# arnab39/equiadapt

Hardware: AMD Instinct MI355X
Metric: canonicalize+invert images/sec (224x224 C8) (higher is better)
Workload: dtype f32 (resampling / FFT / accumulation in fp32; the network's channel contraction as 2xfp16 split of every fp32 operand (within one fp32 ulp), 3 exact products, fp32 accumulate -- closer to fp64 than the fp32 matrix instruction, see step_ms_by_gemm_form); 1 GPU; configs[1]: 224x224x3 synthetic, C8, GroupEquivariantImageCanonicalization + ESCNNEquivariantNetwork in e2cnn's LAYER SHAPES (32 fields x 8 = 256 ch, k5, 3 layers, crop 0.8, resize 96) with this repository's own filter-bank parameterisation (bilinear-rotated banks; e2cnn's steerable basis is not restated -- e2cnn-trained weights enter via load_exported_dense), forward, then invert_canonicalization; batch_per_gpu=256, global_batch=256, parallelism=dp1 (no collective in the forward path)

## Files before the change

equiadapt_amd/_lib.py:

```python
import ctypes
import os
import subprocess
import threading

_HERE = os.path.dirname(os.path.abspath(__file__))
ROOT = os.path.dirname(_HERE)
CSRC = os.path.join(_HERE, "csrc")
SO_PATH = os.environ.get("EQA_LIB") or os.path.join(CSRC, "libeqa_hip.so")
SOURCES = [os.path.join(CSRC, f) for f in ("group_action.hip", "crop_resize.hip", "nearest_action.hip", "pooling.hip", "batchnorm.hip", "winograd.hip", "lift_conv.hip", "lift_conv_wide.hip", "lift_wgrad.hip", "pointcloud.hip", "vnsmall_train.hip", "vnsmall_tail.hip", "fftconv.hip", "fft_filter.hip", "lift_fft.hip", "cgemm3m.hip", "cgemm3m_bf16.hip", "smallconv.hip", "planegemm.hip", "convnet_train.hip", "fourier_act.hip", "nbody.hip")]
HEADERS = [os.path.join(CSRC, "eqa_common.hpp"), os.path.join(CSRC, "vn_common.hpp"), os.path.join(CSRC, "fft48.inc"), os.path.join(CSRC, "fft_common.inc"), os.path.join(CSRC, "cgemm3m_common.inc")]
INCLUDE = os.path.join(ROOT, "include")

ABI_VERSION = 3

_c_f = ctypes.POINTER(ctypes.c_float)
_c_i = ctypes.POINTER(ctypes.c_int32)
_vp = ctypes.c_void_p
_int = ctypes.c_int

SIGNATURES = {
    "eqa_abi_version": (_int, []),
    "eqa_set_option": (_int, [_int, _int]),
    "eqa_get_option": (_int, [_int]),
    "eqa_fold_edge_pad_workspace_bytes": (ctypes.c_int64, [_int] * 4),
    "eqa_fold_edge_pad": (_int, [_vp, _vp, _vp, _int, _int, _int, _int, _vp]),
    "eqa_canon_transform_fwd": (_int, [_vp, _vp, _vp, _vp, _vp] + [_int] * 6 + [_vp]),
    "eqa_invert_action_fwd": (_int, [_vp, _vp, _vp, _vp, _vp, _vp] + [_int] * 6 + [_vp]),
    "eqa_group_action_pair": (_int, [_vp] * 4 + [_int, _int] + [_vp] * 5 + [_int, _int, _vp] + [_int] * 4 + [_vp]),
    "eqa_orbit_expand_fwd": (_int, [_vp, _vp, _vp, _vp] + [_int] * 5 + [_vp]),
    "eqa_group_action_fwd": (_int, [_vp, _vp, _vp, _vp, _vp, _vp] + [_int] * 12 + [_vp]),
    "eqa_group_action_fwd_hint": (_int, [_vp, _vp, _vp, _vp, _vp, _vp] + [_int] * 13 + [_vp]),
    "eqa_crop_resize_aa": (_int, [_vp] * 6 + [_int] * 9 + [_vp]),
    "eqa_mask_action_nearest": (_int, [_vp] * 5 + [_int] * 4 + [_vp]),
    "eqa_mask_action_nearest_planes": (_int, [_vp] * 5 + [_int] * 4 + [_vp]),
    "eqa_boxes_action": (_int, [_vp] * 5 + [_int, ctypes.c_float, _int, _vp]),
    "eqa_image_action_nearest": (_int, [_vp] * 5 + [_int] * 10 + [_vp]),
    "eqa_group_action_bwd_tiles": (_int, [_int, _int]),
    "eqa_group_action_bwd": (_int, [_vp] * 8 + [_int] * 12 + [_vp]),
    "eqa_group_action_bwd_theta": (_int, [_vp] * 8 + [_int] * 12 + [_vp]),
    "eqa_group_pool_workspace_bytes": (ctypes.c_int64, [_int] * 4),
    "eqa_group_pool_argmax": (_int, [_vp, _vp, _vp, _vp] + [_int] * 4 + [_vp]),
    "eqa_window_sums": (_int, [_vp, _vp, _vp, _int, _vp] + [_int] * 5 + [_vp]),
    "eqa_bn_partial_blocks": (ctypes.c_int64, [ctypes.c_int64]),
    "eqa_bn_stats_nhwc": (_int, [_vp, _vp, ctypes.c_int64, _int, _vp]),
    "eqa_bn_relu_dropout_nhwc": (_int, [_vp, _vp, _vp, _vp, ctypes.c_int64, _int, ctypes.c_float, ctypes.c_uint32, _vp]),
    "eqa_bn_bwd_reduce_nhwc": (_int, [_vp] * 5 + [ctypes.c_float, _vp, ctypes.c_int64, _int, _vp, _vp, ctypes.c_uint32, _vp]),
    "eqa_bn_bwd_apply_nhwc": (_int, [_vp] * 8 + [ctypes.c_float, _vp, ctypes.c_int64, _int, _vp, _vp, ctypes.c_uint32, _vp]),
    "eqa_window_sums_nhwc_act": (_int, [_vp, _vp, _vp, _int, ctypes.c_float, ctypes.c_uint32, _vp, _vp] + [_int] * 5 + [_vp]),
    "eqa_bn_bwd_reduce_nhwc_wsgrad": (_int, [_vp] * 4 + [ctypes.c_float, _vp] + [_int] * 5 + [_vp, _vp, ctypes.c_uint32, _vp]),
    "eqa_bn_bwd_apply_nhwc_wsgrad": (_int, [_vp] * 7 + [ctypes.c_float, _vp] + [_int] * 5 + [_vp, _vp, ctypes.c_uint32, _vp]),
    "eqa_vn_blocks": (_int, [_int]),
    "eqa_vn_knn": (_int, [_vp, _vp, _int, _int, _int, _vp]),
    "eqa_vn_convpos_stats": (_int, [_vp, _vp, _vp, _vp, _int, _int, _int, _vp]),
    "eqa_vn_convpos_fwd": (_int, [_vp] * 7 + [_int, _int, _int, _vp]),
    "eqa_vn_convpos_bwd_reduce": (_int, [_vp] * 10 + [_int, _int, _int, _vp]),
    "eqa_vn_convpos_bwd_apply": (_int, [_vp] * 12 + [_int, _int, _int, _vp]),
    "eqa_vn_convpos_max_fwd": (_int, [_vp] * 9 + [_int, _int, _int, _vp]),
    "eqa_vn_convpos_max_bwd_reduce": (_int, [_vp] * 11 + [_int, _int, _int, _vp]),
    "eqa_vn_convpos_max_bwd_apply": (_int, [_vp] * 13 + [_int, _int, _int, _vp]),
    "eqa_vn_tail_blocks": (_int, [_int]),
    "eqa_vn_tail_partial_floats": (_int, [_int]),
    "eqa_vn_tail_pass": (_int, [_int] + [_vp] * 8 + [_int, _int, _vp]),
    "eqa_vn_bn_finalize": (_int, [_vp, _int, _int, _int, ctypes.c_int64] + [_vp] * 5 + [ctypes.c_float, ctypes.c_float, _vp, _vp]),
    "eqa_vn_bn_bwd_finalize": (_int, [_vp, _int, _int, _int, ctypes.c_int64, _vp, _vp, _vp]),
    "eqa_window_grad_table": (_int, [_vp, _vp] + [_int] * 5 + [_vp]),
    "eqa_window_sums_gemv_bwd_workspace_bytes": (ctypes.c_int64, [_int, _int]),
    "eqa_window_sums_gemv_bwd": (_int, [_vp] * 6 + [_int, _int, _int, ctypes.c_double, _vp]),
    "eqa_window_sums_gemv": (_int, [_vp, _vp, _vp, _int, _int, _int, ctypes.c_double, ctypes.c_double, _vp]),
    "eqa_lift_conv_nhwc": (_int, [_vp, _vp, _vp, _int, _vp] + [_int] * 7 + [_vp]),
    "eqa_lift_conv_grouped": (_int, [_vp, _vp, _vp, _int, _vp] + [_int] * 7 + [_vp]),
    "eqa_lift_conv_stats_rows": (_int, [_int] * 7),
    "eqa_lift_conv_nhwc_stats": (_int, [_vp, _vp, _vp, _vp] + [_int] * 7 + [_vp]),
    "eqa_lift_conv_wgrad_supported": (_int, [_int] * 7),
    "eqa_lift_conv_wgrad_workspace_bytes": (ctypes.c_int64, [_int] * 7),
    "eqa_lift_conv_wgrad_nhwc": (_int, [_vp, _vp, _vp, _vp] + [_int] * 7 + [_vp]),
    "eqa_plane_gemm_supported": (_int, [_int, _int]),
    "eqa_plane_gemm": (_int, [_vp, _vp, _vp, ctypes.c_longlong, _int, _int, _int, _vp]),
    "eqa_winograd_f2k5_input": (_int, [_vp, _vp, _vp, _int, _int, _int, _int, _int, _vp]),
    "eqa_winograd_f2k5_output": (_int, [_vp, _vp, _int, _vp, _int, _int, _int, _int, _vp]),
    "eqa_winograd_f4k5_input": (_int, [_vp, _vp, _vp, _int, _int, _int, _int, _int, _vp]),
    "eqa_winograd_f4k5_output": (_int, [_vp, _vp, _int, _vp, _int, _int, _int, _int, _vp]),
    "eqa_winograd_f2k5_input_padded": (_int, [_vp, _vp, _int, _int, _int, _int, _int, _vp]),
    "eqa_winograd_f4k5_input_padded": (_int, [_vp, _vp, _int, _int, _int, _int, _int, _vp]),
    "eqa_winograd_f2k5_output_adjoint": (_int, [_vp, _vp, _int, _int, _int, _int, _vp]),
    "eqa_winograd_f4k5_output_adjoint": (_int, [_vp, _vp, _int, _int, _int, _int, _vp]),
    "eqa_winograd_f2k5_output_sums_workspace_bytes": (ctypes.c_int64, [_int] * 4),
    "eqa_winograd_f2k5_output_sums": (_int, [_vp, _vp, _int, _vp, _vp] + [_int] * 5 + [_vp]),
    "eqa_winograd_f4k5_output_sums": (_int, [_vp, _vp, _int, _vp, _vp] + [_int] * 5 + [_vp]),
    "eqa_fft48k5_tiles": (ctypes.c_int64, [_int]),
    "eqa_fft48k5_tile_pitch": (ctypes.c_int64, [ctypes.c_int64]),
    "eqa_fft48k5_frequencies": (_int, []),
    "eqa_fft48k5_filter_spectra": (_int, [_vp, _vp, _int, _int, _int, _vp]),
    "eqa_fft48k5_input_grad": (_int, [_vp, _vp, _vp] + [_int] * 4 + [_vp]),
    "eqa_fft48k5_grad_transform": (_int, [_vp, _vp, _vp] + [_int] * 4 + [_vp]),
    "eqa_fft48k5_filter_grad": (_int, [_vp, _vp, _int, _int, _vp]),
    "eqa_fft48k5_filter_grad3m": (_int, [_vp, _vp, _int, _int, _vp]),
    "eqa_fft48k5_cgemm3m_supported": (_int, [_int, _int]),
    "eqa_fft48k5_spectra3m_floats": (ctypes.c_int64, [_int, _int]),
    "eqa_fft48k5_filter_spectra3m": (_int, [_vp, _vp, _int, _int, _int, _vp]),
    "eqa_fft48k5_cgemm3m": (_int, [_vp, _vp, _vp, ctypes.c_int64, _int, _int, _vp]),
    "eqa_lift_conv_wide_supported": (_int, [_int, _int, _int, _int]),
    "eqa_lift_conv_wide_weight_floats": (ctypes.c_int64, [_int, _int, _int, _int]),
    "eqa_lift_conv_wide": (_int, [_vp, _vp, _vp, _int, _vp, _int, _int, _int, _int, _int, _int, _int, _vp]),
    "eqa_lift_conv_wide_wgrad_workspace_bytes": (ctypes.c_int64, [_int, _int, _int, _int]),
    "eqa_lift_conv_wide_wgrad": (_int, [_vp, _vp, _vp, _vp, _int, _int, _int, _int, _int, _int, _int, _vp]),
    "eqa_fft48k5_spectra3m_bf16_bytes": (ctypes.c_int64, [_int, _int]),
    "eqa_fft48k5_spectra3m_split": (_int, [_vp, _vp, _int, _int, _vp]),
    "eqa_fft48k5_cgemm3m_bf16x3": (_int, [_vp, _vp, _vp, ctypes.c_int64, _int, _int, _int, _vp]),
    "eqa_fft48k5_spectra3m_f16_bytes": (ctypes.c_int64, [_int, _int]),
    "eqa_fft48k5_spectra3m_split_f16": (_int, [_vp, _vp, _int, _int, ctypes.c_float, _vp]),
    "eqa_fft48k5_cgemm3m_f16x2": (_int, [_vp, _vp, _vp, ctypes.c_int64, _int, _int, _vp, _int, ctypes.c_float, _vp]),
    "eqa_fft48k5_wgrad3m_supported": (_int, [_int, _int]),
    "eqa_fft48k5_wgrad3m": (_int, [_vp, _vp, _vp, ctypes.c_int64, _int, _int, _vp]),
    "eqa_fft48k5_group": (_int, [_int, _int]),
    "eqa_fft48k5_workspace_bytes": (ctypes.c_int64, [_int] * 4),
    "eqa_fft48k5_input": (_int, [_vp, _vp, _vp, _vp] + [_int] * 5 + [_vp]),
    "eqa_fft48k5_input_grouped": (_int, [_vp, _vp, _vp, _vp] + [_int] * 5 + [_vp]),
    "eqa_fft48k5_input_grouped_supported": (_int, [_int]),
    "eqa_lift5_fft48k5_input_supported": (_int, [_int] * 4),
    "eqa_lift5_fft48k5_input": (_int, [_vp, _vp, _vp, _int, _vp] + [_int] * 4 + [_vp]),
    "eqa_lift5_fft48k5_input_dcmax": (_int, [_vp, _vp, _vp, _int, _vp, _vp] + [_int] * 4 + [_vp]),
    "eqa_lift5_pieces_f16_bytes": (ctypes.c_int64, [_int]),
    "eqa_absmax_slots": (_int, [_vp, ctypes.c_int64, _vp, _vp]),
    "eqa_lift5_fft48k5_input_f16x2": (_int, [_vp, _vp, ctypes.c_float, _vp, _int, _vp, _int, _vp, _vp] + [_int] * 4 + [_vp]),
    "eqa_lift5_pieces_bytes": (ctypes.c_int64, [_int]),
    "eqa_lift5_fft48k5_input_bf16x3": (_int, [_vp, _vp, _vp, _int, _vp] + [_int] * 4 + [_vp]),
    "eqa_fft48k5_output": (_int, [_vp, _vp, _vp, _int, _vp] + [_int] * 4 + [_vp]),
    "eqa_fft48k5_output_stats_rows": (ctypes.c_int64, [_int] * 4),
    "eqa_fft48k5_output_stats": (_int, [_vp, _vp, _vp, _vp] + [_int] * 4 + [_vp]),
    "eqa_fft48k5_output_sums": (_int, [_vp, _vp, _vp, _int, _vp, _vp] + [_int] * 5 + [_vp]),
    "eqa_fft48_supported": (_int, [_int]),
    "eqa_fft48_tiles": (ctypes.c_int64, [_int, _int]),
    "eqa_fft48_workspace_bytes": (ctypes.c_int64, [_int] * 5),
    "eqa_fft48_filter_spectra": (_int, [_vp, _vp, _int, _int, _int, _int, _vp]),
    "eqa_fft48_filter_spectra3m": (_int, [_vp, _vp, _int, _int, _int, _int, _vp]),
    "eqa_fft48_input": (_int, [_vp, _vp, _vp, _vp] + [_int] * 6 + [_vp]),
    "eqa_fft48_grad_transform": (_int, [_vp, _vp, _vp] + [_int] * 5 + [_vp]),
    "eqa_fft48_output": (_int, [_vp, _vp, _vp, _int, _vp] + [_int] * 5 + [_vp]),
    "eqa_fft48_input_grad": (_int, [_vp, _vp, _vp] + [_int] * 5 + [_vp]),
    "eqa_fft48_filter_grad": (_int, [_vp, _vp, _int, _int, _int, _int, _vp]),
    "eqa_conv_s2_supported": (_int, [_int] * 5),
    "eqa_conv_s2": (_int, [_vp, _vp, _vp, _int, _vp] + [_int] * 8 + [_vp]),
    "eqa_conv_s2_wgrad_supported": (_int, [_int] * 5),
    "eqa_conv_s2_wgrad_workspace_bytes": (ctypes.c_int64, [_int] * 8),
    "eqa_conv_s2_wgrad": (_int, [_vp] * 4 + [_int] * 8 + [_vp]),
    "eqa_conv_s2_dgrad_supported": (_int, [_int] * 4),
    "eqa_conv_s2_dgrad": (_int, [_vp] * 3 + [_int] * 7 + [_vp]),
    "eqa_bn_act_fwd": (_int, [_vp] * 5 + [ctypes.c_int64, _int, _int, _vp]),
    "eqa_bn_act_partial_blocks": (ctypes.c_int64, [ctypes.c_int64]),
    "eqa_bn_act_stats": (_int, [_vp, _vp, ctypes.c_int64, _int, _vp]),
    "eqa_bn_act_finalize": (_int, [_vp, ctypes.c_int64, _int, _vp, _vp, ctypes.c_double, ctypes.c_double] + [_vp] * 6 + [_vp]),
    "eqa_bn_act_bwd_finalize": (_int, [_vp, ctypes.c_int64, _int] + [_vp] * 7 + [_vp]),
    "eqa_bn_act_bwd_reduce": (_int, [_vp] * 8 + [ctypes.c_int64, _int, _int, _vp]),
    "eqa_bn_act_bwd_apply": (_int, [_vp] * 11 + [ctypes.c_int64, _int, _int, _vp]),
    "eqa_affine_relu_rows": (_int, [_vp, _vp, _vp, _vp, ctypes.c_int64, _int, _vp]),
    "eqa_cosine_group_activations": (_int, [_vp, _vp, _vp, _int, _int, _int, ctypes.c_float, _vp]),
    "eqa_bias_relu_nhwc": (_int, [_vp, _vp, ctypes.c_int64, _int, _vp]),
    "eqa_window_sums_nhwc_workspace_bytes": (ctypes.c_int64, [_int] * 4),
    "eqa_window_sums_nhwc": (_int, [_vp, _vp, _vp, _int, _vp, _vp] + [_int] * 5 + [_vp]),
    "eqa_window_sums_bwd_expand_nhwc": (_int, [_vp, _vp] + [_int] * 5 + [_vp]),
    "eqa_group_argmax": (_int, [_vp, _vp, _int, _int, _vp]),
    "eqa_vnsmall_workspace_bytes": (ctypes.c_int64, [_int, _int]),
    "eqa_vnsmall_fwd": (_int, [_vp, _vp, _vp, _vp, _int, _int, _int, _int, _vp]),
    "eqa_vnsmall_canonicalize": (_int, [_vp] * 6 + [_int] * 4 + [_vp]),
    "eqa_so3_rotate": (_int, [_vp, _vp, _vp, _int, _int, _int, _vp]),
    "eqa_gram_schmidt": (_int, [_vp, _vp, _int, _vp]),
    "eqa_gram_schmidt_bwd": (_int, [_vp, _vp, _vp, _int, _vp]),
    "eqa_modified_gram_schmidt": (_int, [_vp, _vp, _int, _vp]),
    "eqa_rigid_rows": (_int, [_vp, _vp, _vp, _vp, _int, _int, _vp]),
    "eqa_fourier_elu_fwd": (_int, [_vp, _vp, _vp, _vp, ctypes.c_longlong, _int, _vp]),
    "eqa_fourier_elu_bwd": (_int, [_vp, _vp, _vp, _vp, _vp, ctypes.c_longlong, _int, _vp]),
    "eqa_vndeepsets_param_count": (_int, [_int] * 3),
    "eqa_vndeepsets_bwd_blocks": (_int, [_int]),
    "eqa_nbody_adjacency": (_int, [_vp, _vp, ctypes.c_longlong, _int, _vp, _vp, _vp]),
    "eqa_vndeepsets_fwd": (_int, [_vp] * 7 + [_int] * 5 + [ctypes.c_float] + [_int] * 3 + [_vp]),
    "eqa_vndeepsets_train_fwd": (_int, [_vp] * 9 + [_int] * 5 + [ctypes.c_float] + [_int] * 3 + [_vp]),
    "eqa_vndeepsets_bwd": (_int, [_vp] * 10 + [_int] * 5 + [ctypes.c_float] + [_int] * 3 + [_vp]),
}

_lock = threading.Lock()
_lib = None


def source_hash(*names: str) -> str:
    import hashlib

    h = hashlib.sha1()
    for path in [os.path.join(CSRC, n) for n in names] + HEADERS:
        with open(path, "rb") as f:
            h.update(f.read())
    return h.hexdigest()[:16]


class EqaLibraryError(RuntimeError):
    pass


def build(force: bool = False, verbose: bool = False, extra_flags=(), out: str = None) -> str:
    import hashlib
    from concurrent.futures import ThreadPoolExecutor

    if extra_flags and not out:
        raise ValueError("a variant build (extra_flags) needs its own `out`: it must not replace the product library")
    out = out or SO_PATH
    hdr_time = max(os.path.getmtime(p) for p in HEADERS + [os.path.join(INCLUDE, "eqa_hip.h")])
    newest_src = max(hdr_time, max(os.path.getmtime(p) for p in SOURCES))
    if not force and not extra_flags and os.path.exists(out) and os.path.getmtime(out) >= newest_src:
        return out
    hipcc = os.environ.get("HIPCC", "/opt/rocm/bin/hipcc")
    flags = ["--offload-arch=gfx950", "-O3", "-fno-slp-vectorize", "-std=c++17", "-fPIC", "-I", INCLUDE, *extra_flags]
    tag = hashlib.sha1(" ".join(flags).encode()).hexdigest()[:10]
    objdir = os.path.join(CSRC, "_obj")
    os.makedirs(objdir, exist_ok=True)
    import fcntl

    lock_file = open(os.path.join(objdir, ".lock"), "w")
    fcntl.flock(lock_file, fcntl.LOCK_EX)
    try:
        if not force and not extra_flags and os.path.exists(out) and os.path.getmtime(out) >= newest_src:
            return out
        return _build_locked(hipcc, flags, tag, objdir, out, hdr_time, force, verbose, bool(extra_flags))
    finally:
        fcntl.flock(lock_file, fcntl.LOCK_UN)
        lock_file.close()


def _pid_alive(pid: int) -> bool:
    try:
        os.kill(pid, 0)
    except ProcessLookupError:
        return False
    except PermissionError:
        return True
    return True


def _build_locked(hipcc, flags, tag, objdir, out, hdr_time, force, verbose, variant):
    from concurrent.futures import ThreadPoolExecutor
    import re
    import time

    started = time.time()

    def compile_one(src):
        obj = os.path.join(objdir, f"{os.path.splitext(os.path.basename(src))[0]}.{tag}.o")
        if not force and os.path.exists(obj) and os.path.getmtime(obj) >= max(hdr_time, os.path.getmtime(src)):
            return obj, None
        tmp_obj = f"{obj}.tmp{os.getpid()}"
        cmd = [hipcc, *flags, "-c", src, "-o", tmp_obj]
        if verbose:
            print(" ".join(cmd))
        res = subprocess.run(cmd, capture_output=True, text=True)
        if res.returncode != 0:
            if os.path.exists(tmp_obj):
                os.remove(tmp_obj)
            return obj, f"{' '.join(cmd)}\n{res.stdout}\n{res.stderr}"
        os.replace(tmp_obj, obj)
        return obj, None

    with ThreadPoolExecutor(max_workers=min(6, os.cpu_count() or 1)) as pool:
        results = list(pool.map(compile_one, SOURCES))
    errors = [e for _, e in results if e]
    if errors:
        raise EqaLibraryError("hipcc failed:\n" + "\n".join(errors))
    tmp = out + f".tmp{os.getpid()}"
    cmd = [hipcc, "--offload-arch=gfx950", "-shared", "-fPIC", *[o for o, _ in results], "-o", tmp]
    res = subprocess.run(cmd, capture_output=True, text=True)
    if res.returncode != 0:
        raise EqaLibraryError(f"link failed ({res.returncode}):\n{res.stdout}\n{res.stderr}")
    os.replace(tmp, out)
    if not variant:
        keep = {os.path.basename(o) for o, _ in results}
        for name in os.listdir(objdir):
            path = os.path.join(objdir, name)
            try:
                m = re.search(r"\.o\.tmp(\d+)$", name)
                if m:
                    if not _pid_alive(int(m.group(1))):
                        os.remove(path)
                elif name.endswith(".o") and name not in keep and os.path.getmtime(path) < started:
                    os.remove(path)
            except OSError:
                pass
    return out


def load() -> ctypes.CDLL:
    global _lib
    if _lib is not None:
        return _lib
    with _lock:
        if _lib is not None:
            return _lib
        if not os.path.exists(SO_PATH):
            raise EqaLibraryError(
                f"{SO_PATH} is missing. Build it with `python -c 'import __graft_entry__ as g; g.build()'` "
                "(hipcc --offload-arch=gfx950). equiadapt_amd has no CPU fallback."
            )
        lib = ctypes.CDLL(SO_PATH)
        for name, (restype, argtypes) in SIGNATURES.items():
            try:
                fn = getattr(lib, name)
            except AttributeError as exc:
                raise EqaLibraryError(f"{SO_PATH} does not export {name}; rebuild it") from exc
            fn.restype = restype
            fn.argtypes = argtypes
        if lib.eqa_abi_version() != ABI_VERSION:
            raise EqaLibraryError("libeqa_hip.so ABI version mismatch; rebuild it")
        _lib = lib
    return _lib


_ERRORS = {-1: "invalid argument", -2: "kernel launch failed", -3: "unsupported size/shape"}


def check(status: int, what: str) -> None:
    if status != 0:
        raise EqaLibraryError(f"{what} failed: {_ERRORS.get(status, status)}")
```

equiadapt_amd/csrc/crop_resize.hip:

```cpp
#include "eqa_common.hpp"

namespace {

constexpr int kAaBand = 8;
#ifndef EQA_AA_WIDE_MIN_K
#define EQA_AA_WIDE_MIN_K 8
#endif
constexpr int kAaMaxK = 20;

__global__ __launch_bounds__(kThreads) void crop_resize_aa_kernel(const float* __restrict__ x, float* __restrict__ y,
                                                                 const float* __restrict__ wx, const int32_t* __restrict__ x0,
                                                                 const float* __restrict__ wy, const int32_t* __restrict__ y0,
                                                                 int H, int W, int OH, int OW, int K, int max_rows) {
  extern __shared__ __attribute__((aligned(16))) float aa_tmp[];
  const int plane = blockIdx.y;
  const int r0 = blockIdx.x * kAaBand, r1 = min(r0 + kAaBand, OH);
  const int ybeg = y0[r0];
  const int yend = min(y0[r1 - 1] + K, H);
  const int nrows = min(yend - ybeg, max_rows);
  const float* src = x + (size_t)plane * H * W;
  const int rows_par = kThreads / OW;
  if (rows_par >= 1) {
    const int ox = threadIdx.x % OW, rsub = threadIdx.x / OW;
    if (rsub < rows_par) {
      const int xs = x0[ox];
      float wv[EQA_AA_WIDE_MIN_K];
      int xo[EQA_AA_WIDE_MIN_K];
#pragma unroll
      for (int j = 0; j < EQA_AA_WIDE_MIN_K; ++j) {
        wv[j] = j < K ? wx[ox * K + j] : 0.0f;
        xo[j] = min(xs + j, W - 1);
      }
      for (int ry = rsub; ry < nrows; ry += rows_par) {
        const float* row = src + (size_t)(ybeg + ry) * W;
        float xv[EQA_AA_WIDE_MIN_K];
#pragma unroll
        for (int j = 0; j < EQA_AA_WIDE_MIN_K; ++j) xv[j] = j < K ? row[xo[j]] : 0.0f;
        float acc = 0.0f;
#pragma unroll
        for (int j = 0; j < EQA_AA_WIDE_MIN_K; ++j)
          if (j < K) acc += wv[j] * xv[j];
        aa_tmp[ry * OW + ox] = acc;
      }
    }
  } else {
    for (int idx = threadIdx.x; idx < nrows * OW; idx += kThreads) {
      const int ry = idx / OW, ox = idx - ry * OW;
      const float* row = src + (size_t)(ybeg + ry) * W;
      const int xs = x0[ox];
      float acc = 0.0f;
#pragma unroll
      for (int j = 0; j < EQA_AA_WIDE_MIN_K; ++j)
        if (j < K) acc += wx[ox * K + j] * row[min(xs + j, W - 1)];
      aa_tmp[ry * OW + ox] = acc;
    }
  }
  __syncthreads();
  float* dst = y + (size_t)plane * OH * OW;
  for (int idx = threadIdx.x; idx < (r1 - r0) * OW; idx += kThreads) {
    const int r = idx / OW, ox = idx - r * OW;
    const int oy = r0 + r;

    const int ys = y0[oy] - ybeg;
    float acc = 0.0f;
#pragma unroll
    for (int j = 0; j < EQA_AA_WIDE_MIN_K; ++j)
      if (j < K) acc += wy[oy * K + j] * aa_tmp[min(ys + j, nrows - 1) * OW + ox];
    dst[(size_t)oy * OW + ox] = acc;
  }
}


template <int K, int BAND, int NL>
__global__ __launch_bounds__(kThreads, (NL > 5 && K > 5) ? 2 : 4) void crop_resize_aa_staged_kernel(
    const float* __restrict__ x, float* __restrict__ y,
                                                                        const float* __restrict__ wx, const int32_t* __restrict__ x0,
                                                                        const float* __restrict__ wy, const int32_t* __restrict__ y0,
                                                                        int planes, int H, int W, int OH, int OW, int cap_rows,
                                                                        int xb, int xl) {
  extern __shared__ __attribute__((aligned(16))) float aa_tmp[];
  float* rows = aa_tmp;
  float* tmp = aa_tmp + (size_t)cap_rows * xl;
  float* tabw = tmp + (size_t)cap_rows * OW;
  int* taby = reinterpret_cast<int*>(tabw + BAND * K);
  const int r0 = blockIdx.y * BAND, r1 = min(r0 + BAND, OH);
  const int nband = r1 - r0;
  const int plane0 = (int)(blockIdx.z * kXcd + blockIdx.x), plane_step = (int)(gridDim.z * kXcd);
  const int rows_par = kThreads / OW;
  const int ox = rows_par >= 1 ? threadIdx.x % OW : 0, rsub = rows_par >= 1 ? threadIdx.x / OW : 0;
  const int xs_g = x0[ox];
  float wv[K];
  int xo[K];
#pragma unroll
  for (int j = 0; j < K; ++j) {
    wv[j] = wx[ox * K + j];
    xo[j] = min(xs_g - xb + j, xl - 1);
  }
  if ((int)threadIdx.x < nband * K) tabw[threadIdx.x] = wy[r0 * K + threadIdx.x];
  const int ybeg = y0[r0];
  if ((int)threadIdx.x < nband) taby[threadIdx.x] = y0[r0 + threadIdx.x] - ybeg;
  const int yend = min(y0[r1 - 1] + K, H);
  const int nrows = min(yend - ybeg, cap_rows);
  const int nq = xl >> 2;
  const int tq = threadIdx.x & 63, tr = threadIdx.x >> 6;
  const bool prefetch = nq <= 64 && nrows <= 4 * NL;
  const size_t plane_sz = (size_t)H * W;
  const float* src0 = x + (size_t)ybeg * W + xb;
  typedef float aa_f4 __attribute__((ext_vector_type(4)));
  aa_f4 v[NL];
#define EQA_AA_PF_LOAD(plane_)                                                                                          \
  do {                                                                                                                  \
    const float* src_ = src0 + (size_t)(plane_) * plane_sz;                                                             \
    _Pragma("unroll") for (int k = 0; k < NL; ++k)                                                           \
      v[k] = *reinterpret_cast<const aa_f4*>(src_ + (size_t)min(tr + 4 * k, nrows - 1) * W + 4 * min(tq, nq - 1));     \
  } while (0)
  __builtin_amdgcn_s_waitcnt(0x0070);
  if (prefetch && plane0 < planes) EQA_AA_PF_LOAD(plane0);
  for (int plane = plane0; plane < planes; plane += plane_step) {
    if (prefetch) {
      if (tq < nq) {
#pragma unroll
        for (int k = 0; k < NL; ++k)
          if (tr + 4 * k < nrows) *reinterpret_cast<aa_f4*>(rows + (tr + 4 * k) * xl + 4 * tq) = v[k];
      }
      if (plane + plane_step < planes) EQA_AA_PF_LOAD(plane + plane_step);
    } else {
      const float* src = src0 + (size_t)plane * plane_sz;
      for (int q = tq; q < nq; q += 64)
        for (int rb = tr; rb < nrows; rb += 4) *reinterpret_cast<aa_f4*>(rows + rb * xl + 4 * q) = *reinterpret_cast<const aa_f4*>(src + (size_t)rb * W + 4 * q);
    }
    __syncthreads();
    if (rows_par >= 1) {
      if (rsub < rows_par) {
        for (int ry0 = rsub; ry0 < nrows; ry0 += 4 * rows_par) {
          float acc[4] = {0.0f, 0.0f, 0.0f, 0.0f};
#pragma unroll
          for (int u = 0; u < 4; ++u) {
            const float* row = rows + min(ry0 + u * rows_par, nrows - 1) * xl;
#pragma unroll
            for (int j = 0; j < K; ++j)
              acc[u] += wv[j] * row[xo[j]];
          }
#pragma unroll
          for (int u = 0; u < 4; ++u)
            if (ry0 + u * rows_par < nrows) tmp[(ry0 + u * rows_par) * OW + ox] = acc[u];
        }
      }
    } else {
      for (int idx = threadIdx.x; idx < nrows * OW; idx += kThreads) {
        const int ry = idx / OW, oxx = idx - ry * OW;
        const float* row = rows + ry * xl;
        const int xs = x0[oxx] - xb;
        float acc = 0.0f;
#pragma unroll
        for (int j = 0; j < K; ++j)
          acc += wx[oxx * K + j] * row[min(xs + j, xl - 1)];
        tmp[ry * OW + oxx] = acc;
      }
    }
    __syncthreads();
    float* dst = y + (size_t)plane * OH * OW;
    for (int idx = threadIdx.x; idx < nband * OW; idx += kThreads) {
      const int r = idx / OW, oxx = idx - r * OW;
      const int ys = taby[r];
      float acc = 0.0f;
#pragma unroll
      for (int j = 0; j < K; ++j)
        acc += tabw[r * K + j] * tmp[min(ys + j, nrows - 1) * OW + oxx];
      dst[(size_t)(r0 + r) * OW + oxx] = acc;
    }
    __syncthreads();
  }
#undef EQA_AA_PF_LOAD
}

__global__ __launch_bounds__(kThreads) void crop_resize_aa_wide_kernel(const float* __restrict__ x, float* __restrict__ y,
                                                                      const float* __restrict__ wx, const int32_t* __restrict__ x0,
                                                                      const float* __restrict__ wy, const int32_t* __restrict__ y0,
                                                                      int H, int W, int OH, int OW, int K, int max_rows, int xbeg,
                                                                      int xlen, int pad_shift, int row_stride, int rpi) {
  extern __shared__ __attribute__((aligned(16))) float aa_tmp[];
  float* rowbuf = aa_tmp + (size_t)max_rows * OW;
  const int plane = blockIdx.y;
  const int r0 = blockIdx.x * kAaBand, r1 = min(r0 + kAaBand, OH);
  const int ybeg = y0[r0];
  const int yend = min(y0[r1 - 1] + K, H);
  const int nrows = min(yend - ybeg, max_rows);
  const float* src = x + (size_t)plane * H * W;
  auto pos = [&](int e) { return pad_shift ? e + (e >> pad_shift) : e; };
  const bool fixed_col = (kThreads % OW) == 0 && K <= kAaMaxK;
  const bool vec_stage = rpi <= 8 && (xlen & 3) == 0 && (xbeg & 3) == 0 && (W & 3) == 0 && ((((uintptr_t)src) & 15) == 0);
  const int ox_fixed = threadIdx.x % OW;
  const int xs_fixed = x0[ox_fixed] - xbeg;
  float wreg[kAaMaxK];
#pragma unroll
  for (int j = 0; j < kAaMaxK; ++j) wreg[j] = (fixed_col && j < K) ? wx[ox_fixed * K + j] : 0.0f;
  const bool prefetch = vec_stage && xlen <= 4 * kThreads;
  const int e_pf = 4 * threadIdx.x;
  float4 pf[8];
  auto pf_load = [&](int ry0) {
    const int nr = min(rpi, nrows - ry0);
#pragma unroll
    for (int rr = 0; rr < 8; ++rr)
      pf[rr] = *reinterpret_cast<const float4*>(src + (size_t)(ybeg + ry0 + min(rr, nr - 1)) * W + xbeg + min(e_pf, xlen - 4));
  };
  if (prefetch && nrows > 0) pf_load(0);
  for (int ry0 = 0; ry0 < nrows; ry0 += rpi) {
    const int nr = min(rpi, nrows - ry0);
    if (prefetch) {
      if (e_pf < xlen) {
#pragma unroll
        for (int rr = 0; rr < 8; ++rr) {
          if (rr < nr) {
            float* lrow = rowbuf + rr * row_stride;
            lrow[pos(e_pf)] = pf[rr].x; lrow[pos(e_pf + 1)] = pf[rr].y; lrow[pos(e_pf + 2)] = pf[rr].z; lrow[pos(e_pf + 3)] = pf[rr].w;
          }
        }
      }
      if (ry0 + rpi < nrows) pf_load(ry0 + rpi);
    } else if (vec_stage) {
      for (int e = 4 * threadIdx.x; e < xlen; e += 4 * kThreads) {
        float4 v[8];
#pragma unroll
        for (int rr = 0; rr < 8; ++rr)
          v[rr] = *reinterpret_cast<const float4*>(src + (size_t)(ybeg + ry0 + min(rr, nr - 1)) * W + xbeg + e);
#pragma unroll
        for (int rr = 0; rr < 8; ++rr) {
          if (rr < nr) {
            float* lrow = rowbuf + rr * row_stride;
            lrow[pos(e)] = v[rr].x; lrow[pos(e + 1)] = v[rr].y; lrow[pos(e + 2)] = v[rr].z; lrow[pos(e + 3)] = v[rr].w;
          }
        }
      }
    } else {
      for (int rr = 0; rr < nr; ++rr) {
        const float* grow = src + (size_t)(ybeg + ry0 + rr) * W + xbeg;
        float* lrow = rowbuf + rr * row_stride;
        for (int e = threadIdx.x; e < xlen; e += kThreads) lrow[pos(e)] = grow[e];
      }
    }
    __syncthreads();
    if (fixed_col) {
      for (int rr = threadIdx.x / OW; rr < nr; rr += kThreads / OW) {
        const float* row = rowbuf + rr * row_stride;
        float acc = 0.0f;
#pragma unroll
        for (int j = 0; j < kAaMaxK; ++j)
          if (j < K) acc += wreg[j] * row[pos(min(xs_fixed + j, xlen - 1))];
        aa_tmp[(ry0 + rr) * OW + ox_fixed] = acc;
      }
    } else {
      for (int idx = threadIdx.x; idx < nr * OW; idx += kThreads) {
        const int rr = idx / OW, ox = idx - rr * OW;
        const float* row = rowbuf + rr * row_stride;
        const int xs = x0[ox] - xbeg;
        float acc = 0.0f;
        for (int j = 0; j < K; ++j) acc += wx[ox * K + j] * row[pos(min(xs + j, xlen - 1))];
        aa_tmp[(ry0 + rr) * OW + ox] = acc;
      }
    }
    __syncthreads();
  }
  float* dst = y + (size_t)plane * OH * OW;
  for (int idx = threadIdx.x; idx < (r1 - r0) * OW; idx += kThreads) {
    const int r = idx / OW, ox = idx - r * OW;
    const int oy = r0 + r;
    const int ys = y0[oy] - ybeg;
    float acc = 0.0f;
    for (int j = 0; j < K; ++j) acc += wy[oy * K + j] * aa_tmp[min(ys + j, nrows - 1) * OW + ox];
    dst[(size_t)oy * OW + ox] = acc;
  }
}

constexpr int kAaStreamRows = 8;
__global__ __launch_bounds__(kThreads) void crop_resize_aa_stream_kernel(const float* __restrict__ x, float* __restrict__ y,
                                                                        const float* __restrict__ wx, const int32_t* __restrict__ x0,
                                                                        const float* __restrict__ wy, const int32_t* __restrict__ y0,
                                                                        int H, int W, int OH, int OW, int K, int xbeg, int xlen,
                                                                        int pad_shift, int row_stride) {
  extern __shared__ __attribute__((aligned(16))) float aa_rows[];
  const int plane = blockIdx.y;
  const int r0 = blockIdx.x * kAaBand, nr_out = min(kAaBand, OH - r0);
  int ys[kAaBand];
#pragma unroll
  for (int r = 0; r < kAaBand; ++r) ys[r] = y0[r0 + min(r, nr_out - 1)];
  const int ybeg = ys[0];
  const int span = ys[kAaBand - 1] + K - ybeg;
  const float* src = x + (size_t)plane * H * W + xbeg;
  const int e = 4 * (int)threadIdx.x;
  const int e_ld = min(e, xlen - 4);
  auto pos = [&](int i) { return pad_shift ? i + (i >> pad_shift) : i; };
  float4 acc[kAaBand];
#pragma unroll
  for (int r = 0; r < kAaBand; ++r) acc[r] = make_float4(0.f, 0.f, 0.f, 0.f);
  auto load8 = [&](float4 (&v)[kAaStreamRows], int yc) {
#pragma unroll
    for (int q = 0; q < kAaStreamRows; ++q)
      v[q] = *reinterpret_cast<const float4*>(src + (size_t)min(ybeg + yc + q, H - 1) * W + e_ld);
  };
  const int lane = threadIdx.x & 63;
  const int wq = lane >> 3, wr = lane & 7;
  const int ys_w = y0[r0 + min(wr, nr_out - 1)];
  auto wload = [&](int yc) {
    const int t = ybeg + yc + wq - ys_w;
    const bool ok = wr < nr_out && t >= 0 && t < K && yc + wq < span;
    return ok ? wy[(size_t)(r0 + wr) * K + min(max(t, 0), K - 1)] : 0.0f;
  };
  auto add8 = [&](const float4 (&v)[kAaStreamRows], float wv) {
#pragma unroll
    for (int q = 0; q < kAaStreamRows; ++q) {
#pragma unroll
      for (int r = 0; r < kAaBand; ++r) {
        const float w = __builtin_bit_cast(float, __builtin_amdgcn_readlane(__builtin_bit_cast(int, wv), 8 * q + r));
        acc[r].x += w * v[q].x; acc[r].y += w * v[q].y; acc[r].z += w * v[q].z; acc[r].w += w * v[q].w;
      }
    }
  };
  static_assert(kAaStreamRows == 8 && kAaBand == 8, "one weight per lane: 8 rows of a trip x 8 output rows = 64 lanes");
  float4 va[kAaStreamRows], vb[kAaStreamRows];
  float wa, wb = 0.0f;
  load8(va, 0);
  wa = wload(0);
  for (int yc = 0; yc < span; yc += 2 * kAaStreamRows) {
    if (yc + kAaStreamRows < span) { load8(vb, yc + kAaStreamRows); wb = wload(yc + kAaStreamRows); }
    add8(va, wa);
    if (yc + 2 * kAaStreamRows < span) { load8(va, yc + 2 * kAaStreamRows); wa = wload(yc + 2 * kAaStreamRows); }
    if (yc + kAaStreamRows < span) add8(vb, wb);
  }
  float* dst = y + (size_t)plane * OH * OW;
#pragma unroll
  for (int half = 0; half < 2; ++half) {
    if (e < xlen) {
#pragma unroll
      for (int rr = 0; rr < kAaBand / 2; ++rr) {
        float* lrow = aa_rows + rr * row_stride;
        const float4 v = acc[half * (kAaBand / 2) + rr];
        lrow[pos(e)] = v.x; lrow[pos(e + 1)] = v.y; lrow[pos(e + 2)] = v.z; lrow[pos(e + 3)] = v.w;
      }
    }
    __syncthreads();
    for (int idx = threadIdx.x; idx < (kAaBand / 2) * OW; idx += kThreads) {
      const int rr = idx / OW, ox = idx - rr * OW;
      const int r = half * (kAaBand / 2) + rr;
      if (r < nr_out) {
        const float* row = aa_rows + rr * row_stride;
        const int xs = x0[ox] - xbeg;
        float a = 0.0f;
        for (int j = 0; j < K; ++j) a += wx[ox * K + j] * row[pos(min(xs + j, xlen - 1))];
        dst[(size_t)(r0 + r) * OW + ox] = a;
      }
    }
    __syncthreads();
  }
}

}

extern "C" {

int eqa_crop_resize_aa(const float* x, float* y, const float* wx, const int32_t* x0, const float* wy, const int32_t* y0,
                       int planes, int H, int W, int OH, int OW, int K, int max_rows, int x_begin, int x_span, void* stream) {
  if (!x || !y || !wx || !x0 || !wy || !y0 || planes < 0 || H <= 0 || W <= 0 || OH <= 0 || OW <= 0 || K <= 0 || max_rows <= 0)
    return EQA_ERR_INVALID_ARG;
  const size_t lds = (size_t)max_rows * OW * sizeof(float);
  if (lds > 96 * 1024 || planes > 65535) return EQA_ERR_UNSUPPORTED;
  if (planes == 0) return EQA_OK;
  const dim3 grid((OH + kAaBand - 1) / kAaBand, planes);
  if (K > EQA_AA_WIDE_MIN_K && x_span > 0 && x_begin >= 0 && x_begin + x_span <= W) {
    const int stride = (x_span + OW / 2) / OW;
    const int pad_shift = (stride >= 2 && (stride & 1) == 0) ? __builtin_ctz((unsigned)stride) : 0;
    const int row_stride = x_span + (pad_shift ? (x_span >> pad_shift) : 0) + 1;
    const size_t row_bytes = (size_t)row_stride * sizeof(float);
    const int rpi = (int)std::min<size_t>(8, lds + row_bytes <= 96 * 1024 ? (96 * 1024 - lds) / row_bytes : 0);
    const size_t lds2 = lds + (size_t)rpi * row_bytes;
    static const bool stream_off = [] { const char* e = getenv("EQA_AA_STREAM"); return e && e[0] == '0'; }();
    if (!stream_off && x_span <= 4 * kThreads && (x_span & 3) == 0 && (x_begin & 3) == 0 && (W & 3) == 0 && (((uintptr_t)x) & 15) == 0 &&
        (size_t)(kAaBand / 2) * row_bytes <= 64 * 1024) {
      hipLaunchKernelGGL(crop_resize_aa_stream_kernel, grid, dim3(kThreads), (kAaBand / 2) * row_bytes, (hipStream_t)stream, x, y, wx, x0, wy,
                         y0, H, W, OH, OW, K, x_begin, x_span, pad_shift, row_stride);
      return launch_status();
    }
    if (rpi >= 1) {
      hipLaunchKernelGGL(crop_resize_aa_wide_kernel, grid, dim3(kThreads), lds2, (hipStream_t)stream, x, y, wx, x0, wy, y0, H, W, OH,
                         OW, K, max_rows, x_begin, x_span, pad_shift, row_stride, rpi);
      return launch_status();
    }
  }
  static const bool staged_off = [] { const char* e = getenv("EQA_AA_STAGED"); return e && e[0] == '0'; }();
  if (!staged_off && K <= EQA_AA_WIDE_MIN_K && (W & 3) == 0 && (((uintptr_t)x) & 15) == 0 && x_span > 0 && x_begin >= 0 &&
      x_begin + x_span <= W) {
    const int xb = x_begin & ~3, xl = std::min(W, (x_begin + x_span + 3) & ~3) - xb;
    static const int band_env = [] { const char* e = getenv("EQA_AA_BAND"); return e ? atoi(e) : 0; }();
    int band = band_env == 16 ? 16 : (band_env == 8 ? 8 : (OH >= 64 ? 16 : 8));
    auto staged_lds = [&](int bnd) { return ((size_t)(bnd / kAaBand) * max_rows * (xl + OW) + bnd * (EQA_AA_WIDE_MIN_K + 1)) * sizeof(float); };
    if (band == 16 && band_env != 16 && (staged_lds(16) > 64 * 1024 || 16 * K > kThreads)) band = 8;
    const int cap_rows = (band / kAaBand) * max_rows;
    const size_t lds3 = staged_lds(band);
    if (lds3 <= 64 * 1024 && band * K <= kThreads) {
      static const int per_cu = [] { const char* e = getenv("EQA_AA_BLOCKS_PER_CU"); return e ? std::max(1, atoi(e)) : 12; }();
      const int nbands = (OH + band - 1) / band;
      const int groups = std::max(1, (std::min(planes, (256 * per_cu + nbands - 1) / nbands) + kXcd - 1) / kXcd);
      const bool few = cap_rows <= 20;
#define EQA_AA_STAGED(K_)                                                                                                              \
  case K_:                                                                                                                             \
    if (band == 16)                                                                                                                    \
      hipLaunchKernelGGL((crop_resize_aa_staged_kernel<K_, 16, 10>), dim3(kXcd, nbands, groups), dim3(kThreads), lds3, (hipStream_t)stream, x, \
                         y, wx, x0, wy, y0, planes, H, W, OH, OW, cap_rows, xb, xl);                                                   \
    else if (few)                                                                                                                      \
      hipLaunchKernelGGL((crop_resize_aa_staged_kernel<K_, 8, 5>), dim3(kXcd, nbands, groups), dim3(kThreads), lds3, (hipStream_t)stream, x,  \
                         y, wx, x0, wy, y0, planes, H, W, OH, OW, cap_rows, xb, xl);                                                   \
    else                                                                                                                               \
      hipLaunchKernelGGL((crop_resize_aa_staged_kernel<K_, 8, 10>), dim3(kXcd, nbands, groups), dim3(kThreads), lds3, (hipStream_t)stream, x, \
                         y, wx, x0, wy, y0, planes, H, W, OH, OW, cap_rows, xb, xl);                                                   \
    break
      switch (K) {
        EQA_AA_STAGED(1); EQA_AA_STAGED(2); EQA_AA_STAGED(3); EQA_AA_STAGED(4); EQA_AA_STAGED(5); EQA_AA_STAGED(6); EQA_AA_STAGED(7);
        EQA_AA_STAGED(8);
        default: return EQA_ERR_UNSUPPORTED;
      }
#undef EQA_AA_STAGED
      return launch_status();
    }
  }
  hipLaunchKernelGGL(crop_resize_aa_kernel, grid, dim3(kThreads), lds, (hipStream_t)stream, x, y, wx, x0, wy, y0, H, W, OH, OW, K,
                     max_rows);
  return launch_status();
}

}
```

equiadapt_amd/images/canonicalization/discrete_group.py:

```python
import math
from typing import Any, Dict, List, Optional, Tuple, Union

import torch
import torch.nn.functional as F

from equiadapt_amd import ops
from equiadapt_amd.common.basecanonicalization import DiscreteGroupCanonicalization
from equiadapt_amd.images import geometry
from equiadapt_amd.images.transforms import CenterCrop, EdgePad, Resize
from equiadapt_amd.images.utils import (
    canonicalize_masks,
    device_tables,
    canonicalize_boxes,
    flip_boxes,
    flip_masks,
    get_action_on_image_features,
    rotate_boxes,
    rotate_masks,
)



def _get(hyperparams: Any, name: str):
    if isinstance(hyperparams, dict):
        return hyperparams[name]
    return getattr(hyperparams, name)

class _CanonTransformFn(torch.autograd.Function):

    @staticmethod
    def forward(ctx, x, rotation, reflection, gidx, theta, flags, pad, num_rotations):
        ctx.save_for_backward(x, gidx, theta, flags if flags is not None else torch.empty(0))
        ctx.pad, ctx.num_rotations, ctx.has_flags = pad, num_rotations, flags is not None
        return ops.canon_transform(x, gidx, theta, flags, pad)

    @staticmethod
    def backward(ctx, grad_y):
        x, gidx, theta, flags = ctx.saved_tensors
        flags = flags if ctx.has_flags else None
        pad, N = ctx.pad, ctx.num_rotations
        need_x, need_rot, need_ref = ctx.needs_input_grad[0], ctx.needs_input_grad[1], ctx.needs_input_grad[2]
        grad_y = grad_y.contiguous()
        gx = g_rot = g_ref = None
        if need_x or need_rot:
            gx, g_ang = ops.group_action_bwd(x, grad_y, gidx, theta, flags, None, pad, (pad, pad), need_x, need_rot)
            if need_rot:
                g_rot = -g_ang
        if need_ref:
            ridx = gidx % N
            y0 = ops.canon_transform(x, ridx, theta, flags, pad)
            y1 = ops.canon_transform(x, ridx + N, theta, flags, pad)
            g_ref = (grad_y * (y1 - y0)).sum(dim=(1, 2, 3))
        return gx, g_rot, g_ref, None, None, None, None, None


class DiscreteGroupImageCanonicalization(DiscreteGroupCanonicalization):

    def __init__(self, canonicalization_network: torch.nn.Module, canonicalization_hyperparams: Any, in_shape: tuple):
        super().__init__(canonicalization_network)
        self.beta = _get(canonicalization_hyperparams, "beta")
        assert len(in_shape) == 3, "Input shape should be in the format (channels, height, width)"
        self.in_shape = tuple(int(s) for s in in_shape)
        is_grayscale = self.in_shape[0] == 1
        self.pad_size = 0 if is_grayscale else math.ceil(self.in_shape[-1] * 0.5)
        self.pad = torch.nn.Identity() if is_grayscale else EdgePad(self.pad_size)
        self.crop = torch.nn.Identity() if is_grayscale else CenterCrop((self.in_shape[-2], self.in_shape[-1]))
        self.crop_canonization = (
            torch.nn.Identity() if is_grayscale else CenterCrop((
                math.ceil(self.in_shape[-2] * _get(canonicalization_hyperparams, "input_crop_ratio")),
                math.ceil(self.in_shape[-1] * _get(canonicalization_hyperparams, "input_crop_ratio"))))
        )
        self.resize_canonization = (
            torch.nn.Identity() if is_grayscale else Resize(size=_as_size(_get(canonicalization_hyperparams, "resize_shape")))
        )
        self._consts: Dict[str, torch.Tensor] = {}


    def _group_constants(self, device: torch.device) -> Tuple[torch.Tensor, Optional[torch.Tensor]]:
        key = f"{device}:{self.num_rotations}:{self.group_type}"
        hit = self._consts.get(key)
        if hit is None:
            angles = geometry.group_angles(self.num_rotations)
            if self.group_type == "roto-reflection":
                rot = torch.cat([angles, angles], dim=0)
                ref = torch.cat([torch.zeros(self.num_rotations), torch.ones(self.num_rotations)], dim=0)
                hit = (rot.to(device), ref.to(device))
            else:
                hit = (angles.to(device), None)
            self._consts[key] = hit
        return hit

    def groupactivations_to_groupelement(self, group_activations: torch.Tensor,
                                         group_index: Optional[torch.Tensor] = None) -> dict:
        if group_index is None:
            group_index = self.group_index(group_activations)
        rot_comp, ref_comp = self._group_constants(group_activations.device)
        if not self.training and self.gradient_trick == "straight_through":
            element = {"rotation": torch.index_select(rot_comp, 0, group_index)}
            if ref_comp is not None:
                element["reflection"] = torch.index_select(ref_comp, 0, group_index)
            element["group_index"] = group_index
            return element
        onehot = self.groupactivations_to_groupelementonehot(group_activations, group_index)
        if self.gradient_trick != "straight_through":
            group_index = onehot.detach().argmax(dim=-1).to(torch.int32)
        element = {"rotation": torch.sum(onehot * rot_comp, dim=-1)}
        if ref_comp is not None:
            element["reflection"] = torch.sum(onehot * ref_comp, dim=-1)
        element["group_index"] = group_index
        return element

    def get_group_activations(self, x: torch.Tensor) -> torch.Tensor:
        raise NotImplementedError(
            "get_group_activations is not implemented for the DiscreteGroupImageCanonicalization class")

    def get_groupelement(self, x: torch.Tensor) -> Dict[str, torch.Tensor]:
        group_activations = self.get_group_activations(x)
        group_index = self.group_index(group_activations)
        element = self.groupactivations_to_groupelement(group_activations, group_index)
        if not hasattr(self, "canonicalization_info_dict"):
            self.canonicalization_info_dict = {}
        self.canonicalization_info_dict["group_index"] = element.pop("group_index")
        self.canonicalization_info_dict["argmax_index"] = group_index
        self.canonicalization_info_dict["group_element"] = element
        self.canonicalization_info_dict["group_activations"] = group_activations
        return element

    def transformations_before_canonicalization_network_forward(self, x: torch.Tensor) -> torch.Tensor:
        crop, resize = self.crop_canonization, self.resize_canonization
        if (x.is_cuda and x.dtype == torch.float32 and not (torch.is_grad_enabled() and x.requires_grad) and isinstance(resize, Resize)
                and resize.antialias):
            from equiadapt_amd.images.transforms import resized_output_size

            out_hw = resized_output_size(crop.size, resize.size)
            if tuple(out_hw) == tuple(x.shape[-2:]) == tuple(crop.size):
                return x
            key = (tuple(x.shape[-2:]), crop.size, out_hw, str(x.device))
            tabs = self._consts.get(key)
            if tabs is None:
                t = geometry.aa_resize_tables(tuple(x.shape[-2:]), crop.size, out_hw)
                tabs = tuple(v.to(x.device) if isinstance(v, torch.Tensor) else v for v in t)
                self._consts[key] = tabs
            return ops.crop_resize_aa(x, tabs, out_hw)
        return resize(crop(x))


    def canonicalize(self, x: torch.Tensor, targets: Optional[List] = None, **kwargs: Any
                     ) -> Union[torch.Tensor, Tuple[torch.Tensor, List]]:
        self.device = x.device
        element = self.get_groupelement(x)
        gidx = self.canonicalization_info_dict["group_index"]
        reflections = "reflection" in element
        H, W = x.shape[-2:]
        pad = self.pad_size
        theta, flags = device_tables("canonicalize", self.num_rotations, reflections, (H + 2 * pad, W + 2 * pad), x.device)
        x = _CanonTransformFn.apply(x, element["rotation"], element.get("reflection"), gidx, theta, flags, pad,
                                    self.num_rotations)

        if targets:
            image_width = x.shape[-1]
            box_list = [t_["boxes"] for t_ in targets]
            counts = [int(b.shape[0]) for b in box_list]
            if sum(counts) > 0 and all(b.is_cuda and b.dim() == 2 and b.shape[1] == 4 and b.dtype == torch.float32 for b in box_list) \
                    and element["rotation"].dtype == torch.float32:
                for t_, nb in zip(targets, canonicalize_boxes(box_list, element["rotation"].detach(), image_width, reflections)):
                    t_["boxes"] = nb
            else:
                if reflections:
                    for t in range(len(targets)):
                        targets[t]["boxes"] = flip_boxes(targets[t]["boxes"], image_width)
                for t in range(len(targets)):
                    targets[t]["boxes"] = rotate_boxes(targets[t]["boxes"], element["rotation"][t], image_width)
            masks = [t_["masks"] for t_ in targets]
            if all(m.is_cuda and m.dtype == torch.uint8 and m.dim() == 3 and m.shape[-2:] == masks[0].shape[-2:] for m in masks):
                new = canonicalize_masks(masks, gidx, self.num_rotations, flip_all=reflections)
                for t in range(len(targets)):
                    targets[t]["masks"] = new[t]
            else:
                rot_host = element["rotation"].detach().cpu()
                for t in range(len(targets)):
                    m = flip_masks(targets[t]["masks"]) if reflections else targets[t]["masks"]
                    targets[t]["masks"] = rotate_masks(m, -rot_host[t].item())
            return x, targets
        return x

    def invert_canonicalization(self, x_canonicalized_out: torch.Tensor, **kwargs: Any) -> torch.Tensor:
        induced_rep_type = kwargs.get("induced_rep_type", "regular")
        element = dict(self.canonicalization_info_dict["group_element"])
        element["group_index"] = self.canonicalization_info_dict["group_index"]
        return get_action_on_image_features(
            feature_map=x_canonicalized_out,
            group_info_dict=self.group_info_dict,
            group_element_dict=element,
            induced_rep_type=induced_rep_type,
        )


def _as_size(resize_shape: Any):
    if isinstance(resize_shape, int):
        return resize_shape
    return tuple(int(s) for s in resize_shape)


def _num_group(group_type: str, num_rotations: int) -> int:
    return num_rotations if group_type == "rotation" else 2 * num_rotations


class GroupEquivariantImageCanonicalization(DiscreteGroupImageCanonicalization):

    def __init__(self, canonicalization_network: torch.nn.Module, canonicalization_hyperparams: Any, in_shape: tuple):
        super().__init__(canonicalization_network, canonicalization_hyperparams, in_shape)
        self.group_type = canonicalization_network.group_type
        self.num_rotations = canonicalization_network.num_rotations
        self.num_group = _num_group(self.group_type, self.num_rotations)
        self.group_info_dict = {"num_rotations": self.num_rotations, "num_group": self.num_group}

    def get_group_activations(self, x: torch.Tensor) -> torch.Tensor:
        x = self.transformations_before_canonicalization_network_forward(x)
        return self.canonicalization_network(x)


class OptimizedGroupEquivariantImageCanonicalization(DiscreteGroupImageCanonicalization):

    def __init__(self, canonicalization_network: torch.nn.Module, canonicalization_hyperparams: Any, in_shape: tuple):
        super().__init__(canonicalization_network, canonicalization_hyperparams, in_shape)
        self.group_type = _get(canonicalization_hyperparams, "group_type")
        self.num_rotations = _get(canonicalization_hyperparams, "num_rotations")
        self.artifact_err_wt = _get(canonicalization_hyperparams, "artifact_err_wt")
        self.num_group = _num_group(self.group_type, self.num_rotations)
        self.out_vector_size = canonicalization_network.out_vector_size
        size = _get(canonicalization_hyperparams, "resize_shape")
        self.group_augment_size = int(size)
        gray = self.in_shape[0] == 1
        self.group_augment_pad = 0 if gray else math.ceil(self.group_augment_size * 0.5)
        self.crop_group_augment = torch.nn.Identity() if gray else CenterCrop(self.group_augment_size)
        self.pad_group_augment = torch.nn.Identity() if gray else EdgePad(self.group_augment_pad)
        self.reference_vector = torch.nn.Parameter(
            torch.randn(1, self.out_vector_size), requires_grad=_get(canonicalization_hyperparams, "learn_ref_vec"))
        self.group_info_dict = {"num_rotations": self.num_rotations, "num_group": self.num_group}

    def group_augment(self, x: torch.Tensor) -> torch.Tensor:
        s = x.shape[-1]
        pad = self.group_augment_pad
        theta, flags = device_tables("orbit", self.num_rotations, self.group_type == "roto-reflection",
                                     (s + 2 * pad, s + 2 * pad), x.device)
        return ops.orbit_expand(x, theta, flags, pad)

    def _rotate_batch(self, x: torch.Tensor, rot_index: torch.Tensor, sign: float) -> torch.Tensor:
        s = x.shape[-1]
        pad = self.group_augment_pad
        theta = geometry.rotation_theta(sign * geometry.group_angles(self.num_rotations) * 1.0, (s + 2 * pad, s + 2 * pad))
        return ops.group_action(x, rot_index.to(torch.int32), theta.to(x.device), None, None, pad, (s, s), (pad, pad))

    def get_group_activations(self, x: torch.Tensor) -> torch.Tensor:
        x = self.transformations_before_canonicalization_network_forward(x)
        x_augmented = self.group_augment(x)
        vector_out = self.canonicalization_network(x_augmented)
        self.canonicalization_info_dict = {"vector_out": vector_out}

        if self.artifact_err_wt:
            rot_idx = torch.randint(0, self.num_rotations, (x_augmented.shape[0],), device=x.device)
            x_dummy = self._rotate_batch(x_augmented, rot_idx, -1.0)
            x_dummy = self._rotate_batch(x_dummy, rot_idx, +1.0)
            vector_out_dummy = self.canonicalization_network(x_dummy)
            self.canonicalization_info_dict.update({"vector_out_dummy": vector_out_dummy})

        if vector_out.is_cuda and vector_out.dtype == torch.float32 and not torch.is_grad_enabled():
            return ops.cosine_group_activations(vector_out, self.reference_vector.detach(), self.num_group)
        scalar_out = F.cosine_similarity(self.reference_vector.repeat(vector_out.shape[0], 1), vector_out)
        return scalar_out.reshape(self.num_group, -1).T

    def get_optimization_specific_loss(self) -> torch.Tensor:
        vectors = self.canonicalization_info_dict["vector_out"]
        artifact = 0
        if self.artifact_err_wt:
            artifact = F.mse_loss(self.canonicalization_info_dict["vector_out_dummy"], vectors)
        v = vectors.reshape(self.num_group, -1, self.out_vector_size).permute((1, 0, 2))
        gram = v @ v.permute((0, 2, 1))
        mask = 1.0 - torch.eye(self.num_group, device=self.device)
        return torch.abs(gram * mask).mean() + self.artifact_err_wt * artifact
```

equiadapt_amd/images/canonicalization_networks/escnn_networks.py:

```python
import os
from typing import List, Sequence

import torch
import torch.nn as nn
import torch.nn.functional as F

from equiadapt_amd.images.canonicalization_networks.custom_group_equivariant_layers import (
    RotationEquivariantConv,
    RotationEquivariantConvLift,
    RotoReflectionEquivariantConv,
    RotoReflectionEquivariantConvLift,
)
from equiadapt_amd import ops
from equiadapt_amd.common.utils import update_running_stats
from equiadapt_amd.images.canonicalization_networks import fftconv, winograd
from equiadapt_amd.images.canonicalization_networks.pooling import (
    WindowSumsFunction,
    conv_then_group_pool,
    group_pool,
    window_sums_to_activations,
)
from equiadapt_amd.images.canonicalization_networks.steerable_networks import ESCNNSteerableNetwork


# ... 270 lines not shown
class ESCNNEquivariantNetwork(nn.Module):
    def __init__(self, in_shape: tuple, out_channels: int, kernel_size: int, group_type: str = "rotation",
                 num_rotations: int = 4, num_layers: int = 1):
        super().__init__()
        self.in_channels = in_shape[0]
        self.out_channels = out_channels
        self.kernel_size = kernel_size
        self.group_type = group_type
        self.num_rotations = num_rotations
        if group_type == "rotation":
            lift, conv = RotationEquivariantConvLift, RotationEquivariantConv
        elif group_type == "roto-reflection":
            lift, conv = RotoReflectionEquivariantConvLift, RotoReflectionEquivariantConv
        else:
            raise ValueError("group_type must be rotation or roto-reflection for now.")
        self.num_group_elements = num_rotations if group_type == "rotation" else 2 * num_rotations

        def block() -> List[nn.Module]:
            return [_InnerBatchNorm(out_channels, momentum=0.9), nn.ReLU(inplace=True), nn.Dropout(p=0.5)]

        mods: List[nn.Module] = [lift(self.in_channels, out_channels, kernel_size, num_rotations, device="cpu")]
        mods += block()
        for _ in range(num_layers - 2):
            mods.append(conv(out_channels, out_channels, kernel_size, num_rotations, device="cpu"))
            mods += block()
        mods.append(conv(out_channels, out_channels, kernel_size, num_rotations, device="cpu"))
        self.eqv_network = nn.Sequential(*mods)
        self._dense: Sequence = ()
        self._fold_cache: dict = {}

    def _load_from_state_dict(self, state_dict, prefix, *args, **kwargs):
        own = prefix + "eqv_network."
        for k, v in state_dict.items():
            if k.startswith(own) and ("basisexpansion" in k or k.endswith(".filter") or k.endswith(".expanded_bias")
                                      or (k.endswith(".weights") and getattr(v, "dim", lambda: 2)() == 1)):
                raise RuntimeError(
                    f"state_dict key {k!r} comes from e2cnn's steerable-basis parameterisation (the reference's ESCNNEquivariantNetwork). "
                    "equiadapt_amd.ESCNNEquivariantNetwork parameterises its layers by rotated filter banks and cannot load it by key; "
                    "export the trained layers on the e2cnn side (R2Conv.export() -> nn.Conv2d, InnerBatchNorm.export() -> nn.BatchNorm2d) "
                    "and pass them to load_exported_dense(convs, norms).")
        return super()._load_from_state_dict(state_dict, prefix, *args, **kwargs)

    def load_exported_dense(self, convs: Sequence[nn.Conv2d], norms: Sequence[nn.BatchNorm2d]) -> None:
        n_conv = sum(1 for m in self.eqv_network if hasattr(m, "expanded_weights"))
        if len(convs) != n_conv or len(norms) != n_conv - 1:
            raise ValueError(f"expected {n_conv} convs and {n_conv - 1} norms")
        E = self.num_group_elements
        cin = self.in_channels
        for i, cv in enumerate(convs):
            if cv.in_channels != cin:
                raise ValueError(f"exported conv {i} takes {cv.in_channels} channels, the network feeds it {cin}")
            cin = cv.out_channels
        for i, bn in enumerate(norms):
            if bn.num_features != convs[i].out_channels:
                raise ValueError(f"exported norm {i} has {bn.num_features} features, conv {i} produces {convs[i].out_channels}")
        self._dense = (nn.ModuleList(_DenseConv(cv, E, i == 0) for i, cv in enumerate(convs)), nn.ModuleList(norms))
        self._fold_cache.clear()

    def export_dense(self):
        E = self.num_group_elements
        convs, norms = [], []
        with torch.no_grad():
            for m in self.eqv_network:
                if hasattr(m, "expanded_weights"):
                    bank = m.expanded_weights().detach()
                    cv = nn.Conv2d(bank.shape[1], bank.shape[0], m.kernel_size, m.stride, m.padding, bias=m.bias is not None)
                    cv = cv.to(bank.device)
                    cv.weight.copy_(bank)
                    if m.bias is not None:
                        cv.bias.copy_(m.bias.detach().repeat_interleave(E))
                    convs.append(cv)
                elif isinstance(m, _InnerBatchNorm):
                    bn = nn.BatchNorm2d(m.num_features * E, eps=m.eps, momentum=m.momentum).to(m.weight.device)
                    for name in ("weight", "bias", "running_mean", "running_var"):
                        getattr(bn, name).copy_(getattr(m, name).repeat_interleave(E))
                    norms.append(bn.eval())
        return convs, norms

    def _layers(self):
        if self._dense:
            return list(self._dense[0]), list(self._dense[1])
        mods = list(self.eqv_network)
        return [m for m in mods if hasattr(m, "expanded_weights")], [m for m in mods if isinstance(m, _InnerBatchNorm)]

    def _folded(self, conv, bn):
        key = (conv.weights._version, bn.weight._version, bn.bias._version, bn.running_mean._version,
               bn.running_var._version, str(conv.weights.device))
        hit = self._fold_cache.get(id(conv))
        if hit is not None and hit[0] == key:
            return hit[1], hit[2]
        E = conv.num_group_elements
        scale = bn.weight / torch.sqrt(bn.running_var + bn.eps)
        shift = bn.bias - bn.running_mean * scale
        b = conv.bias if conv.bias is not None else torch.zeros_like(scale)
        bias = b * scale + shift
        if not isinstance(conv, _DenseConv):
            scale, bias = scale.repeat_interleave(E), bias.repeat_interleave(E)
        bank = conv.expanded_weights() * scale[:, None, None, None]
        bank, bias = bank.contiguous(memory_format=torch.channels_last), bias.contiguous()
        self._fold_cache[id(conv)] = (key, bank, bias)
        return bank, bias

    def _derived(self, conv, build, *tag):
        key = self._fold_cache[id(conv)][0]
        hit = self._fold_cache.get((*tag, id(conv)))
        if hit is None or hit[0] != key:
            hit = (key, build())
            self._fold_cache[(*tag, id(conv))] = hit
        return hit[1]

    @staticmethod
    def _plain_5x5(conv) -> bool:
        return not conv.lifting and conv.kernel_size == 5 and conv.stride == 1 and conv.padding == 0

    @staticmethod
    def _lift_kernel(conv, bank, h, narrow_unchecked: bool = False):
        if not conv.lifting or os.environ.get("EQA_LIFT_MFMA", "1") == "0":
            return None
        k, (cout, cin) = conv.kernel_size, bank.shape[:2]
        unit = conv.stride == 1 and conv.padding == 0
        if (unit or narrow_unchecked) and ops.lift_conv_supported(cin, k, k, cout):
            return "narrow"
        if (unit and h.is_contiguous(memory_format=torch.channels_last) and h.shape[-2] >= k and h.shape[-1] >= k
                and ops.lift_conv_wide_supported(cin, k, k, cout)):
            return "wide"
        return None

    def _route(self, i, h, bank, convs, nhwc):
        conv, tail = convs[i], convs[-1]
        cout, cin = bank.shape[:2]
        k, kt = conv.kernel_size, tail.kernel_size
        last_before_tail = i == len(convs) - 2
        if nhwc and self._plain_5x5(conv) and fftconv.applicable(h, cin, cout):
            return "fft5", (last_before_tail and kt in (3, 5) and tail.supports_linear_tail() and min(h.shape[-2:]) - 4 >= 2 * kt - 1), 0
        if (nhwc and not conv.lifting and k != 5 and conv.stride == 1 and conv.padding == 0
                and h.is_contiguous(memory_format=torch.channels_last) and fftconv.applicable_k(h.shape, cin, cout, k, h.device)):
            return "fftk", False, 0
        if nhwc and self._plain_5x5(conv) and winograd.applicable(h, cin, cout):
            m = winograd.tile_for(h)
            if last_before_tail and not winograd.sums_applicable(h, kt, m) and winograd.sums_applicable(h, kt, 2):
                m = 2
            return "wino", last_before_tail and winograd.sums_applicable(h, kt, m), m
        lift = self._lift_kernel(conv, bank, h) if nhwc else None
        if lift == "narrow":
            nxt = convs[i + 1] if i + 1 < len(convs) - 1 else None
            if nxt is not None and self._plain_5x5(nxt):
                if fftconv.lift_fused_applicable(h.shape, bank.shape, nxt.out_channels * nxt.num_group_elements, h.device):
                    return "lift_fused", False, 0
                if fftconv.grouped_applicable((h.shape[0], cout, h.shape[2] - k + 1, h.shape[3] - k + 1), cout, cout, h.device):
                    return "lift_grouped", False, 0
            return "lift", False, 0
        return ("lift_wide" if lift == "wide" else "lib"), False, 0

    def _forward_inference(self, x: torch.Tensor) -> torch.Tensor:
        convs, norms = self._layers()
        tail = convs[-1]
        nhwc = (self.out_channels * self.num_group_elements) % 4 == 0
        h = x.contiguous(memory_format=torch.channels_last) if nhwc else x
        pending = None
        for i, (conv, bn) in enumerate(zip(convs[:-1], norms)):
            bank, bias = self._folded(conv, bn)
            route, sums, m = self._route(i, h, bank, convs, nhwc)
            k, (H, W) = conv.kernel_size, h.shape[-2:]
            last_before_tail, shift = i == len(convs) - 2, None
            if route != "fft5" and isinstance(h, (fftconv.GroupedMap, fftconv.LiftedInput)):
                h = h.materialize()
            if route in ("fft5", "fftk", "wino"):
                in_bias, pending = pending, None
                sums_k = tail.kernel_size if sums else 0
                if route == "wino":
                    U = self._derived(conv, lambda: winograd.transform_filters(bank, m), "wino", m)
                    h = winograd.conv5x5(h, U, bias, relu=True, in_bias=in_bias, in_relu=in_bias is not None, sums_k=sums_k)
                else:
                    Bf = self._derived(conv, lambda: fftconv.spectra_for_k(bank), "fft")
                    if route == "fft5":
                        h = fftconv.conv5x5(h, Bf, bias, True, in_bias, in_bias is not None, sums_k=sums_k)
                    else:
                        h = fftconv.conv_kxk(h, Bf, k, bias, True, in_bias, in_bias is not None)
            else:
                if pending is not None:
                    ops.bias_relu_nhwc_(h, pending)
                    pending = None
                if route == "lift_fused":
                    operand = {}
                    form = fftconv.LiftedInput.form_operand()
                    if form is not None:
                        operand[form[1]] = self._derived(conv, lambda: form[2](bank), form[0])
                    h = fftconv.LiftedInput(h, bank, bias, True, **operand)
                elif route != "lib":
                    pack = ops.pack_lift_weights_wide if route == "lift_wide" else ops.pack_lift_weights
                    wpk = self._derived(conv, lambda: pack(bank), "lift")
                    if route == "lift_grouped":
                        h = fftconv.GroupedMap(ops.lift_conv_grouped(h, wpk, bias, True, k, k))
                    else:
                        h = (ops.lift_conv_wide if route == "lift_wide" else ops.lift_conv_nhwc)(h, wpk, bias, True, k, k)
                else:
                    h = F.conv2d(h, bank)
                    if last_before_tail:
                        shift = bias
                    elif nhwc and h.is_contiguous(memory_format=torch.channels_last):
                        pending = bias
                    else:
                        h = torch.relu_(h + bias[None, :, None, None])
            if sums:
                return window_sums_to_activations(h, tail, H - k + 1, W - k + 1)
            if last_before_tail:
                return conv_then_group_pool(h, tail, shift=shift, relu=shift is not None)
        raise AssertionError("unreachable: the network always has at least two convolutions")

    @staticmethod
    def _inner_bn(h: torch.Tensor, bn: nn.BatchNorm3d, E: int, conv_bias) -> torch.Tensor:
        Bn, C, H, W = h.shape
        Fd = C // E
        if bn.training or bn.running_mean is None:
            n = Bn * E * H * W
            s1 = h.sum(dim=(0, 2, 3), dtype=torch.float64).view(Fd, E).sum(1)
            s2 = (h * h).sum(dim=(0, 2, 3), dtype=torch.float64).view(Fd, E).sum(1)
            mean = s1 / n
            var = (s2 / n - mean * mean).clamp_min(0.0)
            with torch.no_grad():
                full_mean = mean if conv_bias is None else mean + conv_bias.double()
                update_running_stats(bn, full_mean, var * (n / max(n - 1, 1)))
            mean, var = mean.float(), var.float()
        else:
            mean = bn.running_mean if conv_bias is None else bn.running_mean - conv_bias
            var = bn.running_var
        scale = bn.weight * torch.rsqrt(var + bn.eps)
        shift = bn.bias - mean * scale
        return h * scale.repeat_interleave(E)[None, :, None, None] + shift.repeat_interleave(E)[None, :, None, None]

    def _forward_training(self, x: torch.Tensor) -> torch.Tensor:
        mods = list(self.eqv_network)
        convs = [m for m in mods if hasattr(m, "expanded_weights")]
        norms = [m for m in mods if isinstance(m, _InnerBatchNorm)]
        drops = [m for m in mods if isinstance(m, nn.Dropout)]
        E = self.num_group_elements
        h = x.contiguous(memory_format=torch.channels_last)
        tail = convs[-1]
        S = None
        epilogue_stats = os.environ.get("EQA_TRAIN_FUSED_BN", "1") != "0" and os.environ.get("EQA_TRAIN_EPILOGUE_STATS", "1") != "0"
        for li, (conv, bn, drop) in enumerate(zip(convs[:-1], norms, drops)):
            bank = conv.expanded_weights()
            part = None
            lift = self._lift_kernel(conv, bank, h, narrow_unchecked=True)
            if not conv.lifting and conv.kernel_size == 5 and winograd.applicable(h, bank.shape[1], bank.shape[0]):
                if (epilogue_stats and (bn.training or bn.running_mean is None) and winograd.Conv5x5Function.stats_supported(h, bank)):
                    h, part = winograd.Conv5x5Function.apply(h, bank, winograd.tile_for(h), True)
                else:
                    h = winograd.Conv5x5Function.apply(h, bank, winograd.tile_for(h))
            elif (not conv.lifting and conv.kernel_size != 5
                  and fftconv.applicable_k(h.shape, bank.shape[1], bank.shape[0], conv.kernel_size, h.device,
                                           h.is_contiguous(memory_format=torch.channels_last))):
                h = fftconv.ConvKxKFunction.apply(h, bank)
            elif lift == "narrow":
                if (epilogue_stats and (bn.training or bn.running_mean is None)
                        and ops.lift_conv_stats_supported(h.shape, conv.kernel_size, conv.kernel_size, bank.shape[0])):
                    h, part = LiftConvFunction.apply(h, bank, True)
                else:
                    h = LiftConvFunction.apply(h, bank)
            elif lift == "wide":
                h = LiftConvFunction.apply(h, bank)
            else:
                h = F.conv2d(h, bank.contiguous(memory_format=torch.channels_last))
            fused = os.environ.get("EQA_TRAIN_FUSED_BN", "1") != "0" and h.is_contiguous(memory_format=torch.channels_last)
            kt = tail.kernel_size
            if (fused and li == len(convs) - 2 and os.environ.get("EQA_TRAIN_FUSED_TAIL", "1") != "0" and kt <= ops.MAX_WINDOW_K
                    and h.shape[-2] > 2 * (kt - 1) and h.shape[-1] > 2 * (kt - 1) and h.shape[0] <= 65535):
                S = InnerBnReluDropoutWindowSums.apply(h, bn.weight, bn.bias, bn, E, conv.bias, drop.p, drop.training, kt, part)
            elif fused:
                h = InnerBnReluDropout.apply(h, bn.weight, bn.bias, bn, E, conv.bias, drop.p, drop.training, part)
            else:
                h = self._inner_bn(h, bn, E, conv.bias)
                h = F.dropout(torch.relu(h), drop.p, drop.training)
        k, O = tail.kernel_size, tail.out_channels
        H, W = h.shape[-2:]
        if S is None:
            S = WindowSumsFunction.apply(h, k)
        weff = tail.expanded_weights().view(O, E, -1).double().sum(0)
        from equiadapt_amd.images.canonicalization_networks.pooling import WindowSumsLinearFn

        if S.is_cuda and S.dtype == torch.float64 and E <= 16 and os.environ.get("EQA_WS_TABLE_KERNEL", "1") != "0":
            act = WindowSumsLinearFn.apply(S.flatten(1), weff, 1.0 / float(O * (H - k + 1) * (W - k + 1)))
        else:
            act = S.flatten(1) @ weff.t() / float(O * (H - k + 1) * (W - k + 1))
        if tail.bias is not None:
            act = act + tail.bias.double().mean()
        hidden_bias = [c.bias.sum() for c in convs[:-1] if c.bias is not None]
        if hidden_bias:
            act = act + 0.0 * torch.stack(hidden_bias).sum().double()
        return act.float()

    def _training_fast_path_ok(self, x: torch.Tensor) -> bool:
        if self._dense or not x.is_cuda or x.dtype != torch.float32 or os.environ.get("EQA_TRAIN_FAST", "1") == "0":
            return False
        if (self.out_channels * self.num_group_elements) % 4 != 0:
            return False
        convs = [m for m in self.eqv_network if hasattr(m, "expanded_weights")]
        if len(convs) < 2 or any(c.stride != 1 or c.padding != 0 for c in convs) or not convs[-1].supports_linear_tail():
            return False
        hw = x.shape[-2] - (self.kernel_size - 1) * (len(convs) - 1)
        k = convs[-1].kernel_size
        return hw >= 2 * k - 1 and x.shape[-1] - (self.kernel_size - 1) * (len(convs) - 1) >= 2 * k - 1 and hw * hw <= 12288

    def forward(self, x: torch.Tensor) -> torch.Tensor:
        if (self.training or torch.is_grad_enabled()) and self._training_fast_path_ok(x):
            return self._forward_training(x)
        if not self.training and not torch.is_grad_enabled() and x.is_cuda and x.dtype == torch.float32:
            convs, norms = self._layers()
            shrink = (self.kernel_size - 1) * (len(convs) - 1)
            oh, ow = x.shape[-2] - shrink, x.shape[-1] - shrink
            if (convs[-1].supports_linear_tail() and 0 < oh and 0 < ow and oh * ow <= 12288
                    and all(n.running_mean is not None and not n.training for n in norms)
                    and all(c.stride == 1 and c.padding == 0 and c.kernel_size == self.kernel_size for c in convs)):
                return self._forward_inference(x)
        if self._dense:
            convs, norms = self._dense
            for i, cv in enumerate(convs):
                x = cv(x)
                if i < len(norms):
                    x = F.relu(norms[i](x))
            fm = x.reshape(x.shape[0], self.out_channels, self.num_group_elements, x.shape[-2], x.shape[-1])
        else:
            fm = self.eqv_network(x)
        return group_pool(fm)
```

equiadapt_amd/images/canonicalization_networks/fftconv.py:

```python
import math
import os
from typing import Optional

import torch

from equiadapt_amd import _lib, ops
from equiadapt_amd.ops import _timed

N, NH, OUT = 48, 25, 44
F = N * (NH - 2) + 2 * NH
ENABLED = os.environ.get("EQA_CONV5_FFT", "1") != "0"
MIN_TILES = int(os.environ.get("EQA_FFT_MIN_TILES", "32"))
TRAIN_FORWARD = os.environ.get("EQA_FFT_TRAIN", "1") != "0"
GEMM = os.environ.get("EQA_FFT_GEMM", "3m")
GEMM_PIECES = os.environ.get("EQA_FFT_GEMM_PIECES", "auto")
AUTO_MIN_CIN = int(os.environ.get("EQA_FFT_GEMM_AUTO_MIN_CIN", "128"))
AUTO_MIN_CIN_H3 = int(os.environ.get("EQA_FFT_GEMM_AUTO_MIN_CIN_H3", "64"))
DCMAX_SLOTS = 256
LAST_FORM = None


def f16_form_takes(cin: int, cout: int) -> bool:
    return cout % 128 == 0 and cin % 32 == 0


def gemm_form(cin: int, cout: int, bounded: bool = False) -> str:
    if GEMM_PIECES in ("f32", "9", "6"):
        return GEMM_PIECES
    if bounded and f16_form_takes(cin, cout) and (GEMM_PIECES == "h3" or cin >= AUTO_MIN_CIN_H3):
        return "h3"
    return "6" if cin >= AUTO_MIN_CIN and cout % 128 == 0 else "f32"


def f16_scale(t: torch.Tensor) -> float:
    mx = float(t.abs().max().item())
    ex = 14 - math.frexp(mx)[1] if 0.0 < mx < float("inf") else 0
    return math.ldexp(1.0, max(-100, min(100, ex)))


class Spectra3M:

    __slots__ = ("data", "cin", "cout", "_pieces", "_pieces_f16")

    def __init__(self, data: torch.Tensor, cin: int, cout: int):
        self.data, self.cin, self.cout, self._pieces, self._pieces_f16 = data, cin, cout, None, None

    def pieces_f16(self):
        if self._pieces_f16 is None:
            lib = _lib.load()
            scale = f16_scale(self.data)
            bh = torch.empty(lib.eqa_fft48k5_spectra3m_f16_bytes(self.cin, self.cout) // 2, dtype=torch.int16, device=self.data.device)
            with torch.cuda.device(self.data.device):
                _lib.check(lib.eqa_fft48k5_spectra3m_split_f16(self.data.data_ptr(), bh.data_ptr(), self.cin, self.cout, scale,
                                                               ops._stream()), "eqa_fft48k5_spectra3m_split_f16")
            self._pieces_f16 = (bh, scale)
        return self._pieces_f16

    def pieces(self) -> torch.Tensor:
        if self._pieces is None:
            lib = _lib.load()
            bp = torch.empty(lib.eqa_fft48k5_spectra3m_bf16_bytes(self.cin, self.cout) // 2, dtype=torch.int16, device=self.data.device)
            with torch.cuda.device(self.data.device):
                _lib.check(lib.eqa_fft48k5_spectra3m_split(self.data.data_ptr(), bp.data_ptr(), self.cin, self.cout,
                                                           ops._stream()), "eqa_fft48k5_spectra3m_split")
            self._pieces = bp
        return self._pieces


def gemm3m_supported(cin: int, cout: int) -> bool:
    return GEMM == "3m" and bool(_lib.load().eqa_fft48k5_cgemm3m_supported(cin, cout))


def filter_spectra3m(bank: torch.Tensor, correlate: bool = True) -> Spectra3M:
    lib = _lib.load()
    Cout, Cin = bank.shape[:2]
    if not (bank.is_cuda and bank.dtype == torch.float32 and lib.eqa_fft48k5_cgemm3m_supported(Cin, Cout)):
        raise RuntimeError("filter_spectra3m: fp32 device bank with Cin % 32 == 0 and Cout % 64 == 0 expected")
    B3 = torch.empty(lib.eqa_fft48k5_spectra3m_floats(Cin, Cout), dtype=torch.float32, device=bank.device)
    with torch.cuda.device(bank.device):
        _lib.check(lib.eqa_fft48k5_filter_spectra3m(bank.contiguous().data_ptr(), B3.data_ptr(), Cout, Cin, int(correlate),
                                                    ops._stream()), "eqa_fft48k5_filter_spectra3m")
    return Spectra3M(B3, Cin, Cout)


def spectra_for(bank: torch.Tensor, correlate: bool = True):
    Cout, Cin = bank.shape[:2]
    if bank.is_cuda and bank.dtype == torch.float32 and gemm3m_supported(Cin, Cout):
        return filter_spectra3m(bank, correlate)
    return filter_spectra(bank, correlate=correlate)


def contract(V: torch.Tensor, B, M: int, vbound: Optional[torch.Tensor] = None) -> torch.Tensor:
    dev = V.device
    if isinstance(B, Spectra3M):
        lib = _lib.load()
        assert V.shape[2] == 2 * B.cin and V.stride(1) == 2 * B.cin and V.stride(0) == lib.eqa_fft48k5_tile_pitch(M) * 2 * B.cin
        Mo = spectra_buffer(M, 2 * B.cout, dev)
        global LAST_FORM
        form = LAST_FORM = gemm_form(B.cin, B.cout, vbound is not None)
        if form == "h3":
            bh, b_scale = B.pieces_f16()
            _lib.check(lib.eqa_fft48k5_cgemm3m_f16x2(V.data_ptr(), bh.data_ptr(), Mo.data_ptr(), M, B.cin, B.cout, vbound.data_ptr(),
                                                     vbound.numel(), b_scale, ops._stream()),
                       "eqa_fft48k5_cgemm3m_f16x2")
            return Mo
        if form in ("9", "6"):
            _lib.check(lib.eqa_fft48k5_cgemm3m_bf16x3(V.data_ptr(), B.pieces().data_ptr(), Mo.data_ptr(), M, B.cin, B.cout, int(form),
                                                      ops._stream()), "eqa_fft48k5_cgemm3m_bf16x3")
            return Mo
        _lib.check(lib.eqa_fft48k5_cgemm3m(V.data_ptr(), B.data.data_ptr(), Mo.data_ptr(), M, B.cin, B.cout,
                                           ops._stream()), "eqa_fft48k5_cgemm3m")
        return Mo
    return torch.bmm(V, B, out=spectra_buffer(M, B.shape[2], dev))


def freq_index():
    ky = torch.arange(N).repeat_interleave(NH - 2)
    kx = torch.arange(1, NH - 1).repeat(N)
    eky = torch.arange(NH).repeat_interleave(2)
    ekx = torch.tensor([0, NH - 1]).repeat(NH)
    return torch.cat([ky, eky]), torch.cat([kx, ekx])


def tiles_k(n: int, k: int) -> int:
    o = N + 1 - k
    return 0 if n < k else (n - (k - 1) + o - 1) // o


def tiles(n: int) -> int:
    return tiles_k(n, 5)


def _stands_for_channels_last(self, memory_format=torch.contiguous_format) -> bool:
    return memory_format == torch.channels_last


class GroupedMap:

    def __init__(self, data: torch.Tensor):
        assert data.dim() == 5 and data.shape[-1] == 16 and data.is_contiguous()
        self.data = data
        self.shape = torch.Size((data.shape[0], data.shape[1] * 16, data.shape[2], data.shape[3]))
        self.device, self.dtype, self.is_cuda = data.device, data.dtype, data.is_cuda

    def data_ptr(self) -> int:
        return self.data.data_ptr()

    def to_channels_last(self) -> torch.Tensor:
        n, g, h, w, _ = self.data.shape
        return self.data.permute(0, 1, 4, 2, 3).reshape(n, g * 16, h, w).contiguous(memory_format=torch.channels_last)

    materialize, is_contiguous = to_channels_last, _stands_for_channels_last


class LiftedInput:

    def __init__(self, x: torch.Tensor, bank: torch.Tensor, bias: Optional[torch.Tensor], relu: bool, pieces: Optional[torch.Tensor] = None,
                 pieces_f16=None):
        assert x.dim() == 4 and x.shape[1] == 3 and bank.shape[1:] == (3, 5, 5)
        self.x = x.contiguous(memory_format=torch.channels_last)
        self.bank = bank.contiguous(memory_format=torch.channels_last)
        self.bias, self.relu = (bias.contiguous() if bias is not None else None), bool(relu)
        self.shape = torch.Size((x.shape[0], bank.shape[0], x.shape[2] - 4, x.shape[3] - 4))
        self.device, self.dtype, self.is_cuda = x.device, x.dtype, x.is_cuda
        self._pieces = pieces
        self._pieces_f16 = pieces_f16

    @staticmethod
    def split_f16(bank: torch.Tensor):
        w = bank.float()
        C = w.shape[0]
        scale = f16_scale(w)
        wp = torch.zeros(C, 5, 8, 4, dtype=torch.float32, device=w.device)
        wp[:, :, 1:6, :3] = w.permute(0, 2, 3, 1) * scale
        chunks = wp.reshape(C, 5, 4, 8)
        h1 = chunks.half()
        h2 = (chunks - h1.float()).half()
        return torch.stack([h1, h2], dim=1).contiguous(), scale

    @staticmethod
    def split_bf16(bank: torch.Tensor) -> torch.Tensor:
        w = bank.float()
        C = w.shape[0]
        wp = torch.zeros(C, 5, 6, 4, dtype=torch.float32, device=w.device)
        wp[:, :, :5, :3] = w.permute(0, 2, 3, 1)
        chunks = torch.zeros(C, 16, 8, dtype=torch.float32, device=w.device)
        chunks[:, :15] = wp.reshape(C, 5, 3, 8).reshape(C, 15, 8)
        p0 = chunks.bfloat16()
        r1 = chunks - p0.float()
        p1 = r1.bfloat16()
        p2 = (r1 - p1.float()).bfloat16()
        assert torch.equal((p0.float() + p1.float()) + p2.float(), chunks), "the three bf16 pieces of a weight must add up exactly"
        return torch.stack([p0, p1, p2], dim=1).contiguous()

    @classmethod
    def form_operand(cls):
        return {"h2": ("lifth", "pieces_f16", cls.split_f16), "bf16x3": ("liftp", "pieces", cls.split_bf16)}.get(LIFT_FFT_FORM)

    def pieces_f16(self):
        if self._pieces_f16 is None:
            self._pieces_f16 = self.split_f16(self.bank)
        return self._pieces_f16

    def pieces(self) -> torch.Tensor:
        if self._pieces is None:
            self._pieces = self.split_bf16(self.bank)
        return self._pieces

    def spectra_into(self, V: torch.Tensor, B, st: int) -> Optional[torch.Tensor]:
        lib = _lib.load()
        nimg, C, H, W = self.shape
        dims = (nimg, H + 4, W + 4, C, st)
        px, pV = self.x.data_ptr(), V.data_ptr()
        p_b = self.bias.data_ptr() if self.bias is not None else None
        want_dc = self.relu and isinstance(B, Spectra3M) and gemm_form(B.cin, B.cout, True) == "h3"
        vbound = None
        if LIFT_FFT_FORM == "h2" and px % 16 == 0:
            wh, w_scale = self.pieces_f16()
            xbound = torch.empty(DCMAX_SLOTS, dtype=torch.float32, device=self.device)
            _lib.check(lib.eqa_absmax_slots(px, self.x.numel(), xbound.data_ptr(), st), "eqa_absmax_slots")
            if want_dc:
                vbound = torch.empty(DCMAX_SLOTS, dtype=torch.float32, device=self.device)
            _lib.check(lib.eqa_lift5_fft48k5_input_f16x2(px, wh.data_ptr(), w_scale, xbound.data_ptr(), DCMAX_SLOTS, p_b, int(self.relu), pV,
                                                         vbound.data_ptr() if want_dc else None, *dims), "eqa_lift5_fft48k5_input_f16x2")
        elif LIFT_FFT_FORM == "bf16x3":
            _lib.check(lib.eqa_lift5_fft48k5_input_bf16x3(px, self.pieces().data_ptr(), p_b, int(self.relu), pV, *dims),
                       "eqa_lift5_fft48k5_input_bf16x3")
        elif want_dc:
            vbound = torch.empty(DCMAX_SLOTS, dtype=torch.float32, device=self.device)
            _lib.check(lib.eqa_lift5_fft48k5_input_dcmax(px, self.bank.data_ptr(), p_b, 1, pV, vbound.data_ptr(), *dims),
                       "eqa_lift5_fft48k5_input_dcmax")
        else:
            _lib.check(lib.eqa_lift5_fft48k5_input(px, self.bank.data_ptr(), p_b, int(self.relu), pV, *dims), "eqa_lift5_fft48k5_input")
        return vbound

    def materialize(self) -> torch.Tensor:
        return ops.lift_conv_nhwc(self.x, ops.pack_lift_weights(self.bank), self.bias, self.relu, 5, 5)

    is_contiguous = _stands_for_channels_last


LIFT_FFT_FORM = os.environ.get("EQA_LIFT_FFT_FORM", "h2")
LIFT_FFT_FUSED_DEFAULT = "1"


def lift_fused_applicable(x_shape, bank_shape, cout_next: int, device) -> bool:
    if os.environ.get("EQA_LIFT_FFT_FUSED", LIFT_FFT_FUSED_DEFAULT) == "0" or len(x_shape) != 4:
        return False
    C, Cin, kh, kw = bank_shape
    if not _lib.load().eqa_lift5_fft48k5_input_supported(Cin, kh, kw, C):
        return False
    out_shape = (x_shape[0], C, x_shape[2] - 4, x_shape[3] - 4)
    return x_shape[2] >= 5 and x_shape[3] >= 5 and grouped_applicable(out_shape, C, cout_next, device)


def _tiles_pay(shape, cin: int, cout: int, max_waste: float) -> bool:
    if shape[1] != cin or (not gemm3m_supported(cin, cout) and ops.plane_gemm_supported(cin, cout)):
        return False
    H, W = shape[-2:]
    if H < 16 or W < 16 or shape[0] * tiles(H) * tiles(W) < MIN_TILES:
        return False
    return tiles(H) * OUT <= max_waste * (H - 4) and tiles(W) * OUT <= max_waste * (W - 4)


def grouped_applicable(shape, cin: int, cout: int, device, max_waste: float = 1.12) -> bool:
    if not (ENABLED and device.type == "cuda" and len(shape) == 4 and cin % 16 == 0):
        return False
    if os.environ.get("EQA_FFT_GROUPED", "1") == "0" or not _lib.load().eqa_fft48k5_input_grouped_supported(cin):
        return False
    return _tiles_pay(shape, cin, cout, max_waste)


def applicable(x: torch.Tensor, cin: int, cout: int, max_waste: float = 1.12) -> bool:
    if isinstance(x, (GroupedMap, LiftedInput)):
        return grouped_applicable(x.shape, cin, cout, x.device, max_waste)
    if not (ENABLED and x.is_cuda and x.dtype == torch.float32 and x.dim() == 4 and x.is_contiguous(memory_format=torch.channels_last)):
        return False
    return _tiles_pay(x.shape, cin, cout, max_waste)


def _order(C: int, G: int) -> torch.Tensor:
    p = torch.arange(2 * C)
    grp, r = p // (2 * G), p % (2 * G)
    return (r // G) * C + grp * G + r % G


def group_sizes(cin: int, cout: int):
    return (16 if cin % 16 == 0 else 1), 1


def filter_spectra(bank: torch.Tensor, groups=None, correlate: bool = True) -> torch.Tensor:
    Cout, Cin = bank.shape[:2]
    if groups is None and bank.is_cuda and bank.dtype == torch.float32:
        lib = _lib.load()
        B = torch.empty((F, 2 * Cin, 2 * Cout), dtype=torch.float32, device=bank.device)
        with torch.cuda.device(bank.device):
            _lib.check(lib.eqa_fft48k5_filter_spectra(bank.contiguous().data_ptr(), B.data_ptr(), Cout, Cin, int(correlate),
                                                      ops._stream()), "eqa_fft48k5_filter_spectra")
        return B
    assert correlate, "the host construction is the correlation (forward) form"
    gin, gout = groups if groups is not None else group_sizes(Cin, Cout)
    wp = torch.zeros(Cout, Cin, N, N, dtype=torch.float64, device=bank.device)
    wp[:, :, :5, :5] = bank.double()
    W = torch.fft.rfft2(wp).conj() / float(N * N)
    ky, kx = freq_index()
    W = W[:, :, ky.to(W.device), kx.to(W.device)]
    Wr = W.real.permute(2, 1, 0).contiguous()
    Wi = W.imag.permute(2, 1, 0).contiguous()
    top = torch.cat([Wr, Wi], dim=2)
    bot = torch.cat([-Wi, Wr], dim=2)
    full = torch.cat([top, bot], dim=1)
    full = full[:, _order(Cin, gin).to(bank.device)][:, :, _order(Cout, gout).to(bank.device)]
    return full.float().contiguous()


def spectra_buffer(M: int, width: int, device) -> torch.Tensor:
    pitch = _lib.load().eqa_fft48k5_tile_pitch(M)
    return torch.empty((F, pitch, width), dtype=torch.float32, device=device)[:, :M]


def output_stats_supported(nimg: int, OH: int, OW: int, cout: int) -> bool:
    return _lib.load().eqa_fft48k5_output_stats_rows(nimg, OH, OW, cout) > 0


KSIZES = (3, 5, 7, 9)


def _transform(name: str, k: int, *args) -> None:
    lib = _lib.load()
    if k == 5:
        _lib.check(getattr(lib, "eqa_fft48k5_" + name)(*args), "eqa_fft48k5_" + name)
    else:
        _lib.check(getattr(lib, "eqa_fft48_" + name)(*args[:-1], k, args[-1]), "eqa_fft48_" + name)


def _workspace(k: int, nimg: int, rows: int, out_cols: int, C: int, device) -> torch.Tensor:
    lib = _lib.load()
    nbytes = lib.eqa_fft48k5_workspace_bytes(nimg, rows, out_cols, C) if k == 5 else lib.eqa_fft48_workspace_bytes(nimg, rows, out_cols, C, k)
    return torch.empty(max(nbytes, 4) // 4, dtype=torch.float32, device=device)


def applicable_k(x_shape, cin: int, cout: int, k: int, device, channels_last: bool = True) -> bool:
    if not (ENABLED and k in KSIZES and k != 5 and device.type == "cuda" and channels_last and len(x_shape) == 4 and x_shape[1] == cin):
        return False
    if os.environ.get("EQA_FFT_ANYK", "1") == "0":
        return False
    nimg, _, H, W = x_shape
    if H < max(16, k) or W < max(16, k) or nimg * tiles_k(H, k) * tiles_k(W, k) < 8:
        return False
    oh, ow = H - k + 1, W - k + 1
    t = tiles_k(H, k) * tiles_k(W, k)
    fft_us = t * (F * 8 * (cin + cout) * 2.2 / 4.0e6 + F * 6 * cin * cout / 100e6)
    direct_us = oh * ow * k * k * 2 * cin * cout / 110e6
    return fft_us * 1.3 < direct_us


def spectra_for_k(bank: torch.Tensor, correlate: bool = True):
    k = bank.shape[-1]
    if k == 5:
        return spectra_for(bank, correlate)
    lib = _lib.load()
    Cout, Cin = bank.shape[:2]
    assert bank.is_cuda and bank.dtype == torch.float32 and bank.shape[-2] == k and lib.eqa_fft48_supported(k)
    st = ops._stream()
    with torch.cuda.device(bank.device):
        if gemm3m_supported(Cin, Cout):
            B3 = torch.empty(lib.eqa_fft48k5_spectra3m_floats(Cin, Cout), dtype=torch.float32, device=bank.device)
            _lib.check(lib.eqa_fft48_filter_spectra3m(bank.contiguous().data_ptr(), B3.data_ptr(), Cout, Cin, k, int(correlate), st),
                       "eqa_fft48_filter_spectra3m")
            return Spectra3M(B3, Cin, Cout)
        B = torch.empty((F, 2 * Cin, 2 * Cout), dtype=torch.float32, device=bank.device)
        _lib.check(lib.eqa_fft48_filter_spectra(bank.contiguous().data_ptr(), B.data_ptr(), Cout, Cin, k, int(correlate), st),
                   "eqa_fft48_filter_spectra")
        return B


def conv_kxk(x: torch.Tensor, B, k: int, bias: Optional[torch.Tensor], relu: bool, in_bias: Optional[torch.Tensor] = None,
             in_relu: bool = False, keep_V: Optional[list] = None, sums_k: int = 0, stats: Optional[list] = None) -> torch.Tensor:
    lib = _lib.load()
    nimg, Cin, H, W = x.shape
    if isinstance(B, Spectra3M):
        Cout = B.cout
        assert B.cin == Cin
    else:
        Cout = B.shape[2] // 2
        assert B.shape == (F, 2 * Cin, 2 * Cout)
    assert k == 5 or not (sums_k or stats is not None or isinstance(x, (GroupedMap, LiftedInput))), "k = 5 only"
    OH, OW = H - k + 1, W - k + 1
    TX = tiles_k(W, k)
    M = nimg * tiles_k(H, k) * TX
    dev = x.device
    st = ops._stream()
    V = spectra_buffer(M, 2 * Cin, dev)
    p_bias = bias.data_ptr() if bias is not None else None
    vbound = None
    with torch.cuda.device(dev):
        if isinstance(x, LiftedInput):
            assert in_bias is None and not in_relu
            with _timed("lift_fft_input"):
                vbound = x.spectra_into(V, B, st)
        else:
            T = _workspace(k, nimg, H, OW, Cin, dev)
            with _timed("fft_input"):
                _transform("input_grouped" if isinstance(x, GroupedMap) else "input", k, x.data_ptr(), T.data_ptr(), V.data_ptr(),
                           in_bias.data_ptr() if in_bias is not None else None, int(in_relu), nimg, H, W, Cin, st)
            del T
        with _timed("fft_gemm"):
            Mo = contract(V, B, M, vbound)
        if keep_V is not None:
            keep_V.append(V)
        del V
        T2 = _workspace(k, nimg, OH, OW, Cout, dev)
        if sums_k:
            S = torch.empty((nimg, Cout, sums_k, sums_k), dtype=torch.float64, device=dev)
            ws = torch.empty(nimg * OH * TX * Cout * (2 * sums_k - 1), dtype=torch.float32, device=dev)
            with _timed("fft_output_sums"):
                _lib.check(lib.eqa_fft48k5_output_sums(Mo.data_ptr(), T2.data_ptr(), p_bias, int(relu), S.data_ptr(), ws.data_ptr(),
                                                       nimg, OH, OW, Cout, sums_k, st), "eqa_fft48k5_output_sums")
            return S
        y = torch.empty((nimg, Cout, OH, OW), dtype=torch.float32, device=dev, memory_format=torch.channels_last)
        if stats is not None:
            assert bias is None and not relu
            part = torch.empty((lib.eqa_fft48k5_output_stats_rows(nimg, OH, OW, Cout), Cout, 2), dtype=torch.float64, device=dev)
            with _timed("fft_output"):
                _lib.check(lib.eqa_fft48k5_output_stats(Mo.data_ptr(), T2.data_ptr(), y.data_ptr(), part.data_ptr(), nimg, OH, OW, Cout, st),
                           "eqa_fft48k5_output_stats")
            stats.append(part)
            return y
        with _timed("fft_output"):
            _transform("output", k, Mo.data_ptr(), T2.data_ptr(), p_bias, int(relu), y.data_ptr(), nimg, OH, OW, Cout, st)
        return y


def conv5x5(x: torch.Tensor, B: torch.Tensor, bias: Optional[torch.Tensor], relu: bool,
            in_bias: Optional[torch.Tensor] = None, in_relu: bool = False, sums_k: int = 0,
            keep_V: Optional[list] = None, stats: Optional[list] = None) -> torch.Tensor:
    return conv_kxk(x, B, 5, bias, relu, in_bias, in_relu, keep_V, sums_k, stats)


def grad_spectra(dy: torch.Tensor, k: int = 5) -> torch.Tensor:
    nimg, Cout, OH, OW = dy.shape
    M = nimg * tiles_k(OH + k - 1, k) * tiles_k(OW + k - 1, k)
    T = _workspace(k, nimg, OH, OW, Cout, dy.device)
    G = spectra_buffer(M, 2 * Cout, dy.device)
    with torch.cuda.device(dy.device):
        _transform("grad_transform", k, dy.data_ptr(), T.data_ptr(), G.data_ptr(), nimg, OH, OW, Cout, ops._stream())
    return G


def filter_grad_k(V: torch.Tensor, dy: torch.Tensor, cin: int, k: int, G: Optional[torch.Tensor] = None) -> torch.Tensor:
    lib = _lib.load()
    nimg, Cout, OH, OW = dy.shape
    dev = dy.device
    M = V.shape[1]
    assert V.shape == (F, M, 2 * cin) and M == nimg * tiles_k(OH + k - 1, k) * tiles_k(OW + k - 1, k)
    st = ops._stream()
    if G is None:
        G = grad_spectra(dy, k)
    dbank = torch.empty((Cout, cin, k, k), dtype=torch.float32, device=dev)
    with torch.cuda.device(dev):
        packed = GEMM == "3m" and lib.eqa_fft48k5_wgrad3m_supported(cin, Cout) and os.environ.get("EQA_FFT_WGRAD3M", "1") != "0"
        if packed:
            D = torch.empty((F, cin, 2, Cout), dtype=torch.float32, device=dev)
            _lib.check(lib.eqa_fft48k5_wgrad3m(V.data_ptr(), G.data_ptr(), D.data_ptr(), M, cin, Cout, st), "eqa_fft48k5_wgrad3m")
        else:
            D = torch.bmm(V.transpose(1, 2), G)
        if k != 5:
            _lib.check(lib.eqa_fft48_filter_grad(D.data_ptr(), dbank.data_ptr(), Cout, cin, k, int(packed), st), "eqa_fft48_filter_grad")
        elif packed:
            _lib.check(lib.eqa_fft48k5_filter_grad3m(D.data_ptr(), dbank.data_ptr(), Cout, cin, st), "eqa_fft48k5_filter_grad3m")
        else:
            _lib.check(lib.eqa_fft48k5_filter_grad(D.data_ptr(), dbank.data_ptr(), Cout, cin, st), "eqa_fft48k5_filter_grad")
    return dbank


def filter_grad(V: torch.Tensor, dy: torch.Tensor, cin: int, G: Optional[torch.Tensor] = None) -> torch.Tensor:
    return filter_grad_k(V, dy, cin, 5, G)


def input_grad(dy: torch.Tensor, bank: torch.Tensor, G: Optional[torch.Tensor] = None) -> torch.Tensor:
    k = bank.shape[-1]
    nimg, Cout, OH, OW = dy.shape
    Cin = bank.shape[1]
    dev = dy.device
    if G is None:
        G = grad_spectra(dy, k)
    B2 = spectra_for_k(bank.detach().permute(1, 0, 2, 3).contiguous(), correlate=False)
    st = ops._stream()
    H, W = OH + k - 1, OW + k - 1
    dx = torch.empty((nimg, Cin, H, W), dtype=torch.float32, device=dev, memory_format=torch.channels_last)
    with torch.cuda.device(dev):
        Cg = contract(G, B2, G.shape[1])
        T2 = _workspace(k, nimg, N * tiles_k(H, k), OW, Cin, dev)
        _transform("input_grad", k, Cg.data_ptr(), T2.data_ptr(), dx.data_ptr(), nimg, H, W, Cin, st)
    return dx


grad_spectra_k, input_grad_k = grad_spectra, input_grad


class ConvKxKFunction(torch.autograd.Function):

    @staticmethod
    def forward(ctx, x, bank):
        keep: list = []
        k = bank.shape[-1]
        y = conv_kxk(x, spectra_for_k(bank.detach()), k, None, False, keep_V=keep)
        ctx.save_for_backward(bank, *keep)
        return y

    @staticmethod
    def backward(ctx, dy):
        bank, V = ctx.saved_tensors
        k = bank.shape[-1]
        dy = dy.contiguous(memory_format=torch.channels_last)
        G = grad_spectra_k(dy, k)
        dx = input_grad_k(dy, bank, G) if ctx.needs_input_grad[0] else None
        dbank = filter_grad_k(V, dy, bank.shape[1], k, G).to(bank.dtype) if ctx.needs_input_grad[1] else None
        return dx, dbank
```

equiadapt_amd/ops.py:

```python
from typing import Optional, Tuple

import torch

from equiadapt_amd import _lib


MAX_WINDOW_K = 10


def _stream() -> int:
    return _raw_stream(_current_device())


try:
    _raw_stream, _current_device = torch._C._cuda_getCurrentRawStream, torch._C._cuda_getDevice
except AttributeError:
    def _raw_stream(_dev):
        return torch.cuda.current_stream().cuda_stream

    def _current_device():
        return 0


class KernelTimer:
# ... 54 lines not shown
    gidx: Optional[torch.Tensor],
    theta: torch.Tensor,
    flags: Optional[torch.Tensor],
    chan_map: Optional[torch.Tensor],
    pad: int,
    out_hw: Tuple[int, int],
    top_left: Tuple[int, int],
    n_out: Optional[int] = None,
) -> torch.Tensor:
    lib = _lib.load()
    src = _need(src, "src")
    theta = _need(theta, "theta")
    B, C, H, W = src.shape
    E = theta.shape[0]
    gidx, p_gidx = _opt(gidx, "gidx", torch.int32)
    flags, p_flags = _opt(flags, "flags", torch.int32)
    chan_map, p_map = _opt(chan_map, "chan_map", torch.int32)
    G = chan_map.shape[1] if chan_map is not None else 1
    if n_out is None:
        n_out = B if gidx is not None else E * B
    OH, OW = out_hw
    dst = torch.empty((n_out, C, OH, OW), dtype=torch.float32, device=src.device)
    with torch.cuda.device(src.device):
        st = lib.eqa_group_action_fwd(src.data_ptr(), dst.data_ptr(), p_gidx, theta.data_ptr(), p_flags, p_map, E, G,
                                      n_out, B, C, H, W, pad, OH, OW, top_left[0], top_left[1], _stream())
    _lib.check(st, "eqa_group_action_fwd")
    return dst


def group_action_bwd(
    src: torch.Tensor,
    grad_out: torch.Tensor,
    gidx: Optional[torch.Tensor],
    theta: torch.Tensor,
    flags: Optional[torch.Tensor],
    chan_map: Optional[torch.Tensor],
    pad: int,
    top_left: Tuple[int, int],
    want_src: bool,
    want_angle: bool,
    want_theta: bool = False,
) -> Tuple[Optional[torch.Tensor], Optional[torch.Tensor]]:
    lib = _lib.load()
    src = _need(src, "src")
    grad_out = _need(grad_out, "grad_out")
    theta = _need(theta, "theta")
    B, C, H, W = src.shape
    n_out, C2, OH, OW = grad_out.shape
    assert C2 == C
    E = theta.shape[0]
    gidx, p_gidx = _opt(gidx, "gidx", torch.int32)
    flags, p_flags = _opt(flags, "flags", torch.int32)
    chan_map, p_map = _opt(chan_map, "chan_map", torch.int32)
    G = chan_map.shape[1] if chan_map is not None else 1
    if want_src and pad > 0 and gidx is not None and n_out == B and chan_map is None and not lib.eqa_get_option(0):
        Hp, Wp = H + 2 * pad, W + 2 * pad
        g_frame = torch.empty((B, C, Hp, Wp), dtype=torch.float32, device=src.device)
        with torch.cuda.device(src.device):
            st = lib.eqa_group_action_bwd(g_frame.data_ptr(), grad_out.data_ptr(), p_gidx, theta.data_ptr(), p_flags, None,
                                          g_frame.data_ptr(), None, E, 1, n_out, B, C, Hp, Wp, 0, OH, OW, top_left[0], top_left[1],
                                          _stream())
            _lib.check(st, "eqa_group_action_bwd (frame gather)")
            g_src = torch.empty_like(src)
            ws = torch.empty((lib.eqa_fold_edge_pad_workspace_bytes(B * C, H, W, pad) // 4,), dtype=torch.float32, device=src.device)
            _lib.check(lib.eqa_fold_edge_pad(g_frame.data_ptr(), g_src.data_ptr(), ws.data_ptr(), B * C, H, W, pad, _stream()),
                       "eqa_fold_edge_pad")
        if not (want_angle or want_theta):
            return g_src, None
        _, g_t = group_action_bwd(src, grad_out, gidx, theta, flags, chan_map, pad, top_left, False, want_angle, want_theta)
        return g_src, g_t
    g_src = torch.zeros_like(src) if want_src else None
    tiles = lib.eqa_group_action_bwd_tiles(OH, OW)
    if want_theta:
        partial = torch.empty((n_out, tiles, 6), dtype=torch.float32, device=src.device)
        with torch.cuda.device(src.device):
            st = lib.eqa_group_action_bwd_theta(src.data_ptr(), grad_out.data_ptr(), p_gidx, theta.data_ptr(), p_flags, p_map,
                                                g_src.data_ptr() if want_src else None, partial.data_ptr(),
                                                E, G, n_out, B, C, H, W, pad, OH, OW, top_left[0], top_left[1], _stream())
        _lib.check(st, "eqa_group_action_bwd_theta")
        return g_src, partial.sum(dim=1)
    partial = torch.empty((n_out, tiles), dtype=torch.float32, device=src.device) if want_angle else None
    with torch.cuda.device(src.device):
        st = lib.eqa_group_action_bwd(src.data_ptr(), grad_out.data_ptr(), p_gidx, theta.data_ptr(), p_flags, p_map,
                                      g_src.data_ptr() if want_src else None, partial.data_ptr() if want_angle else None,
                                      E, G, n_out, B, C, H, W, pad, OH, OW, top_left[0], top_left[1], _stream())
    _lib.check(st, "eqa_group_action_bwd")
    g_angle = partial.sum(dim=1) * (3.141592653589793 / 180.0) if want_angle else None
    return g_src, g_angle


_window_hints: dict = {}


def _hint_key(theta: torch.Tensor):
    return (theta.device.index, theta.data_ptr(), theta.numel())


def register_window_hint(theta: torch.Tensor, max_window_rows: int) -> None:
    import weakref

    key = _hint_key(theta)
    _window_hints[key] = int(max_window_rows)
    weakref.finalize(theta, _window_hints.pop, key, None)


def _window_hint(theta: torch.Tensor, explicit: Optional[int]) -> int:
    return int(explicit) if explicit is not None else _window_hints.get(_hint_key(theta), 0)


def canon_transform(x: torch.Tensor, gidx: torch.Tensor, theta: torch.Tensor, flags: Optional[torch.Tensor], pad: int,
                    max_window: Optional[int] = None) -> torch.Tensor:
    lib = _lib.load()
    x = _need(x, "x")
    gidx = _need(gidx, "gidx", torch.int32)
    theta = _need(theta, "theta")
    flags, p_flags = _opt(flags, "flags", torch.int32)
    B, C, H, W = x.shape
    y = torch.empty_like(x)
    hint = _window_hint(theta, max_window)
    with torch.cuda.device(x.device), _timed("canon_transform"):
        if hint > 0 and B > 0:
            st = lib.eqa_group_action_fwd_hint(x.data_ptr(), y.data_ptr(), gidx.data_ptr(), theta.data_ptr(), p_flags, None,
                                               theta.shape[0], 1, B, B, C, H, W, pad, H, W, pad, pad, hint, _stream())
        else:
            st = lib.eqa_canon_transform_fwd(x.data_ptr(), y.data_ptr(), gidx.data_ptr(), theta.data_ptr(), p_flags,
                                             theta.shape[0], B, C, H, W, pad, _stream())
    _lib.check(st, "eqa_canon_transform_fwd")
    return y


def invert_action(f: torch.Tensor, gidx: torch.Tensor, theta: torch.Tensor, flags: Optional[torch.Tensor],
                  chan_map: Optional[torch.Tensor], max_window: Optional[int] = None) -> torch.Tensor:
    lib = _lib.load()
    f = _need(f, "feature_map")
    gidx = _need(gidx, "gidx", torch.int32)
    theta = _need(theta, "theta")
    flags, p_flags = _opt(flags, "flags", torch.int32)
    chan_map, p_map = _opt(chan_map, "chan_map", torch.int32)
    G = chan_map.shape[1] if chan_map is not None else 1
    B, C, H, W = f.shape
    out = torch.empty_like(f)
    hint = _window_hint(theta, max_window)
    with torch.cuda.device(f.device), _timed("invert_action"):
        if hint > 0 and B > 0:
            st = lib.eqa_group_action_fwd_hint(f.data_ptr(), out.data_ptr(), gidx.data_ptr(), theta.data_ptr(), p_flags, p_map,
                                               theta.shape[0], G, B, B, C, H, W, 0, H, W, 0, 0, hint, _stream())
        else:
            st = lib.eqa_invert_action_fwd(f.data_ptr(), out.data_ptr(), gidx.data_ptr(), theta.data_ptr(), p_flags, p_map,
                                           theta.shape[0], G, B, C, H, W, _stream())
    _lib.check(st, "eqa_invert_action_fwd")
    return out


def group_action_pair(x: torch.Tensor, f: torch.Tensor, gidx: torch.Tensor, theta_canon: torch.Tensor,
                      flags_canon: Optional[torch.Tensor], pad: int, theta_inv: torch.Tensor, flags_inv: Optional[torch.Tensor],
                      chan_map: Optional[torch.Tensor]):
    lib = _lib.load()
    x, f = _need(x, "x"), _need(f, "feature_map")
    gidx = _need(gidx, "gidx", torch.int32)
    theta_canon, theta_inv = _need(theta_canon, "theta_canon"), _need(theta_inv, "theta_inv")
    flags_canon, p_fc = _opt(flags_canon, "flags_canon", torch.int32)
    flags_inv, p_fi = _opt(flags_inv, "flags_inv", torch.int32)
    chan_map, p_map = _opt(chan_map, "chan_map", torch.int32)
    G = chan_map.shape[1] if chan_map is not None else 1
    B, C, H, W = x.shape
    if f.shape[0] != B or tuple(f.shape[2:]) != (H, W) or theta_canon.shape[0] != theta_inv.shape[0]:
        raise ValueError(f"group_action_pair: x {tuple(x.shape)} and f {tuple(f.shape)} must share batch and spatial size, and the tables their element count")
    y, out = torch.empty_like(x), torch.empty_like(f)
    with torch.cuda.device(x.device), _timed("group_action_pair"):
        st = lib.eqa_group_action_pair(x.data_ptr(), y.data_ptr(), theta_canon.data_ptr(), p_fc, pad, C, f.data_ptr(), out.data_ptr(),
                                       theta_inv.data_ptr(), p_fi, p_map, G, f.shape[1], gidx.data_ptr(), theta_canon.shape[0], B, H, W,
                                       _stream())
    _lib.check(st, "eqa_group_action_pair")
    return y, out


def orbit_expand(x: torch.Tensor, theta: torch.Tensor, flags: Optional[torch.Tensor], pad: int) -> torch.Tensor:
    lib = _lib.load()
    x = _need(x, "x")
    theta = _need(theta, "theta")
    flags, p_flags = _opt(flags, "flags", torch.int32)
    B, C, S, S2 = x.shape
    if S != S2:
        raise ValueError("orbit_expand expects square images (the reference crops to a square resize_shape)")
    E = theta.shape[0]
    y = torch.empty((E * B, C, S, S), dtype=torch.float32, device=x.device)
    with torch.cuda.device(x.device):
        st = lib.eqa_orbit_expand_fwd(x.data_ptr(), y.data_ptr(), theta.data_ptr(), p_flags, E, B, C, S, pad, _stream())
    _lib.check(st, "eqa_orbit_expand_fwd")
    return y


def group_pool_argmax(feature_map: torch.Tensor, want_index: bool = True) -> Tuple[torch.Tensor, Optional[torch.Tensor]]:
    lib = _lib.load()
    feature_map = _need(feature_map, "feature_map")
    B, Cf, G, Hf, Wf = feature_map.shape
    HW = Hf * Wf
    act = torch.empty((B, G), dtype=torch.float32, device=feature_map.device)
    gidx = torch.empty((B,), dtype=torch.int32, device=feature_map.device) if want_index else None
    nbytes = lib.eqa_group_pool_workspace_bytes(B, Cf, G, HW)
    ws = torch.empty((max(nbytes, 8) // 8,), dtype=torch.float64, device=feature_map.device)
    with torch.cuda.device(feature_map.device), _timed("group_pool"):
        st = lib.eqa_group_pool_argmax(feature_map.data_ptr(), act.data_ptr(), gidx.data_ptr() if want_index else None,
                                       ws.data_ptr(), B, Cf, G, HW, _stream())
    _lib.check(st, "eqa_group_pool_argmax")
    return act, gidx


def window_sums(x: torch.Tensor, k: int, scale: Optional[torch.Tensor] = None, shift: Optional[torch.Tensor] = None,
                relu: bool = False) -> torch.Tensor:
    lib = _lib.load()
    B, C, H, W = x.shape
    scale, p_scale = _opt(scale, "scale", torch.float32)
    shift, p_shift = _opt(shift, "shift", torch.float32)
    out = torch.empty((B, C, k, k), dtype=torch.float64, device=x.device)
    if (x.is_cuda and x.dtype == torch.float32 and C % 4 == 0 and not x.is_contiguous()
            and x.is_contiguous(memory_format=torch.channels_last) and H > 2 * (k - 1) and W > 2 * (k - 1)):
        ws = torch.empty((max(lib.eqa_window_sums_nhwc_workspace_bytes(B, C, H, k), 4) // 4,), dtype=torch.float32, device=x.device)
        with torch.cuda.device(x.device), _timed("window_sums"):
            st = lib.eqa_window_sums_nhwc(x.data_ptr(), p_scale, p_shift, int(relu), out.data_ptr(), ws.data_ptr(), B, C, H, W, k, _stream())
        _lib.check(st, "eqa_window_sums_nhwc")
        return out
    x = _need(x, "x")
    with torch.cuda.device(x.device), _timed("window_sums"):
        st = lib.eqa_window_sums(x.data_ptr(), p_scale, p_shift, int(relu), out.data_ptr(), B, C, H, W, k, _stream())
    _lib.check(st, "eqa_window_sums")
    return out


def group_argmax(act: torch.Tensor) -> torch.Tensor:
    lib = _lib.load()
    act = _need(act.detach(), "group_activations")
    B, G = act.shape
    gidx = torch.empty((B,), dtype=torch.int32, device=act.device)
    with torch.cuda.device(act.device):
        st = lib.eqa_group_argmax(act.data_ptr(), gidx.data_ptr(), B, G, _stream())
    _lib.check(st, "eqa_group_argmax")
    return gidx


def so3_rotate(x: torch.Tensor, R: torch.Tensor, transpose: bool = False) -> torch.Tensor:
    lib = _lib.load()
    x = _need(x, "x")
    R = _need(R, "R")
    B, three, N = x.shape
    if three != 3 or tuple(R.shape) != (B, 3, 3):
        raise ValueError("so3_rotate expects x:(B,3,N) and R:(B,3,3)")
    y = torch.empty_like(x)
    with torch.cuda.device(x.device):
        st = lib.eqa_so3_rotate(x.data_ptr(), R.data_ptr(), y.data_ptr(), B, N, int(transpose), _stream())
    _lib.check(st, "eqa_so3_rotate")
    return y


def gram_schmidt(v: torch.Tensor) -> torch.Tensor:
    lib = _lib.load()
    v = _need(v, "vectors")
    if v.dim() != 3 or v.shape[1:] != (3, 3):
        raise ValueError("gram_schmidt expects (B,3,3)")
    out = torch.empty_like(v)
    with torch.cuda.device(v.device):
        st = lib.eqa_gram_schmidt(v.data_ptr(), out.data_ptr(), v.shape[0], _stream())
    _lib.check(st, "eqa_gram_schmidt")
    return out


def vnsmall_forward(x: torch.Tensor, params: torch.Tensor, k: int = 20, pooling: str = "mean") -> torch.Tensor:
    lib = _lib.load()
    x = _need(x, "point_cloud")
    params = _need(params, "params")
    B, three, N = x.shape
    if pooling not in ("mean", "max"):
        raise ValueError(f"Pooling type {pooling} not supported")
    if three != 3 or params.numel() != (1310 if pooling == "mean" else 1751):
        raise ValueError("vnsmall_forward expects x:(B,3,N) and 1310 (mean) / 1751 (max) packed parameters")
    out = torch.empty((B, 3, 3), dtype=torch.float32, device=x.device)
    ws = torch.empty((max(lib.eqa_vnsmall_workspace_bytes(B, N), 4) // 4,), dtype=torch.float32, device=x.device)
    with torch.cuda.device(x.device), _timed("vnsmall_fwd"):
        st = lib.eqa_vnsmall_fwd(x.data_ptr(), params.data_ptr(), out.data_ptr(), ws.data_ptr(), B, N, k, int(pooling == "max"), _stream())
    _lib.check(st, "eqa_vnsmall_fwd")
    return out


def vnsmall_canonicalize(x: torch.Tensor, params: torch.Tensor, k: int = 20, pooling: str = "mean"):
    lib = _lib.load()
    x = _need(x, "point_cloud")
    params = _need(params, "params")
    B, three, N = x.shape
    if pooling not in ("mean", "max"):
        raise ValueError(f"Pooling type {pooling} not supported")
    if three != 3 or params.numel() != (1310 if pooling == "mean" else 1751):
        raise ValueError("vnsmall_canonicalize expects x:(B,3,N) and 1310 (mean) / 1751 (max) packed parameters")
    vec = torch.empty((B, 3, 3), dtype=torch.float32, device=x.device)
    R = torch.empty((B, 3, 3), dtype=torch.float32, device=x.device)
    y = torch.empty_like(x)
    ws = torch.empty((max(lib.eqa_vnsmall_workspace_bytes(B, N), 4) // 4,), dtype=torch.float32, device=x.device)
    with torch.cuda.device(x.device), _timed("vnsmall_fwd"):
        st = lib.eqa_vnsmall_canonicalize(x.data_ptr(), params.data_ptr(), vec.data_ptr(), R.data_ptr(), y.data_ptr(), ws.data_ptr(),
                                          B, N, k, int(pooling == "max"), _stream())
    _lib.check(st, "eqa_vnsmall_canonicalize")
    return vec, R, y


def crop_resize_aa(x: torch.Tensor, tables, out_hw: Tuple[int, int]) -> torch.Tensor:
    lib = _lib.load()
    x = _need(x, "x")
    wx, x0, wy, y0, K, max_rows, x_begin, x_span = tables
    B, C, H, W = x.shape
    y = torch.empty((B, C, out_hw[0], out_hw[1]), dtype=torch.float32, device=x.device)
    with torch.cuda.device(x.device), _timed("crop_resize_aa"):
        st = lib.eqa_crop_resize_aa(x.data_ptr(), y.data_ptr(), wx.data_ptr(), x0.data_ptr(), wy.data_ptr(), y0.data_ptr(),
                                    B * C, H, W, out_hw[0], out_hw[1], K, max_rows, x_begin, x_span, _stream())
    _lib.check(st, "eqa_crop_resize_aa")
    return y


def mask_action_nearest(masks: torch.Tensor, eidx: torch.Tensor, rtheta: torch.Tensor, flags: Optional[torch.Tensor]) -> torch.Tensor:
    lib = _lib.load()
    masks = _need(masks, "masks", torch.uint8)
    eidx = _need(eidx, "eidx", torch.int32)
    rtheta = _need(rtheta, "rtheta")
    flags, p_flags = _opt(flags, "flags", torch.int32)
    n, H, W = masks.shape
    out = torch.empty_like(masks)
    with torch.cuda.device(masks.device), _timed("mask_action"):
        st = lib.eqa_mask_action_nearest(masks.data_ptr(), out.data_ptr(), eidx.data_ptr(), rtheta.data_ptr(), p_flags,
                                         rtheta.shape[0], n, H, W, _stream())
    _lib.check(st, "eqa_mask_action_nearest")
    return out


_plane_tables: dict = {}


def mask_action_nearest_planes(mask_list, eidx: torch.Tensor, rtheta: torch.Tensor, flags: Optional[torch.Tensor]) -> torch.Tensor:
    lib = _lib.load()
    eidx = _need(eidx, "eidx", torch.int32)
    rtheta = _need(rtheta, "rtheta")
    flags, p_flags = _opt(flags, "flags", torch.int32)
    masks = [_need(m, "masks", torch.uint8) for m in mask_list]
    H, W = masks[0].shape[-2:]
    ptrs = tuple(m.data_ptr() + k * H * W for m in masks for k in range(m.shape[0]))
    n = len(ptrs)
    dev = masks[0].device
    key = (ptrs, str(dev))
    table = _plane_tables.get(key)
    if table is None:
        if len(_plane_tables) >= 64:
            _plane_tables.clear()
        table = torch.tensor(ptrs, dtype=torch.int64).to(dev)
        _plane_tables[key] = table
    out = torch.empty((n, H, W), dtype=torch.uint8, device=dev)
    with torch.cuda.device(dev), _timed("mask_action"):
        st = lib.eqa_mask_action_nearest_planes(table.data_ptr(), out.data_ptr(), eidx.data_ptr(), rtheta.data_ptr(), p_flags,
                                                rtheta.shape[0], n, H, W, _stream())
    _lib.check(st, "eqa_mask_action_nearest_planes")
    return out


def boxes_action(boxes: torch.Tensor, img_of_box: torch.Tensor, rotation_deg: torch.Tensor, width: float,
                 flip_all: bool) -> Tuple[torch.Tensor, Optional[torch.Tensor]]:
    lib = _lib.load()
    boxes = _need(boxes, "boxes")
    img_of_box = _need(img_of_box, "img_of_box", torch.int32)
    rotation_deg = _need(rotation_deg, "rotation_deg")
    out = torch.empty_like(boxes)
    flipped = torch.empty_like(boxes) if flip_all else None
    with torch.cuda.device(boxes.device):
        st = lib.eqa_boxes_action(boxes.data_ptr(), img_of_box.data_ptr(), rotation_deg.data_ptr(),
                                  flipped.data_ptr() if flip_all else None, out.data_ptr(), boxes.shape[0], float(width),
                                  int(flip_all), _stream())
    _lib.check(st, "eqa_boxes_action")
    return out, flipped


def conv_s2_supported(cin: int, cout: int, k: int, pad: int, planar: bool) -> bool:
    return bool(_lib.load().eqa_conv_s2_supported(cin, cout, k, pad, int(planar)))


def pack_conv_s2_weights(w: torch.Tensor, planar: bool) -> torch.Tensor:
    Cout, Cin, K, _ = w.shape
    if planar:
        wp = torch.zeros(Cout, 4, K, K, dtype=w.dtype, device=w.device)
        wp[:, :Cin] = w
        return wp.permute(2, 3, 1, 0).reshape(K * K, 4, Cout // 16, 16).permute(0, 2, 1, 3).contiguous()
    t = w.permute(2, 3, 1, 0).reshape(K * K, Cin // 16, 4, 4, Cout // 16, 16)
    return t.permute(0, 1, 4, 2, 5, 3).contiguous()


def conv_s2(x: torch.Tensor, wp: torch.Tensor, bias: Optional[torch.Tensor], gelu: bool, cout: int, k: int, pad: int,
            planar: bool) -> torch.Tensor:
    lib = _lib.load()
    x, wp = _need(x, "x"), _need(wp, "wp")
    bias, p_bias = _opt(bias, "bias", torch.float32)
    if planar:
        B, cin, H, W = x.shape
    else:
        B, H, W, cin = x.shape
    OH, OW = (H + 2 * pad - k) // 2 + 1, (W + 2 * pad - k) // 2 + 1
    y = torch.empty((B, OH, OW, cout), dtype=torch.float32, device=x.device)
    with torch.cuda.device(x.device), _timed("conv_s2"):
        st = lib.eqa_conv_s2(x.data_ptr(), wp.data_ptr(), p_bias, int(gelu), y.data_ptr(), B, cin, H, W, cout, k, pad, int(planar), _stream())
    _lib.check(st, "eqa_conv_s2")
    return y


def pack_conv_s2_dgrad_weights(w: torch.Tensor) -> torch.Tensor:
    Cout, Cin, K, _ = w.shape
    t = w.permute(2, 3, 0, 1).reshape(K * K, Cout // 16, 4, 4, Cin // 16, 16)
    return t.permute(0, 1, 4, 2, 5, 3).contiguous()


def conv_s2_train_supported(cin: int, cout: int, k: int, pad: int, planar: bool) -> bool:
    lib = _lib.load()
    return bool(lib.eqa_conv_s2_wgrad_supported(cin, cout, k, pad, int(planar))) and (planar or bool(lib.eqa_conv_s2_dgrad_supported(cin, cout, k, pad)))


def conv_s2_wgrad(x: torch.Tensor, dz: torch.Tensor, k: int, pad: int, planar: bool) -> torch.Tensor:
    lib = _lib.load()
    x, dz = _need(x, "x"), _need(dz, "dz")
    if planar:
        B, cin, H, W = x.shape
    else:
        B, H, W, cin = x.shape
    cout = dz.shape[-1]
    dw = torch.empty((cout, cin, k, k), dtype=torch.float32, device=x.device)
    ws = torch.empty((max(lib.eqa_conv_s2_wgrad_workspace_bytes(B, cin, H, W, cout, k, pad, int(planar)), 16) // 4,), dtype=torch.float32, device=x.device)
    with torch.cuda.device(x.device), _timed("conv_s2_wgrad"):
        st = lib.eqa_conv_s2_wgrad(x.data_ptr(), dz.data_ptr(), dw.data_ptr(), ws.data_ptr(), B, cin, H, W, cout, k, pad, int(planar), _stream())
    _lib.check(st, "eqa_conv_s2_wgrad")
    return dw


def conv_s2_dgrad(dz: torch.Tensor, wd: torch.Tensor, in_hw: Tuple[int, int], cin: int, k: int, pad: int) -> torch.Tensor:
    lib = _lib.load()
    dz, wd = _need(dz, "dz"), _need(wd, "wd")
    B, cout = dz.shape[0], dz.shape[-1]
    dx = torch.empty((B, in_hw[0], in_hw[1], cin), dtype=torch.float32, device=dz.device)
    with torch.cuda.device(dz.device), _timed("conv_s2_dgrad"):
        st = lib.eqa_conv_s2_dgrad(dz.data_ptr(), wd.data_ptr(), dx.data_ptr(), B, cin, in_hw[0], in_hw[1], cout, k, pad, _stream())
    _lib.check(st, "eqa_conv_s2_dgrad")
    return dx


def _bn_act_partials(z: torch.Tensor) -> torch.Tensor:
    lib = _lib.load()
    npix, C = z.shape
    part = torch.empty((max(lib.eqa_bn_act_partial_blocks(npix), 1), C, 2), dtype=torch.float64, device=z.device)
    with torch.cuda.device(z.device), _timed("bn_act_stats"):
        st = lib.eqa_bn_act_stats(z.data_ptr(), part.data_ptr(), npix, C, _stream())
    _lib.check(st, "eqa_bn_act_stats")
    return part


def bn_batch_stats(z: torch.Tensor):
    z = _need(z, "z")
    sums = _bn_act_partials(z).sum(0)
    mean = sums[:, 0] / z.shape[0]
    var = (sums[:, 1] / z.shape[0] - mean * mean).clamp_min(0.0)
    return mean, var


def bn_fold_batch_stats(z: torch.Tensor, bn: torch.nn.modules.batchnorm._BatchNorm):
    from equiadapt_amd.common.utils import mark_written

    lib = _lib.load()
    z = _need(z, "z")
    npix, C = z.shape
    part = _bn_act_partials(z)
    out = torch.empty((4, C), dtype=torch.float32, device=z.device)
    track = bn.track_running_stats and bn.running_mean is not None
    momentum = 0.0
    if track:
        with torch.no_grad():
            bn.num_batches_tracked += 1
        momentum = bn.momentum if bn.momentum is not None else 1.0 / float(bn.num_batches_tracked)
    with torch.cuda.device(z.device):
        st = lib.eqa_bn_act_finalize(part.data_ptr(), npix, C, bn.weight.data_ptr(), bn.bias.data_ptr(), float(bn.eps), float(momentum),
                                     bn.running_mean.data_ptr() if track else None, bn.running_var.data_ptr() if track else None,
                                     out[0].data_ptr(), out[1].data_ptr(), out[2].data_ptr(), out[3].data_ptr(), _stream())
    _lib.check(st, "eqa_bn_act_finalize")
    if track:
        mark_written(bn.running_mean, bn.running_var)
    return out[0], out[1], out[2], out[3]


def bn_act_fwd(z: torch.Tensor, scale: torch.Tensor, shift: torch.Tensor, rowscale: Optional[torch.Tensor], act: int) -> torch.Tensor:
    lib = _lib.load()
    z, scale, shift = _need(z, "z"), _need(scale, "scale"), _need(shift, "shift")
    rowscale, p_rs = _opt(rowscale, "rowscale", torch.float32)
    npix, C = z.shape
    y = torch.empty_like(z)
    with torch.cuda.device(z.device), _timed("bn_act_fwd"):
        st = lib.eqa_bn_act_fwd(z.data_ptr(), scale.data_ptr(), shift.data_ptr(), p_rs, y.data_ptr(), npix, C, act, _stream())
    _lib.check(st, "eqa_bn_act_fwd")
    return y


def bn_act_bwd(gy: torch.Tensor, z: torch.Tensor, scale: torch.Tensor, shift: torch.Tensor, mean: torch.Tensor, rstd: torch.Tensor,
               gamma: torch.Tensor, rowscale: Optional[torch.Tensor], act: int):
    lib = _lib.load()
    gy, z = _need(gy, "gy"), _need(z, "z")
    rowscale, p_rs = _opt(rowscale, "rowscale", torch.float32)
    npix, C = z.shape
    part = torch.empty((max(lib.eqa_bn_act_partial_blocks(npix), 1), C, 2), dtype=torch.float64, device=z.device)
    with torch.cuda.device(z.device), _timed("bn_act_bwd_reduce"):
        st = lib.eqa_bn_act_bwd_reduce(gy.data_ptr(), z.data_ptr(), scale.data_ptr(), shift.data_ptr(), mean.data_ptr(), rstd.data_ptr(), p_rs,
                                       part.data_ptr(), npix, C, act, _stream())
    _lib.check(st, "eqa_bn_act_bwd_reduce")
    coef = torch.empty((5, C), dtype=torch.float32, device=z.device)
    with torch.cuda.device(z.device):
        st = lib.eqa_bn_act_bwd_finalize(part.data_ptr(), npix, C, gamma.data_ptr(), rstd.data_ptr(), coef[0].data_ptr(), coef[1].data_ptr(),
                                         coef[2].data_ptr(), coef[3].data_ptr(), coef[4].data_ptr(), _stream())
    _lib.check(st, "eqa_bn_act_bwd_finalize")
    dgamma, dbeta, gscale, m1, m2 = coef[0], coef[1], coef[2], coef[3], coef[4]
    dz = torch.empty_like(z)
    with torch.cuda.device(z.device), _timed("bn_act_bwd_apply"):
        st = lib.eqa_bn_act_bwd_apply(gy.data_ptr(), z.data_ptr(), scale.data_ptr(), shift.data_ptr(), mean.data_ptr(), rstd.data_ptr(), p_rs,
                                      gscale.data_ptr(), m1.data_ptr(), m2.data_ptr(), dz.data_ptr(), npix, C, act, _stream())
    _lib.check(st, "eqa_bn_act_bwd_apply")
    return dz, dgamma, dbeta


def affine_relu_rows(h: torch.Tensor, scale: torch.Tensor, shift: torch.Tensor) -> torch.Tensor:
    lib = _lib.load()
    h, scale, shift = _need(h, "h"), _need(scale, "scale"), _need(shift, "shift")
    rows, D = h.shape
    z = torch.empty_like(h)
    with torch.cuda.device(h.device):
        st = lib.eqa_affine_relu_rows(h.data_ptr(), scale.data_ptr(), shift.data_ptr(), z.data_ptr(), rows, D, _stream())
    _lib.check(st, "eqa_affine_relu_rows")
    return z


def cosine_group_activations(v: torch.Tensor, ref: torch.Tensor, num_group: int, eps: float = 1e-8) -> torch.Tensor:
    lib = _lib.load()
    v, ref = _need(v, "vector_out"), _need(ref.reshape(-1), "reference_vector")
    R, V = v.shape
    if R % num_group or ref.numel() != V:
        raise ValueError("cosine_group_activations expects (G*B, V) embeddings and a (V) reference vector")
    B = R // num_group
    act = torch.empty((B, num_group), dtype=torch.float32, device=v.device)
    with torch.cuda.device(v.device):
        st = lib.eqa_cosine_group_activations(v.data_ptr(), ref.data_ptr(), act.data_ptr(), B, num_group, V, float(eps), _stream())
    _lib.check(st, "eqa_cosine_group_activations")
    return act


def bias_relu_nhwc_(x: torch.Tensor, bias: torch.Tensor) -> torch.Tensor:
    lib = _lib.load()
    if not (x.is_cuda and x.dtype == torch.float32 and x.is_contiguous(memory_format=torch.channels_last)):
        raise RuntimeError("bias_relu_nhwc_ expects a channels-last fp32 tensor on the device")
    bias = _need(bias, "bias")
    B, C, H, W = x.shape
    with torch.cuda.device(x.device), _timed("bias_relu"):
        st = lib.eqa_bias_relu_nhwc(x.data_ptr(), bias.data_ptr(), B * H * W, C, _stream())
    _lib.check(st, "eqa_bias_relu_nhwc")
    return x


def window_sums_gemv(S: torch.Tensor, weff: torch.Tensor, scale: float, shift) -> torch.Tensor:
    lib = _lib.load()
    S = _need(S, "S", torch.float64)
    weff = _need(weff, "weff", torch.float64)
    B, K = S.shape
    E = weff.shape[0]
    act = torch.empty((B, E), dtype=torch.float32, device=S.device)
    sh = shift if isinstance(shift, float) else 0.0
    with torch.cuda.device(S.device), _timed("sums_gemv"):
        st = lib.eqa_window_sums_gemv(S.data_ptr(), weff.data_ptr(), act.data_ptr(), B, K, E, float(scale), sh, _stream())
    _lib.check(st, "eqa_window_sums_gemv")
    if not isinstance(shift, float):
        act += shift.to(torch.float32)
    return act


def window_sums_gemv_bwd(dact: torch.Tensor, weff: torch.Tensor, S: torch.Tensor, scale: float, need_dS: bool, need_dW: bool):
    lib = _lib.load()
    dact = _need(dact, "dact")
    weff, S = _need(weff, "weff", torch.float64), _need(S, "S", torch.float64)
    B, K = S.shape
    E = weff.shape[0]
    dS = torch.empty_like(S) if need_dS else None
    dW = torch.empty_like(weff) if need_dW else None
    ws = torch.empty((max(lib.eqa_window_sums_gemv_bwd_workspace_bytes(K, E), 8) // 8,), dtype=torch.float64, device=S.device) if need_dW else None
    with torch.cuda.device(S.device), _timed("sums_gemv_bwd"):
        st = lib.eqa_window_sums_gemv_bwd(dact.data_ptr(), weff.data_ptr(), S.data_ptr(), dS.data_ptr() if need_dS else None,
                                          dW.data_ptr() if need_dW else None, ws.data_ptr() if need_dW else None, B, K, E, float(scale), _stream())
    _lib.check(st, "eqa_window_sums_gemv_bwd")
    return dS, dW


def window_grad_table(dS: torch.Tensor, H: int, W: int) -> torch.Tensor:
    lib = _lib.load()
    dS = _need(dS, "dS", torch.float64)
    B, C, k, _ = dS.shape
    T = 2 * (k - 1) + 1
    table = torch.empty((B, T, T, C), dtype=torch.float32, device=dS.device)
    with torch.cuda.device(dS.device), _timed("window_grad_table"):
        st = lib.eqa_window_grad_table(dS.data_ptr(), table.data_ptr(), B, C, H, W, k, _stream())
    _lib.check(st, "eqa_window_grad_table")
    return table


def plane_gemm_supported(cin: int, cout: int) -> bool:
    return bool(_lib.load().eqa_plane_gemm_supported(cin, cout))


def pack_plane_gemm_weights(U: torch.Tensor) -> torch.Tensor:
    P, Cin, Cout = U.shape
    t = U.float().reshape(P, Cin // 16, 2, 2, 4, Cout // 32, 32)
    return t.permute(0, 1, 5, 2, 3, 6, 4).contiguous()


def plane_gemm(V: torch.Tensor, Upk: torch.Tensor, M: torch.Tensor, tiles: int) -> None:
    lib = _lib.load()
    V, Upk, M = _need(V, "V"), _need(Upk, "Upk"), _need(M, "M")
# ... 342 lines not shown
```

include/eqa_hip.h:

```cpp
#ifndef EQA_HIP_H
#define EQA_HIP_H

#include <stdint.h>

#ifdef __cplusplus
extern "C" {
#endif

#define EQA_OK 0
#define EQA_ERR_INVALID_ARG (-1)
#define EQA_ERR_LAUNCH (-2)
#define EQA_ERR_UNSUPPORTED (-3)

#define EQA_FLIP_SRC 1
#define EQA_FLIP_DST 2

#define EQA_ABI_VERSION 3
int eqa_abi_version(void);

int eqa_set_option(int key, int value);
int eqa_get_option(int key);

int eqa_canon_transform_fwd(const float* x, float* y, const int32_t* gidx, const float* theta,
                            const int32_t* flags, int num_elements, int B, int C, int H, int W, int pad,
                            void* stream);

int eqa_invert_action_fwd(const float* f, float* out, const int32_t* gidx, const float* theta,
                          const int32_t* flags, const int32_t* chan_map, int num_elements, int G, int B, int C,
                          int H, int W, void* stream);

int eqa_group_action_pair(const float* x, float* y, const float* theta_canon, const int32_t* flags_canon, int pad, int C,
                          const float* f, float* out, const float* theta_inv, const int32_t* flags_inv,
                          const int32_t* chan_map, int G, int Cf, const int32_t* gidx, int num_elements, int B, int H,
                          int W, void* stream);

int eqa_orbit_expand_fwd(const float* x, float* y, const float* theta, const int32_t* flags, int num_elements,
                         int B, int C, int S, int pad, void* stream);

int eqa_group_action_fwd(const float* src, float* dst, const int32_t* gidx, const float* theta,
                         const int32_t* flags, const int32_t* chan_map, int num_elements, int G, int n_out,
                         int B, int C, int H, int W, int pad, int OH, int OW, int top, int left, void* stream);
int eqa_group_action_fwd_hint(const float* src, float* dst, const int32_t* gidx, const float* theta, const int32_t* flags,
                              const int32_t* chan_map, int num_elements, int G, int n_out, int B, int C, int H, int W,
                              int pad, int OH, int OW, int top, int left, int max_window, void* stream);

int eqa_crop_resize_aa(const float* x, float* y, const float* wx, const int32_t* x0, const float* wy, const int32_t* y0,
                       int planes, int H, int W, int OH, int OW, int K, int max_rows, int x_begin, int x_span, void* stream);

int eqa_mask_action_nearest(const uint8_t* m, uint8_t* out, const int32_t* eidx, const float* rtheta, const int32_t* flags,
                            int num_elements, int n_masks, int H, int W, void* stream);
int eqa_mask_action_nearest_planes(const uint8_t* const* planes, uint8_t* out, const int32_t* eidx, const float* rtheta,
                                   const int32_t* flags, int num_elements, int n_masks, int H, int W, void* stream);

int eqa_boxes_action(const float* boxes, const int32_t* img_of_box, const float* rotation_deg, float* flipped, float* out,
                     int n, float width, int flip_all, void* stream);

int eqa_image_action_nearest(const float* x, float* out, const int32_t* eidx, const float* rtheta, const int32_t* flags,
                             int num_elements, int n_planes, int src_mod, int H, int W, int pad, int OH, int OW, int top,
                             int left, void* stream);

int64_t eqa_fold_edge_pad_workspace_bytes(int planes, int H, int W, int pad);
int eqa_fold_edge_pad(const float* gframe, float* gsrc, void* workspace, int planes, int H, int W, int pad, void* stream);
int eqa_group_action_bwd_tiles(int OH, int OW);
int eqa_group_action_bwd(const float* src, const float* grad_out, const int32_t* gidx, const float* theta,
                         const int32_t* flags, const int32_t* chan_map, float* grad_src, float* grad_angle_partial,
                         int num_elements, int G, int n_out, int B, int C, int H, int W, int pad, int OH, int OW,
                         int top, int left, void* stream);
int eqa_group_action_bwd_theta(const float* src, const float* grad_out, const int32_t* gidx, const float* theta,
                               const int32_t* flags, const int32_t* chan_map, float* grad_src, float* grad_theta_partial,
                               int num_elements, int G, int n_out, int B, int C, int H, int W, int pad, int OH, int OW,
                               int top, int left, void* stream);

int64_t eqa_group_pool_workspace_bytes(int B, int Cf, int G, int HW);
int eqa_group_pool_argmax(const float* feat, float* act, int32_t* gidx, void* workspace, int B, int Cf, int G,
                          int HW, void* stream);

int eqa_window_sums(const float* x, const float* scale, const float* shift, int relu, double* out, int B, int C, int H,
                    int W, int k, void* stream);

int eqa_conv_s2_supported(int Cin, int Cout, int K, int pad, int planar);
int eqa_conv_s2(const float* x, const float* wp, const float* bias, int gelu, float* y, int B, int Cin, int H, int W, int Cout, int K,
                int pad, int planar, void* stream);
int eqa_conv_s2_wgrad_supported(int Cin, int Cout, int K, int pad, int planar);
int64_t eqa_conv_s2_wgrad_workspace_bytes(int B, int Cin, int H, int W, int Cout, int K, int pad, int planar);
int eqa_conv_s2_wgrad(const float* x, const float* dz, float* dw, void* workspace, int B, int Cin, int H, int W, int Cout, int K, int pad,
                      int planar, void* stream);
int eqa_conv_s2_dgrad_supported(int Cin, int Cout, int K, int pad);
int eqa_conv_s2_dgrad(const float* dz, const float* wd, float* dx, int B, int Cin, int H, int W, int Cout, int K, int pad, void* stream);
int eqa_bn_act_fwd(const float* z, const float* scale, const float* shift, const float* rowscale, float* y, int64_t npix, int C, int act,
                   void* stream);
int64_t eqa_bn_act_partial_blocks(int64_t npix);
int eqa_bn_act_stats(const float* z, double* partial, int64_t npix, int C, void* stream);
int eqa_bn_act_finalize(const double* partial, int64_t npix, int C, const float* gamma, const float* beta, double eps, double momentum,
                        float* running_mean, float* running_var, float* scale, float* shift, float* mean, float* rstd, void* stream);
int eqa_bn_act_bwd_finalize(const double* partial, int64_t npix, int C, const float* gamma, const float* rstd, float* dgamma, float* dbeta,
                            float* gscale, float* m1, float* m2, void* stream);
int eqa_bn_act_bwd_reduce(const float* gy, const float* z, const float* scale, const float* shift, const float* mean, const float* rstd,
                          const float* rowscale, double* partial, int64_t npix, int C, int act, void* stream);
int eqa_bn_act_bwd_apply(const float* gy, const float* z, const float* scale, const float* shift, const float* mean, const float* rstd,
                         const float* rowscale, const float* gscale, const float* m1, const float* m2, float* dz, int64_t npix, int C,
                         int act, void* stream);
int eqa_affine_relu_rows(const float* h, const float* scale, const float* shift, float* z, int64_t rows, int D, void* stream);
int eqa_cosine_group_activations(const float* v, const float* ref, float* act, int B, int G, int V, float eps, void* stream);
int eqa_window_grad_table(const double* dS, float* table, int B, int C, int H, int W, int k, void* stream);
int64_t eqa_window_sums_gemv_bwd_workspace_bytes(int K, int E);
int eqa_window_sums_gemv_bwd(const float* dact, const double* Wm, const double* S, double* dS, double* dWm, void* workspace, int B, int K,
                             int E, double scale, void* stream);
int eqa_bias_relu_nhwc(float* x, const float* bias, int64_t n_pixels, int C, void* stream);
int64_t eqa_window_sums_nhwc_workspace_bytes(int B, int C, int H, int k);
int eqa_window_sums_nhwc(const float* x, const float* scale, const float* shift, int relu, double* out, void* workspace,
                         int B, int C, int H, int W, int k, void* stream);
int eqa_window_sums_bwd_expand_nhwc(const float* table, float* dx, int B, int H, int W, int C, int k, void* stream);

int64_t eqa_bn_partial_blocks(int64_t n_pixels);
int eqa_bn_stats_nhwc(const float* x, double* partial, int64_t n_pixels, int C, void* stream);
int eqa_bn_relu_dropout_nhwc(const float* x, const float* scale, const float* shift, float* y, int64_t n_pixels, int C,
                             float drop_p, uint32_t seed, void* stream);
int eqa_bn_bwd_reduce_nhwc(const float* gy, const float* y, const float* x, const float* mean, const float* rstd, float drop_p,
                           double* partial, int64_t n_pixels, int C, const float* scale, const float* shift, uint32_t seed,
                           void* stream);
int eqa_bn_bwd_apply_nhwc(const float* gy, const float* y, const float* x, const float* mean, const float* rstd, const float* a,
                          const float* b, const float* d, float drop_p, float* dx, int64_t n_pixels, int C, const float* scale,
                          const float* shift, uint32_t seed, void* stream);
int eqa_window_sums_nhwc_act(const float* x, const float* scale, const float* shift, int relu, float drop_p, uint32_t seed, double* out,
                             void* workspace, int B, int C, int H, int W, int k, void* stream);
int eqa_bn_bwd_reduce_nhwc_wsgrad(const float* table, const float* x, const float* mean, const float* rstd, float drop_p,
                                  double* partial, int B, int H, int W, int C, int k, const float* scale, const float* shift,
                                  uint32_t seed, void* stream);
int eqa_bn_bwd_apply_nhwc_wsgrad(const float* table, const float* x, const float* mean, const float* rstd, const float* a,
                                 const float* b, const float* d, float drop_p, float* dx, int B, int H, int W, int C, int k,
                                 const float* scale, const float* shift, uint32_t seed, void* stream);

int eqa_window_sums_gemv(const double* S, const double* Wm, float* act, int B, int K, int E, double scale, double shift,
                         void* stream);

int eqa_lift_conv_nhwc(const float* x, const float* wpk, const float* bias, int relu, float* y, int nimg, int H, int W,
                       int Cin, int KH, int KW, int Cout, void* stream);
int eqa_lift_conv_grouped(const float* x, const float* wpk, const float* bias, int relu, float* y, int nimg, int H, int W, int Cin,
                          int KH, int KW, int Cout, void* stream);
int eqa_lift_conv_wide_supported(int Cin, int KH, int KW, int Cout);
int64_t eqa_lift_conv_wide_weight_floats(int Cin, int KH, int KW, int Cout);
int eqa_lift_conv_wide(const float* x, const float* wpk, const float* bias, int relu, float* y, int nimg, int H, int W, int Cin,
                       int KH, int KW, int Cout, void* stream);
int64_t eqa_lift_conv_wide_wgrad_workspace_bytes(int Cin, int KH, int KW, int Cout);
int eqa_lift_conv_wide_wgrad(const float* x, const float* dy, void* workspace, float* dbank, int nimg, int H, int W, int Cin, int KH,
                             int KW, int Cout, void* stream);
int eqa_lift_conv_stats_rows(int nimg, int H, int W, int Cin, int KH, int KW, int Cout);
int eqa_lift_conv_nhwc_stats(const float* x, const float* wpk, float* y, double* partial, int nimg, int H, int W, int Cin, int KH,
                             int KW, int Cout, void* stream);

int eqa_lift_conv_wgrad_supported(int nimg, int H, int W, int Cin, int Cout, int KH, int KW);
int64_t eqa_lift_conv_wgrad_workspace_bytes(int nimg, int H, int W, int Cin, int Cout, int KH, int KW);
int eqa_lift_conv_wgrad_nhwc(const float* x, const float* dy, void* workspace, float* dbank, int nimg, int H, int W, int Cin,
                             int Cout, int KH, int KW, void* stream);

int eqa_plane_gemm_supported(int Cin, int Cout);
int eqa_plane_gemm(const float* V, const float* Upk, float* M, long long T, int P, int Cin, int Cout, void* stream);

int eqa_winograd_f2k5_input(const float* x, float* V, const float* in_bias, int in_relu, int nimg, int H, int W, int C,
                            void* stream);
int eqa_winograd_f2k5_output(const float* M, const float* bias, int relu, float* y, int nimg, int OH, int OW, int C,
                             void* stream);
int eqa_winograd_f4k5_input(const float* x, float* V, const float* in_bias, int in_relu, int nimg, int H, int W, int C,
                            void* stream);
int eqa_winograd_f4k5_output(const float* M, const float* bias, int relu, float* y, int nimg, int OH, int OW, int C,
                             void* stream);
int eqa_winograd_f2k5_input_padded(const float* x, float* V, int nimg, int H, int W, int C, int pad, void* stream);
int eqa_winograd_f4k5_input_padded(const float* x, float* V, int nimg, int H, int W, int C, int pad, void* stream);
int eqa_winograd_f2k5_output_adjoint(const float* dY, float* dM, int nimg, int OH, int OW, int C, void* stream);
int eqa_winograd_f4k5_output_adjoint(const float* dY, float* dM, int nimg, int OH, int OW, int C, void* stream);
int64_t eqa_winograd_f2k5_output_sums_workspace_bytes(int nimg, int OH, int C, int k_next);
int eqa_winograd_f2k5_output_sums(const float* M, const float* bias, int relu, double* S, void* workspace, int nimg,
                                  int OH, int OW, int C, int k_next, void* stream);
int eqa_winograd_f4k5_output_sums(const float* M, const float* bias, int relu, double* S, void* workspace, int nimg,
                                  int OH, int OW, int C, int k_next, void* stream);

int64_t eqa_fft48k5_tiles(int n);
int64_t eqa_fft48k5_tile_pitch(int64_t tiles);
int eqa_fft48k5_frequencies(void);
int eqa_fft48k5_filter_spectra(const float* bank, float* B, int Cout, int Cin, int correlate, void* stream);
int eqa_fft48k5_cgemm3m_supported(int Cin, int Cout);
int64_t eqa_fft48k5_spectra3m_floats(int Cin, int Cout);
int eqa_fft48k5_filter_spectra3m(const float* bank, float* B3, int Cout, int Cin, int correlate, void* stream);
int eqa_fft48k5_cgemm3m(const float* V, const float* B3, float* Mo, int64_t M, int Cin, int Cout, void* stream);
int64_t eqa_fft48k5_spectra3m_bf16_bytes(int Cin, int Cout);
int eqa_fft48k5_spectra3m_split(const float* B3, void* Bp, int Cin, int Cout, void* stream);
int eqa_fft48k5_cgemm3m_bf16x3(const float* V, const void* Bp, float* Mo, int64_t M, int Cin, int Cout, int terms, void* stream);
int64_t eqa_fft48k5_spectra3m_f16_bytes(int Cin, int Cout);
int eqa_fft48k5_spectra3m_split_f16(const float* B3, void* Bh, int Cin, int Cout, float b_scale, void* stream);
int eqa_fft48k5_cgemm3m_f16x2(const float* V, const void* Bh, float* Mo, int64_t M, int Cin, int Cout, const float* vbound, int nbound,
                              float b_scale, void* stream);
int eqa_fft48k5_wgrad3m_supported(int Cin, int Cout);
int eqa_fft48k5_wgrad3m(const float* V, const float* G, float* D, int64_t M, int Cin, int Cout, void* stream);
int eqa_fft48k5_filter_grad3m(const float* D, float* dbank, int Cout, int Cin, void* stream);
int eqa_fft48k5_group(int C, int side);
int64_t eqa_fft48k5_workspace_bytes(int nimg, int rows, int out_cols, int C);
int eqa_fft48k5_input(const float* x, float* T, float* V, const float* in_bias, int in_relu, int nimg, int H, int W, int C,
                      void* stream);
int eqa_fft48k5_input_grouped_supported(int C);
int eqa_fft48k5_input_grouped(const float* x, float* T, float* V, const float* in_bias, int in_relu, int nimg, int H, int W, int C,
                              void* stream);
int eqa_lift5_fft48k5_input_supported(int Cin, int KH, int KW, int Cout);
int eqa_lift5_fft48k5_input(const float* x, const float* bank, const float* bias, int relu, float* V, int nimg, int H0, int W0, int Cout,
                            void* stream);
#define EQA_LIFT5_DCMAX_SLOTS 256
int eqa_lift5_fft48k5_input_dcmax(const float* x, const float* bank, const float* bias, int relu, float* V, float* dcmax, int nimg, int H0,
                                  int W0, int Cout, void* stream);
int64_t eqa_lift5_pieces_f16_bytes(int Cout);
int eqa_absmax_slots(const float* x, int64_t n, float* slots, void* stream);
int eqa_lift5_fft48k5_input_f16x2(const float* x, const void* wpieces, float w_scale, const float* xbound, int nxbound, const float* bias,
                                  int relu, float* V, float* dcmax, int nimg, int H0, int W0, int Cout, void* stream);
int64_t eqa_lift5_pieces_bytes(int Cout);
int eqa_lift5_fft48k5_input_bf16x3(const float* x, const void* wpieces, const float* bias, int relu, float* V, int nimg, int H0, int W0,
                                   int Cout, void* stream);
int eqa_fft48k5_output(const float* Mo, float* T2, const float* bias, int relu, float* y, int nimg, int OH, int OW, int C,
                       void* stream);
int64_t eqa_fft48k5_output_stats_rows(int nimg, int OH, int OW, int C);
int eqa_fft48k5_output_stats(const float* Mo, float* T2, float* y, double* partial, int nimg, int OH, int OW, int C, void* stream);
int eqa_fft48k5_grad_transform(const float* dy, float* T, float* G, int nimg, int OH, int OW, int C, void* stream);
int eqa_fft48k5_filter_grad(const float* D, float* dbank, int Cout, int Cin, void* stream);
int eqa_fft48k5_input_grad(const float* Cg, float* T2, float* dx, int nimg, int H, int W, int C, void* stream);
int eqa_fft48k5_output_sums(const float* Mo, float* T2, const float* bias, int relu, double* S, void* workspace, int nimg,
                            int OH, int OW, int C, int k_next, void* stream);

int eqa_fft48_supported(int ksize);
int64_t eqa_fft48_tiles(int n, int ksize);
int64_t eqa_fft48_workspace_bytes(int nimg, int rows, int out_cols, int C, int ksize);
int eqa_fft48_filter_spectra(const float* bank, float* B, int Cout, int Cin, int ksize, int correlate, void* stream);
int eqa_fft48_filter_spectra3m(const float* bank, float* B3, int Cout, int Cin, int ksize, int correlate, void* stream);
int eqa_fft48_input(const float* x, float* T, float* V, const float* in_bias, int in_relu, int nimg, int H, int W, int C, int ksize,
                    void* stream);
int eqa_fft48_grad_transform(const float* dy, float* T, float* G, int nimg, int OH, int OW, int C, int ksize, void* stream);
int eqa_fft48_output(const float* Mo, float* T2, const float* bias, int relu, float* y, int nimg, int OH, int OW, int C, int ksize,
                     void* stream);
int eqa_fft48_input_grad(const float* Cg, float* T2, float* dx, int nimg, int H, int W, int C, int ksize, void* stream);
int eqa_fft48_filter_grad(const float* D, float* dbank, int Cout, int Cin, int ksize, int packed, void* stream);

int eqa_group_argmax(const float* act, int32_t* gidx, int B, int G, void* stream);

int eqa_so3_rotate(const float* x, const float* R, float* y, int B, int N, int transpose, void* stream);

#define EQA_VNSMALL_PARAMS 1310
#define EQA_VNSMALL_PARAMS_MAX 1751
int64_t eqa_vnsmall_workspace_bytes(int B, int N);
int eqa_vnsmall_fwd(const float* x, const float* params, float* out, void* workspace, int B, int N, int k, int pooling,
                    void* stream);
int eqa_vnsmall_canonicalize(const float* x, const float* params, float* vectors, float* R, float* y, void* workspace, int B, int N,
                             int k, int pooling, void* stream);

int eqa_vn_blocks(int N);
int eqa_vn_knn(const float* x, int32_t* idx, int B, int N, int k, void* stream);
int eqa_vn_convpos_stats(const float* x, const int32_t* idx, const float* Wf, float* partial, int B, int N, int k, void* stream);
int eqa_vn_convpos_fwd(const float* x, const int32_t* idx, const float* Wf, const float* Wd, const float* scale, const float* shift,
                       float* pooled, int B, int N, int k, void* stream);
int eqa_vn_convpos_bwd_reduce(const float* x, const int32_t* idx, const float* Wf, const float* Wd, const float* scale,
                              const float* shift, const float* mean, const float* rstd, const float* gpool, float* partial, int B,
                              int N, int k, void* stream);
int eqa_vn_convpos_bwd_apply(const float* x, const int32_t* idx, const float* Wf, const float* Wd, const float* scale,
                             const float* shift, const float* mean, const float* rstd, const float* m1, const float* m2,
                             const float* gpool, float* partial, int B, int N, int k, void* stream);

int eqa_vn_convpos_max_fwd(const float* x, const int32_t* idx, const float* Wf, const float* Wd, const float* scale,
                           const float* shift, const float* Wp, float* pooled, uint8_t* sel, int B, int N, int k, void* stream);
int eqa_vn_convpos_max_bwd_reduce(const float* x, const int32_t* idx, const float* Wf, const float* Wd, const float* scale,
                                  const float* shift, const float* mean, const float* rstd, const float* gpool,
                                  const uint8_t* sel, float* partial, int B, int N, int k, void* stream);
int eqa_vn_convpos_max_bwd_apply(const float* x, const int32_t* idx, const float* Wf, const float* Wd, const float* scale,
                                 const float* shift, const float* mean, const float* rstd, const float* m1, const float* m2,
                                 const float* gpool, const uint8_t* sel, float* partial, int B, int N, int k, void* stream);

int eqa_vn_tail_blocks(int N);
int eqa_vn_tail_partial_floats(int pass);
int eqa_vn_tail_pass(int pass, const float* pooled, const float* weights, const float* stat, const float* red, const float* mask,
                     const float* gout, float* partial, float* g_pooled, int B, int N, void* stream);
int eqa_vn_bn_finalize(const float* partial, int nblk, int stride, int C, long long M, const float* gamma, const float* beta,
                       float* running_mean, float* running_var, long long* num_batches_tracked, float momentum, float eps, float* stat,
                       void* stream);
int eqa_vn_bn_bwd_finalize(const float* partial, int nblk, int stride, int C, long long M, float* grads, float* red, void* stream);

int eqa_gram_schmidt(const float* v, float* out, int B, void* stream);
int eqa_gram_schmidt_bwd(const float* v, const float* grad_out, float* grad_v, int B, void* stream);

int eqa_modified_gram_schmidt(const float* v, float* out, int B, void* stream);
int eqa_rigid_rows(const float* x, const float* R, const float* t, float* out, int M, int mode, void* stream);

int eqa_fourier_elu_fwd(const float* x, const float* scale, const float* shift, float* y, long long npix, int fields, void* stream);
int eqa_fourier_elu_bwd(const float* x, const float* scale, const float* shift, const float* dy, float* dx, long long npix, int fields,
                        void* stream);

int eqa_vndeepsets_param_count(int H, int L, int features);
int eqa_vndeepsets_bwd_blocks(int S);
int eqa_nbody_adjacency(const int64_t* rows, const int64_t* cols, long long E, int S, int32_t* adj, int32_t* flag, void* stream);
int eqa_vndeepsets_fwd(const float* loc, const float* vel, const float* charges, const int32_t* adj, const float* params, float* rot,
                       float* trans, int S, int H, int L, int features, int softplus, float slope, int layer_mean, int final_mean,
                       int canon_translation, void* stream);
int eqa_vndeepsets_train_fwd(const float* loc, const float* vel, const float* charges, const int32_t* adj, const float* params,
                             const float* mask, float* saved, float* rot, float* trans, int S, int H, int L, int features,
                             int softplus, float slope, int layer_mean, int final_mean, int canon_translation, void* stream);
int eqa_vndeepsets_bwd(const float* loc, const float* vel, const float* charges, const int32_t* adj, const float* params,
                       const float* mask, const float* saved, const float* grad_rot, const float* grad_trans, float* partial, int S,
                       int H, int L, int features, int softplus, float slope, int layer_mean, int final_mean, int canon_translation,
                       void* stream);

#ifdef __cplusplus
}
#endif
#endif
```

Before: 72240 images/s.

## Emit channels-last resize output with fused absmax bound for lift FFT input

The antialiased crop-resize kernels gain an NHWC variant that writes channels-last output directly, packing all channels of a pixel in one store. Each block also computes a per-block absolute maximum into slots. The lift FFT layer reuses those slots instead of launching a separate absmax reduction. When the canonicalization network's first layer reads channels-last input, this removes a layout conversion and a reduction pass, at the cost of more template variants, an extra block-level reduction, and a tensor-attached cache keyed by data pointer and version.

```diff
diff --git a/equiadapt_amd/_lib.py b/equiadapt_amd/_lib.py
--- a/equiadapt_amd/_lib.py
+++ b/equiadapt_amd/_lib.py
@@ -31,6 +31,8 @@
     "eqa_group_action_fwd": (_int, [_vp, _vp, _vp, _vp, _vp, _vp] + [_int] * 12 + [_vp]),
     "eqa_group_action_fwd_hint": (_int, [_vp, _vp, _vp, _vp, _vp, _vp] + [_int] * 13 + [_vp]),
     "eqa_crop_resize_aa": (_int, [_vp] * 6 + [_int] * 9 + [_vp]),
+    "eqa_crop_resize_aa_nhwc_bound_slots": (_int, [_vp] + [_int] * 10),
+    "eqa_crop_resize_aa_nhwc_bound": (_int, [_vp] * 6 + [_int] * 10 + [_vp, _int, _vp]),
     "eqa_mask_action_nearest": (_int, [_vp] * 5 + [_int] * 4 + [_vp]),
     "eqa_mask_action_nearest_planes": (_int, [_vp] * 5 + [_int] * 4 + [_vp]),
     "eqa_boxes_action": (_int, [_vp] * 5 + [_int, ctypes.c_float, _int, _vp]),
diff --git a/equiadapt_amd/csrc/crop_resize.hip b/equiadapt_amd/csrc/crop_resize.hip
--- a/equiadapt_amd/csrc/crop_resize.hip
+++ b/equiadapt_amd/csrc/crop_resize.hip
@@ -8,10 +8,37 @@
 #endif
 constexpr int kAaMaxK = 20;
 
+template <bool NHWC>
+__device__ __forceinline__ float* aa_plane_dst(float* y, int plane, int OH, int OW, int cpi, int& stride) {
+  if constexpr (NHWC) {
+    stride = cpi;
+    return y + (size_t)(plane / cpi) * OH * OW * cpi + plane % cpi;
+  } else {
+    stride = 1;
+    return y + (size_t)plane * OH * OW;
+  }
+}
+__device__ __forceinline__ void aa_block_absmax(float m, float* __restrict__ slots) {
+  __shared__ float red[kThreads / 64];
+#pragma unroll
+  for (int o = 32; o > 0; o >>= 1) m = fmaxf(m, __shfl_xor(m, o));
+  if ((threadIdx.x & 63) == 0) red[threadIdx.x >> 6] = m;
+  __syncthreads();
+  static_assert(kThreads == 256, "four waves");
+  if (threadIdx.x == 0)
+    slots[((size_t)blockIdx.z * gridDim.y + blockIdx.y) * gridDim.x + blockIdx.x] = fmaxf(fmaxf(red[0], red[1]), fmaxf(red[2], red[3]));
+}
+struct __attribute__((packed, aligned(4))) aa_px2 { float v[2]; };
+struct __attribute__((packed, aligned(4))) aa_px3 { float v[3]; };
+constexpr int kAaNhwcMaxC = 3;
+constexpr int kAaNhwcPix = 6;
+
+template <bool NHWC>
 __global__ __launch_bounds__(kThreads) void crop_resize_aa_kernel(const float* __restrict__ x, float* __restrict__ y,
                                                                  const float* __restrict__ wx, const int32_t* __restrict__ x0,
                                                                  const float* __restrict__ wy, const int32_t* __restrict__ y0,
-                                                                 int H, int W, int OH, int OW, int K, int max_rows) {
+                                                                 int H, int W, int OH, int OW, int K, int max_rows, int cpi,
+                                                                 float* __restrict__ slots) {
   extern __shared__ __attribute__((aligned(16))) float aa_tmp[];
   const int plane = blockIdx.y;
   const int r0 = blockIdx.x * kAaBand, r1 = min(r0 + kAaBand, OH);
@@ -56,7 +83,9 @@
     }
   }
   __syncthreads();
-  float* dst = y + (size_t)plane * OH * OW;
+  int dstride;
+  float* dst = aa_plane_dst<NHWC>(y, plane, OH, OW, cpi, dstride);
+  float amax = 0.0f;
   for (int idx = threadIdx.x; idx < (r1 - r0) * OW; idx += kThreads) {
     const int r = idx / OW, ox = idx - r * OW;
     const int oy = r0 + r;
@@ -66,18 +95,21 @@
 #pragma unroll
     for (int j = 0; j < EQA_AA_WIDE_MIN_K; ++j)
       if (j < K) acc += wy[oy * K + j] * aa_tmp[min(ys + j, nrows - 1) * OW + ox];
-    dst[(size_t)oy * OW + ox] = acc;
-  }
-}
-
-
-template <int K, int BAND, int NL>
-__global__ __launch_bounds__(kThreads, (NL > 5 && K > 5) ? 2 : 4) void crop_resize_aa_staged_kernel(
+    dst[((size_t)oy * OW + ox) * dstride] = acc;
+    if constexpr (NHWC) amax = fmaxf(amax, fabsf(acc));
+  }
+  if constexpr (NHWC) aa_block_absmax(amax, slots);
+}
+
+constexpr int kAaNhwcMinBlocks = 3;
+template <int K, int BAND, int NL, bool NHWC>
+__global__ __launch_bounds__(kThreads, (NL > 5 && K > 5) ? 2 : (NHWC ? kAaNhwcMinBlocks : 4)) void crop_resize_aa_staged_kernel(
     const float* __restrict__ x, float* __restrict__ y,
                                                                         const float* __restrict__ wx, const int32_t* __restrict__ x0,
                                                                         const float* __restrict__ wy, const int32_t* __restrict__ y0,
-                                                                        int planes, int H, int W, int OH, int OW, int cap_rows,
-                                                                        int xb, int xl) {
+                                                                        int items, int H, int W, int OH, int OW, int cap_rows,
+                                                                        int xb, int xl, int cpi, float* __restrict__ slots) {
+  constexpr int CMAX = NHWC ? kAaNhwcMaxC : 1, PMAX = NHWC ? kAaNhwcPix : 1;
   extern __shared__ __attribute__((aligned(16))) float aa_tmp[];
   float* rows = aa_tmp;
   float* tmp = aa_tmp + (size_t)cap_rows * xl;
@@ -85,7 +117,7 @@
   int* taby = reinterpret_cast<int*>(tabw + BAND * K);
   const int r0 = blockIdx.y * BAND, r1 = min(r0 + BAND, OH);
   const int nband = r1 - r0;
-  const int plane0 = (int)(blockIdx.z * kXcd + blockIdx.x), plane_step = (int)(gridDim.z * kXcd);
+  const int item0 = (int)(blockIdx.z * kXcd + blockIdx.x), item_step = (int)(gridDim.z * kXcd);
   const int rows_par = kThreads / OW;
   const int ox = rows_par >= 1 ? threadIdx.x % OW : 0, rsub = rows_par >= 1 ? threadIdx.x / OW : 0;
   const int xs_g = x0[ox];
@@ -115,70 +147,115 @@
       v[k] = *reinterpret_cast<const aa_f4*>(src_ + (size_t)min(tr + 4 * k, nrows - 1) * W + 4 * min(tq, nq - 1));     \
   } while (0)
   __builtin_amdgcn_s_waitcnt(0x0070);
-  if (prefetch && plane0 < planes) EQA_AA_PF_LOAD(plane0);
-  for (int plane = plane0; plane < planes; plane += plane_step) {
-    if (prefetch) {
-      if (tq < nq) {
-#pragma unroll
-        for (int k = 0; k < NL; ++k)
-          if (tr + 4 * k < nrows) *reinterpret_cast<aa_f4*>(rows + (tr + 4 * k) * xl + 4 * tq) = v[k];
-      }
-      if (plane + plane_step < planes) EQA_AA_PF_LOAD(plane + plane_step);
-    } else {
-      const float* src = src0 + (size_t)plane * plane_sz;
-      for (int q = tq; q < nq; q += 64)
-        for (int rb = tr; rb < nrows; rb += 4) *reinterpret_cast<aa_f4*>(rows + rb * xl + 4 * q) = *reinterpret_cast<const aa_f4*>(src + (size_t)rb * W + 4 * q);
-    }
-    __syncthreads();
-    if (rows_par >= 1) {
-      if (rsub < rows_par) {
-        for (int ry0 = rsub; ry0 < nrows; ry0 += 4 * rows_par) {
-          float acc[4] = {0.0f, 0.0f, 0.0f, 0.0f};
-#pragma unroll
-          for (int u = 0; u < 4; ++u) {
-            const float* row = rows + min(ry0 + u * rows_par, nrows - 1) * xl;
+  if (prefetch && item0 < items) EQA_AA_PF_LOAD(NHWC ? item0 * cpi : item0);
+  float amax = 0.0f;
+  for (int item = item0; item < items; item += item_step) {
+    float outv[PMAX][CMAX];
+    for (int c = 0; c < (NHWC ? cpi : 1); ++c) {
+      const int plane = NHWC ? item * cpi + c : item;
+      const bool last_of_item = !NHWC || c + 1 == cpi;
+      const bool more = !last_of_item || item + item_step < items;
+      const int next = !last_of_item ? plane + 1 : (NHWC ? (item + item_step) * cpi : item + item_step);
+      if (prefetch) {
+        if (tq < nq) {
+#pragma unroll
+          for (int k = 0; k < NL; ++k)
+            if (tr + 4 * k < nrows) *reinterpret_cast<aa_f4*>(rows + (tr + 4 * k) * xl + 4 * tq) = v[k];
+        }
+        if (more) EQA_AA_PF_LOAD(next);
+      } else {
+        const float* src = src0 + (size_t)plane * plane_sz;
+        for (int q = tq; q < nq; q += 64)
+          for (int rb = tr; rb < nrows; rb += 4) *reinterpret_cast<aa_f4*>(rows + rb * xl + 4 * q) = *reinterpret_cast<const aa_f4*>(src + (size_t)rb * W + 4 * q);
+      }
+      __syncthreads();
+      if (rows_par >= 1) {
+        if (rsub < rows_par) {
+          for (int ry0 = rsub; ry0 < nrows; ry0 += 4 * rows_par) {
+            float acc[4] = {0.0f, 0.0f, 0.0f, 0.0f};
+#pragma unroll
+            for (int u = 0; u < 4; ++u) {
+              const float* row = rows + min(ry0 + u * rows_par, nrows - 1) * xl;
+#pragma unroll
+              for (int j = 0; j < K; ++j)
+                acc[u] += wv[j] * row[xo[j]];
+            }
+#pragma unroll
+            for (int u = 0; u < 4; ++u)
+              if (ry0 + u * rows_par < nrows) tmp[(ry0 + u * rows_par) * OW + ox] = acc[u];
+          }
+        }
+      } else {
+        for (int idx = threadIdx.x; idx < nrows * OW; idx += kThreads) {
+          const int ry = idx / OW, oxx = idx - ry * OW;
+          const float* row = rows + ry * xl;
+          const int xs = x0[oxx] - xb;
+          float acc = 0.0f;
+#pragma unroll
+          for (int j = 0; j < K; ++j)
+            acc += wx[oxx * K + j] * row[min(xs + j, xl - 1)];
+          tmp[ry * OW + oxx] = acc;
+        }
+      }
+      __syncthreads();
+      if constexpr (NHWC) {
+#pragma unroll
+        for (int p = 0; p < PMAX; ++p) {
+          const int idx = (int)threadIdx.x + p * kThreads;
+          float acc = 0.0f;
+          if (idx < nband * OW) {
+            const int r = idx / OW, oxx = idx - r * OW;
+            const int ys = taby[r];
 #pragma unroll
             for (int j = 0; j < K; ++j)
-              acc[u] += wv[j] * row[xo[j]];
+              acc += tabw[r * K + j] * tmp[min(ys + j, nrows - 1) * OW + oxx];
           }
 #pragma unroll
-          for (int u = 0; u < 4; ++u)
-            if (ry0 + u * rows_par < nrows) tmp[(ry0 + u * rows_par) * OW + ox] = acc[u];
-        }
-      }
-    } else {
-      for (int idx = threadIdx.x; idx < nrows * OW; idx += kThreads) {
-        const int ry = idx / OW, oxx = idx - ry * OW;
-        const float* row = rows + ry * xl;
-        const int xs = x0[oxx] - xb;
-        float acc = 0.0f;
-#pragma unroll
-        for (int j = 0; j < K; ++j)
-          acc += wx[oxx * K + j] * row[min(xs + j, xl - 1)];
-        tmp[ry * OW + oxx] = acc;
-      }
-    }
-    __syncthreads();
-    float* dst = y + (size_t)plane * OH * OW;
-    for (int idx = threadIdx.x; idx < nband * OW; idx += kThreads) {
-      const int r = idx / OW, oxx = idx - r * OW;
-      const int ys = taby[r];
-      float acc = 0.0f;
-#pragma unroll
-      for (int j = 0; j < K; ++j)
-        acc += tabw[r * K + j] * tmp[min(ys + j, nrows - 1) * OW + oxx];
-      dst[(size_t)(r0 + r) * OW + oxx] = acc;
-    }
-    __syncthreads();
-  }
+          for (int q = CMAX - 1; q > 0; --q) outv[p][q] = outv[p][q - 1];
+          outv[p][0] = acc;
+        }
+      } else {
+        float* dst = y + (size_t)plane * OH * OW;
+        for (int idx = threadIdx.x; idx < nband * OW; idx += kThreads) {
+          const int r = idx / OW, oxx = idx - r * OW;
+          const int ys = taby[r];
+          float acc = 0.0f;
+#pragma unroll
+          for (int j = 0; j < K; ++j)
+            acc += tabw[r * K + j] * tmp[min(ys + j, nrows - 1) * OW + oxx];
+          dst[(size_t)(r0 + r) * OW + oxx] = acc;
+        }
+      }
+      __syncthreads();
+    }
+    if constexpr (NHWC) {
+      float* dst = y + ((size_t)item * OH + r0) * OW * cpi;
+#pragma unroll
+      for (int p = 0; p < PMAX; ++p) {
+        const int idx = (int)threadIdx.x + p * kThreads;
+        if (idx < nband * OW) {
+          float* d = dst + (size_t)idx * cpi;
+          if (cpi == 3) *reinterpret_cast<aa_px3*>(d) = aa_px3{{outv[p][2], outv[p][1], outv[p][0]}};
+          else if (cpi == 2) *reinterpret_cast<aa_px2*>(d) = aa_px2{{outv[p][1], outv[p][0]}};
+          else d[0] = outv[p][0];
+#pragma unroll
+          for (int c = 0; c < CMAX; ++c)
+            if (c < cpi) amax = fmaxf(amax, fabsf(outv[p][c]));
+        }
+      }
+    }
+  }
+  if constexpr (NHWC) aa_block_absmax(amax, slots);
 #undef EQA_AA_PF_LOAD
 }
 
+template <bool NHWC>
 __global__ __launch_bounds__(kThreads) void crop_resize_aa_wide_kernel(const float* __restrict__ x, float* __restrict__ y,
                                                                       const float* __restrict__ wx, const int32_t* __restrict__ x0,
                                                                       const float* __restrict__ wy, const int32_t* __restrict__ y0,
                                                                       int H, int W, int OH, int OW, int K, int max_rows, int xbeg,
-                                                                      int xlen, int pad_shift, int row_stride, int rpi) {
+                                                                      int xlen, int pad_shift, int row_stride, int rpi, int cpi,
+                                                                      float* __restrict__ slots) {
   extern __shared__ __attribute__((aligned(16))) float aa_tmp[];
   float* rowbuf = aa_tmp + (size_t)max_rows * OW;
   const int plane = blockIdx.y;
@@ -261,23 +338,28 @@
     }
     __syncthreads();
   }
-  float* dst = y + (size_t)plane * OH * OW;
+  int dstride;
+  float* dst = aa_plane_dst<NHWC>(y, plane, OH, OW, cpi, dstride);
+  float amax = 0.0f;
   for (int idx = threadIdx.x; idx < (r1 - r0) * OW; idx += kThreads) {
     const int r = idx / OW, ox = idx - r * OW;
     const int oy = r0 + r;
     const int ys = y0[oy] - ybeg;
     float acc = 0.0f;
     for (int j = 0; j < K; ++j) acc += wy[oy * K + j] * aa_tmp[min(ys + j, nrows - 1) * OW + ox];
-    dst[(size_t)oy * OW + ox] = acc;
-  }
+    dst[((size_t)oy * OW + ox) * dstride] = acc;
+    if constexpr (NHWC) amax = fmaxf(amax, fabsf(acc));
+  }
+  if constexpr (NHWC) aa_block_absmax(amax, slots);
 }
 
 constexpr int kAaStreamRows = 8;
+template <bool NHWC>
 __global__ __launch_bounds__(kThreads) void crop_resize_aa_stream_kernel(const float* __restrict__ x, float* __restrict__ y,
                                                                         const float* __restrict__ wx, const int32_t* __restrict__ x0,
                                                                         const float* __restrict__ wy, const int32_t* __restrict__ y0,
                                                                         int H, int W, int OH, int OW, int K, int xbeg, int xlen,
-                                                                        int pad_shift, int row_stride) {
+                                                                        int pad_shift, int row_stride, int cpi, float* __restrict__ slots) {
   extern __shared__ __attribute__((aligned(16))) float aa_rows[];
   const int plane = blockIdx.y;
   const int r0 = blockIdx.x * kAaBand, nr_out = min(kAaBand, OH - r0);
@@ -327,7 +409,9 @@
     if (yc + 2 * kAaStreamRows < span) { load8(va, yc + 2 * kAaStreamRows); wa = wload(yc + 2 * kAaStreamRows); }
     if (yc + kAaStreamRows < span) add8(vb, wb);
   }
-  float* dst = y + (size_t)plane * OH * OW;
+  int dstride;
+  float* dst = aa_plane_dst<NHWC>(y, plane, OH, OW, cpi, dstride);
+  float amax = 0.0f;
 #pragma unroll
   for (int half = 0; half < 2; ++half) {
     if (e < xlen) {
@@ -347,24 +431,31 @@
         const int xs = x0[ox] - xbeg;
         float a = 0.0f;
         for (int j = 0; j < K; ++j) a += wx[ox * K + j] * row[pos(min(xs + j, xlen - 1))];
-        dst[(size_t)(r0 + r) * OW + ox] = a;
+        dst[((size_t)(r0 + r) * OW + ox) * dstride] = a;
+        if constexpr (NHWC) amax = fmaxf(amax, fabsf(a));
       }
     }
     __syncthreads();
   }
-}
-
-}
-
-extern "C" {
-
-int eqa_crop_resize_aa(const float* x, float* y, const float* wx, const int32_t* x0, const float* wy, const int32_t* y0,
-                       int planes, int H, int W, int OH, int OW, int K, int max_rows, int x_begin, int x_span, void* stream) {
-  if (!x || !y || !wx || !x0 || !wy || !y0 || planes < 0 || H <= 0 || W <= 0 || OH <= 0 || OW <= 0 || K <= 0 || max_rows <= 0)
-    return EQA_ERR_INVALID_ARG;
+  if constexpr (NHWC) aa_block_absmax(amax, slots);
+}
+
+constexpr int kAaNhwcMaxSlots = 4096;
+template <bool NHWC>
+static int aa_launch(const float* x, float* y, const float* wx, const int32_t* x0, const float* wy, const int32_t* y0, int planes, int cpi,
+                     int H, int W, int OH, int OW, int K, int max_rows, int x_begin, int x_span, float* slots, int* nslots,
+                     bool count_only, void* stream) {
   const size_t lds = (size_t)max_rows * OW * sizeof(float);
   if (lds > 96 * 1024 || planes > 65535) return EQA_ERR_UNSUPPORTED;
-  if (planes == 0) return EQA_OK;
+  auto slots_ok = [&](const dim3& g, int& status) {
+    if constexpr (!NHWC) return true;
+    const size_t n = (size_t)g.x * g.y * g.z;
+    if (n > (size_t)kAaNhwcMaxSlots) { status = EQA_ERR_UNSUPPORTED; return false; }
+    if (count_only) { *nslots = (int)n; status = EQA_OK; return false; }
+    if (*nslots != (int)n) { status = EQA_ERR_INVALID_ARG; return false; }
+    return true;
+  };
+  int status = EQA_OK;
   const dim3 grid((OH + kAaBand - 1) / kAaBand, planes);
   if (K > EQA_AA_WIDE_MIN_K && x_span > 0 && x_begin >= 0 && x_begin + x_span <= W) {
     const int stride = (x_span + OW / 2) / OW;
@@ -376,13 +467,15 @@
     static const bool stream_off = [] { const char* e = getenv("EQA_AA_STREAM"); return e && e[0] == '0'; }();
     if (!stream_off && x_span <= 4 * kThreads && (x_span & 3) == 0 && (x_begin & 3) == 0 && (W & 3) == 0 && (((uintptr_t)x) & 15) == 0 &&
         (size_t)(kAaBand / 2) * row_bytes <= 64 * 1024) {
-      hipLaunchKernelGGL(crop_resize_aa_stream_kernel, grid, dim3(kThreads), (kAaBand / 2) * row_bytes, (hipStream_t)stream, x, y, wx, x0, wy,
-                         y0, H, W, OH, OW, K, x_begin, x_span, pad_shift, row_stride);
+      if (!slots_ok(grid, status)) return status;
+      hipLaunchKernelGGL(crop_resize_aa_stream_kernel<NHWC>, grid, dim3(kThreads), (kAaBand / 2) * row_bytes, (hipStream_t)stream, x, y, wx, x0, wy,
+                         y0, H, W, OH, OW, K, x_begin, x_span, pad_shift, row_stride, cpi, slots);
       return launch_status();
     }
     if (rpi >= 1) {
-      hipLaunchKernelGGL(crop_resize_aa_wide_kernel, grid, dim3(kThreads), lds2, (hipStream_t)stream, x, y, wx, x0, wy, y0, H, W, OH,
-                         OW, K, max_rows, x_begin, x_span, pad_shift, row_stride, rpi);
+      if (!slots_ok(grid, status)) return status;
+      hipLaunchKernelGGL(crop_resize_aa_wide_kernel<NHWC>, grid, dim3(kThreads), lds2, (hipStream_t)stream, x, y, wx, x0, wy, y0, H, W, OH,
+                         OW, K, max_rows, x_begin, x_span, pad_shift, row_stride, rpi, cpi, slots);
       return launch_status();
     }
   }
@@ -394,24 +487,30 @@
     int band = band_env == 16 ? 16 : (band_env == 8 ? 8 : (OH >= 64 ? 16 : 8));
     auto staged_lds = [&](int bnd) { return ((size_t)(bnd / kAaBand) * max_rows * (xl + OW) + bnd * (EQA_AA_WIDE_MIN_K + 1)) * sizeof(float); };
     if (band == 16 && band_env != 16 && (staged_lds(16) > 64 * 1024 || 16 * K > kThreads)) band = 8;
+    if (NHWC && band == 16 && 16 * OW > kAaNhwcPix * kThreads) band = 8;
     const int cap_rows = (band / kAaBand) * max_rows;
     const size_t lds3 = staged_lds(band);
     if (lds3 <= 64 * 1024 && band * K <= kThreads) {
+      if (NHWC && (cpi > kAaNhwcMaxC || band * OW > kAaNhwcPix * kThreads)) return EQA_ERR_UNSUPPORTED;
       static const int per_cu = [] { const char* e = getenv("EQA_AA_BLOCKS_PER_CU"); return e ? std::max(1, atoi(e)) : 12; }();
+      static const int per_cu_nhwc = [] { const char* e = getenv("EQA_AA_NHWC_BLOCKS_PER_CU"); return e ? std::max(1, atoi(e)) : 3; }();
       const int nbands = (OH + band - 1) / band;
-      const int groups = std::max(1, (std::min(planes, (256 * per_cu + nbands - 1) / nbands) + kXcd - 1) / kXcd);
+      const int items = NHWC ? planes / cpi : planes;
+      const int groups = std::max(1, (std::min(items, (256 * (NHWC ? per_cu_nhwc : per_cu) + nbands - 1) / nbands) + kXcd - 1) / kXcd);
       const bool few = cap_rows <= 20;
+      if (K < 1 || K > EQA_AA_WIDE_MIN_K) return EQA_ERR_UNSUPPORTED;
+      if (!slots_ok(dim3(kXcd, nbands, groups), status)) return status;
 #define EQA_AA_STAGED(K_)                                                                                                              \
   case K_:                                                                                                                             \
     if (band == 16)                                                                                                                    \
-      hipLaunchKernelGGL((crop_resize_aa_staged_kernel<K_, 16, 10>), dim3(kXcd, nbands, groups), dim3(kThreads), lds3, (hipStream_t)stream, x, \
-                         y, wx, x0, wy, y0, planes, H, W, OH, OW, cap_rows, xb, xl);                                                   \
+      hipLaunchKernelGGL((crop_resize_aa_staged_kernel<K_, 16, 10, NHWC>), dim3(kXcd, nbands, groups), dim3(kThreads), lds3, (hipStream_t)stream, x, \
+                         y, wx, x0, wy, y0, items, H, W, OH, OW, cap_rows, xb, xl, cpi, slots);                                        \
     else if (few)                                                                                                                      \
-      hipLaunchKernelGGL((crop_resize_aa_staged_kernel<K_, 8, 5>), dim3(kXcd, nbands, groups), dim3(kThreads), lds3, (hipStream_t)stream, x,  \
-                         y, wx, x0, wy, y0, planes, H, W, OH, OW, cap_rows, xb, xl);                                                   \
+      hipLaunchKernelGGL((crop_resize_aa_staged_kernel<K_, 8, 5, NHWC>), dim3(kXcd, nbands, groups), dim3(kThreads), lds3, (hipStream_t)stream, x,  \
+                         y, wx, x0, wy, y0, items, H, W, OH, OW, cap_rows, xb, xl, cpi, slots);                                        \
     else                                                                                                                               \
-      hipLaunchKernelGGL((crop_resize_aa_staged_kernel<K_, 8, 10>), dim3(kXcd, nbands, groups), dim3(kThreads), lds3, (hipStream_t)stream, x, \
-                         y, wx, x0, wy, y0, planes, H, W, OH, OW, cap_rows, xb, xl);                                                   \
+      hipLaunchKernelGGL((crop_resize_aa_staged_kernel<K_, 8, 10, NHWC>), dim3(kXcd, nbands, groups), dim3(kThreads), lds3, (hipStream_t)stream, x, \
+                         y, wx, x0, wy, y0, items, H, W, OH, OW, cap_rows, xb, xl, cpi, slots);                                        \
     break
       switch (K) {
         EQA_AA_STAGED(1); EQA_AA_STAGED(2); EQA_AA_STAGED(3); EQA_AA_STAGED(4); EQA_AA_STAGED(5); EQA_AA_STAGED(6); EQA_AA_STAGED(7);
@@ -422,9 +521,44 @@
       return launch_status();
     }
   }
-  hipLaunchKernelGGL(crop_resize_aa_kernel, grid, dim3(kThreads), lds, (hipStream_t)stream, x, y, wx, x0, wy, y0, H, W, OH, OW, K,
-                     max_rows);
+  if (!slots_ok(grid, status)) return status;
+  hipLaunchKernelGGL(crop_resize_aa_kernel<NHWC>, grid, dim3(kThreads), lds, (hipStream_t)stream, x, y, wx, x0, wy, y0, H, W, OH, OW, K,
+                     max_rows, cpi, slots);
   return launch_status();
 }
 
 }
+
+extern "C" {
+
+int eqa_crop_resize_aa(const float* x, float* y, const float* wx, const int32_t* x0, const float* wy, const int32_t* y0,
+                       int planes, int H, int W, int OH, int OW, int K, int max_rows, int x_begin, int x_span, void* stream) {
+  if (!x || !y || !wx || !x0 || !wy || !y0 || planes < 0 || H <= 0 || W <= 0 || OH <= 0 || OW <= 0 || K <= 0 || max_rows <= 0)
+    return EQA_ERR_INVALID_ARG;
+  if ((size_t)max_rows * OW * sizeof(float) > 96 * 1024 || planes > 65535) return EQA_ERR_UNSUPPORTED;
+  if (planes == 0) return EQA_OK;
+  return aa_launch<false>(x, y, wx, x0, wy, y0, planes, 0, H, W, OH, OW, K, max_rows, x_begin, x_span, nullptr, nullptr, false, stream);
+}
+
+int eqa_crop_resize_aa_nhwc_bound_slots(const float* x, int nimg, int planes_per_image, int H, int W, int OH, int OW, int K, int max_rows,
+                                        int x_begin, int x_span) {
+  if (nimg <= 0 || planes_per_image <= 0 || H <= 0 || W <= 0 || OH <= 0 || OW <= 0 || K <= 0 || max_rows <= 0) return 0;
+  if ((int64_t)nimg * planes_per_image > 65535) return 0;
+  int n = 0;
+  const int st = aa_launch<true>(x, nullptr, nullptr, nullptr, nullptr, nullptr, nimg * planes_per_image, planes_per_image, H, W, OH, OW, K,
+                                 max_rows, x_begin, x_span, nullptr, &n, true, nullptr);
+  return st == EQA_OK ? n : 0;
+}
+
+int eqa_crop_resize_aa_nhwc_bound(const float* x, float* y, const float* wx, const int32_t* x0, const float* wy, const int32_t* y0, int nimg,
+                                  int planes_per_image, int H, int W, int OH, int OW, int K, int max_rows, int x_begin, int x_span,
+                                  float* slots, int nslots, void* stream) {
+  if (!x || !y || !wx || !x0 || !wy || !y0 || !slots || nimg <= 0 || planes_per_image <= 0 || H <= 0 || W <= 0 || OH <= 0 || OW <= 0 ||
+      K <= 0 || max_rows <= 0 || nslots <= 0)
+    return EQA_ERR_INVALID_ARG;
+  if ((int64_t)nimg * planes_per_image > 65535) return EQA_ERR_UNSUPPORTED;
+  return aa_launch<true>(x, y, wx, x0, wy, y0, nimg * planes_per_image, planes_per_image, H, W, OH, OW, K, max_rows, x_begin, x_span, slots,
+                         &nslots, false, stream);
+}
+
+}
diff --git a/equiadapt_amd/images/canonicalization/discrete_group.py b/equiadapt_amd/images/canonicalization/discrete_group.py
--- a/equiadapt_amd/images/canonicalization/discrete_group.py
+++ b/equiadapt_amd/images/canonicalization/discrete_group.py
@@ -1,4 +1,5 @@
 import math
+import os
 from typing import Any, Dict, List, Optional, Tuple, Union
 
 import torch
@@ -19,6 +20,14 @@
     rotate_masks,
 )
 
+HEAD_FUSED_DEFAULT = "0"
+
+
+def _network_reads_channels_last(net, x: torch.Tensor, out_hw) -> bool:
+    ask = getattr(net, "reads_channels_last_input", None)
+    if ask is None or torch.is_grad_enabled() or net.training or os.environ.get("EQA_HEAD_FUSED", HEAD_FUSED_DEFAULT) == "0":
+        return False
+    return ask(x.new_empty((1,)).expand(x.shape[0], x.shape[1], out_hw[0], out_hw[1]))
 
 
 def _get(hyperparams: Any, name: str):
@@ -141,7 +150,7 @@
                 t = geometry.aa_resize_tables(tuple(x.shape[-2:]), crop.size, out_hw)
                 tabs = tuple(v.to(x.device) if isinstance(v, torch.Tensor) else v for v in t)
                 self._consts[key] = tabs
-            return ops.crop_resize_aa(x, tabs, out_hw)
+            return ops.crop_resize_aa(x, tabs, out_hw, channels_last=_network_reads_channels_last(self.canonicalization_network, x, out_hw))
         return resize(crop(x))
 
 
diff --git a/equiadapt_amd/images/canonicalization_networks/escnn_networks.py b/equiadapt_amd/images/canonicalization_networks/escnn_networks.py
--- a/equiadapt_amd/images/canonicalization_networks/escnn_networks.py
+++ b/equiadapt_amd/images/canonicalization_networks/escnn_networks.py
@@ -596,17 +596,32 @@
         k = convs[-1].kernel_size
         return hw >= 2 * k - 1 and x.shape[-1] - (self.kernel_size - 1) * (len(convs) - 1) >= 2 * k - 1 and hw * hw <= 12288
 
+    def _inference_path_ok(self, x: torch.Tensor) -> bool:
+        if self.training or torch.is_grad_enabled() or not (x.is_cuda and x.dtype == torch.float32):
+            return False
+        convs, norms = self._layers()
+        shrink = (self.kernel_size - 1) * (len(convs) - 1)
+        oh, ow = x.shape[-2] - shrink, x.shape[-1] - shrink
+        return (convs[-1].supports_linear_tail() and 0 < oh and 0 < ow and oh * ow <= 12288
+                and all(n.running_mean is not None and not n.training for n in norms)
+                and all(c.stride == 1 and c.padding == 0 and c.kernel_size == self.kernel_size for c in convs))
+
+    def reads_channels_last_input(self, x: torch.Tensor) -> bool:
+        if (self.training or torch.is_grad_enabled()) and self._training_fast_path_ok(x):
+            return False
+        if not self._inference_path_ok(x) or (self.out_channels * self.num_group_elements) % 4 != 0:
+            return False
+        convs, norms = self._layers()
+        if len(convs) < 3:
+            return False
+        bank, _ = self._folded(convs[0], norms[0])
+        return self._route(0, x, bank, convs, True)[0] == "lift_fused"
+
     def forward(self, x: torch.Tensor) -> torch.Tensor:
         if (self.training or torch.is_grad_enabled()) and self._training_fast_path_ok(x):
             return self._forward_training(x)
-        if not self.training and not torch.is_grad_enabled() and x.is_cuda and x.dtype == torch.float32:
-            convs, norms = self._layers()
-            shrink = (self.kernel_size - 1) * (len(convs) - 1)
-            oh, ow = x.shape[-2] - shrink, x.shape[-1] - shrink
-            if (convs[-1].supports_linear_tail() and 0 < oh and 0 < ow and oh * ow <= 12288
-                    and all(n.running_mean is not None and not n.training for n in norms)
-                    and all(c.stride == 1 and c.padding == 0 and c.kernel_size == self.kernel_size for c in convs)):
-                return self._forward_inference(x)
+        if self._inference_path_ok(x):
+            return self._forward_inference(x)
         if self._dense:
             convs, norms = self._dense
             for i, cv in enumerate(convs):
diff --git a/equiadapt_amd/images/canonicalization_networks/fftconv.py b/equiadapt_amd/images/canonicalization_networks/fftconv.py
--- a/equiadapt_amd/images/canonicalization_networks/fftconv.py
+++ b/equiadapt_amd/images/canonicalization_networks/fftconv.py
@@ -217,11 +217,13 @@
         vbound = None
         if LIFT_FFT_FORM == "h2" and px % 16 == 0:
             wh, w_scale = self.pieces_f16()
-            xbound = torch.empty(DCMAX_SLOTS, dtype=torch.float32, device=self.device)
-            _lib.check(lib.eqa_absmax_slots(px, self.x.numel(), xbound.data_ptr(), st), "eqa_absmax_slots")
+            xbound = ops.attached_absmax(self.x)
+            if xbound is None:
+                xbound = torch.empty(DCMAX_SLOTS, dtype=torch.float32, device=self.device)
+                _lib.check(lib.eqa_absmax_slots(px, self.x.numel(), xbound.data_ptr(), st), "eqa_absmax_slots")
             if want_dc:
                 vbound = torch.empty(DCMAX_SLOTS, dtype=torch.float32, device=self.device)
-            _lib.check(lib.eqa_lift5_fft48k5_input_f16x2(px, wh.data_ptr(), w_scale, xbound.data_ptr(), DCMAX_SLOTS, p_b, int(self.relu), pV,
+            _lib.check(lib.eqa_lift5_fft48k5_input_f16x2(px, wh.data_ptr(), w_scale, xbound.data_ptr(), xbound.numel(), p_b, int(self.relu), pV,
                                                          vbound.data_ptr() if want_dc else None, *dims), "eqa_lift5_fft48k5_input_f16x2")
         elif LIFT_FFT_FORM == "bf16x3":
             _lib.check(lib.eqa_lift5_fft48k5_input_bf16x3(px, self.pieces().data_ptr(), p_b, int(self.relu), pV, *dims),
diff --git a/equiadapt_amd/ops.py b/equiadapt_amd/ops.py
--- a/equiadapt_amd/ops.py
+++ b/equiadapt_amd/ops.py
@@ -380,17 +380,39 @@
     return vec, R, y
 
 
-def crop_resize_aa(x: torch.Tensor, tables, out_hw: Tuple[int, int]) -> torch.Tensor:
+def crop_resize_aa(x: torch.Tensor, tables, out_hw: Tuple[int, int], channels_last: bool = False) -> torch.Tensor:
     lib = _lib.load()
     x = _need(x, "x")
     wx, x0, wy, y0, K, max_rows, x_begin, x_span = tables
     B, C, H, W = x.shape
+    nslots = lib.eqa_crop_resize_aa_nhwc_bound_slots(x.data_ptr(), B, C, H, W, out_hw[0], out_hw[1], K, max_rows, x_begin,
+                                                     x_span) if channels_last else 0
+    if nslots > 0:
+        y = torch.empty((B, C, out_hw[0], out_hw[1]), dtype=torch.float32, device=x.device, memory_format=torch.channels_last)
+        slots = torch.empty(nslots, dtype=torch.float32, device=x.device)
+        with torch.cuda.device(x.device), _timed("crop_resize_aa"):
+            st = lib.eqa_crop_resize_aa_nhwc_bound(x.data_ptr(), y.data_ptr(), wx.data_ptr(), x0.data_ptr(), wy.data_ptr(), y0.data_ptr(),
+                                                   B, C, H, W, out_hw[0], out_hw[1], K, max_rows, x_begin, x_span, slots.data_ptr(), nslots,
+                                                   _stream())
+        _lib.check(st, "eqa_crop_resize_aa_nhwc_bound")
+        y._eqa_absmax = (slots, y.data_ptr(), y.numel(), y._version)
+        return y
     y = torch.empty((B, C, out_hw[0], out_hw[1]), dtype=torch.float32, device=x.device)
     with torch.cuda.device(x.device), _timed("crop_resize_aa"):
         st = lib.eqa_crop_resize_aa(x.data_ptr(), y.data_ptr(), wx.data_ptr(), x0.data_ptr(), wy.data_ptr(), y0.data_ptr(),
                                     B * C, H, W, out_hw[0], out_hw[1], K, max_rows, x_begin, x_span, _stream())
     _lib.check(st, "eqa_crop_resize_aa")
-    return y
+    return y.contiguous(memory_format=torch.channels_last) if channels_last else y
+
+
+def attached_absmax(x: torch.Tensor) -> Optional[torch.Tensor]:
+    tag = getattr(x, "_eqa_absmax", None)
+    if tag is None:
+        return None
+    slots, ptr, numel, version = tag
+    if x.data_ptr() != ptr or x.numel() != numel or x._version != version or not x.is_contiguous(memory_format=torch.channels_last):
+        return None
+    return slots
 
 
 def mask_action_nearest(masks: torch.Tensor, eidx: torch.Tensor, rtheta: torch.Tensor, flags: Optional[torch.Tensor]) -> torch.Tensor:
diff --git a/include/eqa_hip.h b/include/eqa_hip.h
--- a/include/eqa_hip.h
+++ b/include/eqa_hip.h
@@ -46,6 +46,11 @@
 
 int eqa_crop_resize_aa(const float* x, float* y, const float* wx, const int32_t* x0, const float* wy, const int32_t* y0,
                        int planes, int H, int W, int OH, int OW, int K, int max_rows, int x_begin, int x_span, void* stream);
+int eqa_crop_resize_aa_nhwc_bound_slots(const float* x, int nimg, int planes_per_image, int H, int W, int OH, int OW, int K, int max_rows,
+                                        int x_begin, int x_span);
+int eqa_crop_resize_aa_nhwc_bound(const float* x, float* y, const float* wx, const int32_t* x0, const float* wy, const int32_t* y0, int nimg,
+                                  int planes_per_image, int H, int W, int OH, int OW, int K, int max_rows, int x_begin, int x_span,
+                                  float* slots, int nslots, void* stream);
 
 int eqa_mask_action_nearest(const uint8_t* m, uint8_t* out, const int32_t* eidx, const float* rtheta, const int32_t* flags,
                             int num_elements, int n_masks, int H, int W, void* stream);
```

Measured after the change: 72750 images/s, median of 4. No clear change (+0.7%).
